# jopohl/urh

Measured on NVIDIA H100. Metric: MSamples/s IQ demod+digitize (complex64), higher is better.
Workload: dtype f32

## Files before the change

urh_b200/csrc/center.cu:

```cuda
#include "dense.cuh"
#include "tilescan.cuh"

#include <math.h>
#include <stdlib.h>

int urh_window_var_bitwise(urh_ctx* ctx, const float* d_x, int64_t n, const int64_t* d_prefix, int64_t t0, int64_t t1, int64_t r0,
                           int64_t r1, float* h_out2);

struct CenStats {
    double sum, sumsq;
    float mn, mx;
    long long cnt;
};

__global__ void __launch_bounds__(URH_WARPS_PER_BLOCK * 32)
k_tile_stats_f32(const float* __restrict__ x, int64_t n, int64_t ntiles, UrhTileStats* __restrict__ ts) {
    const int lane = threadIdx.x & 31;
    const int64_t tile = (int64_t)blockIdx.x * URH_WARPS_PER_BLOCK + (threadIdx.x >> 5);
    if (tile >= ntiles) return;
    const int64_t base = tile * URH_TILE;
    UrhStatAcc acc;
    acc.init();
    acc.all_noise = false;
    if (base + URH_TILE <= n && (((uintptr_t)x) & 15) == 0) {
        const float4* p = (const float4*)(x + base) + lane;
        constexpr int ITERS = URH_TILE / 128;
        float4 cur[4], nxt[4];
#pragma unroll
        for (int j = 0; j < 4; j++) cur[j] = __ldg(p + j * 32);
        for (int it = 0; it < ITERS; it += 4) {
            if (it + 4 < ITERS) {
#pragma unroll
                for (int j = 0; j < 4; j++) nxt[j] = __ldg(p + (it + 4 + j) * 32);
            }
#pragma unroll
            for (int j = 0; j < 4; j++) {
                acc.add(cur[j].x); acc.add(cur[j].y); acc.add(cur[j].z); acc.add(cur[j].w);
            }
#pragma unroll
            for (int j = 0; j < 4; j++) cur[j] = nxt[j];
        }
    } else {
        for (int j = lane; j < URH_TILE; j += 32)
            if (base + j < n) acc.add(x[base + j]);
    }
    acc.store(ts + tile, lane);
}

struct ScanKept {
    const UrhTileStats* ts;
    int64_t* prefix;
    __device__ __forceinline__ int64_t load(int64_t t) const { return ts[t].cnt; }
    __device__ __forceinline__ void post(int64_t t, const int64_t& excl, const int64_t&) const { prefix[t] = excl; }
};
struct CenAddI64 {
    __device__ __forceinline__ int64_t operator()(int64_t a, int64_t b) const { return a + b; }
};

static int kept_prefix(urh_ctx* ctx, const UrhTileStats* ts, int64_t ntiles, int64_t* prefix) {
    ScanKept fk;
    fk.ts = ts; fk.prefix = prefix;
    return urhts::scan<int64_t, CenAddI64, ScanKept>(ctx, ntiles, (int64_t)0, CenAddI64(), fk, prefix + ntiles);
}

#define CEN_PER (URH_TILE / 256)
__device__ __forceinline__ int64_t cen_tile_ranks(const float* __restrict__ x, int64_t n, int64_t t, int64_t tile_rank0, float (&v)[CEN_PER],
                                                  int* s_pre) {
    const int64_t base = t * URH_TILE + (int64_t)threadIdx.x * CEN_PER;
    int mine = 0;
#pragma unroll
    for (int j = 0; j < CEN_PER; j++) {
        v[j] = (base + j < n) ? x[base + j] : -5.0f;
        mine += (v[j] > -4.0f) ? 1 : 0;
    }
    s_pre[threadIdx.x] = mine;
    __syncthreads();
    for (int off = 1; off < 256; off <<= 1) {
        int add = 0;
        if (threadIdx.x >= off) add = s_pre[threadIdx.x - off];
        __syncthreads();
        s_pre[threadIdx.x] += add;
        __syncthreads();
    }
    return tile_rank0 + s_pre[threadIdx.x] - mine;
}

__device__ __forceinline__ void cen_block_fold(double sum, double sq, float mn, float mx, long long cnt, CenStats* out) {
    __shared__ double s_sum[256], s_sq[256];
    __shared__ float s_mn[256], s_mx[256];
    __shared__ long long s_cnt[256];
    __syncthreads();
    s_sum[threadIdx.x] = sum; s_sq[threadIdx.x] = sq; s_mn[threadIdx.x] = mn; s_mx[threadIdx.x] = mx; s_cnt[threadIdx.x] = cnt;
    __syncthreads();
    for (int off = 128; off > 0; off >>= 1) {
        if (threadIdx.x < off) {
            s_sum[threadIdx.x] += s_sum[threadIdx.x + off];
            s_sq[threadIdx.x] += s_sq[threadIdx.x + off];
            s_mn[threadIdx.x] = fminf(s_mn[threadIdx.x], s_mn[threadIdx.x + off]);
            s_mx[threadIdx.x] = fmaxf(s_mx[threadIdx.x], s_mx[threadIdx.x + off]);
            s_cnt[threadIdx.x] += s_cnt[threadIdx.x + off];
        }
        __syncthreads();
    }
    if (threadIdx.x == 0) {
        CenStats r;
        r.sum = s_sum[0]; r.sumsq = s_sq[0]; r.mn = s_mn[0]; r.mx = s_mx[0]; r.cnt = s_cnt[0];
        *out = r;
    }
}

int urh_center_tiles_begin(urh_ctx* ctx, const float* d_x, const UrhTileStats* ts, int64_t n, int64_t* h_total) {
    const int64_t ntiles = urh_div_up(n, URH_TILE);
    int64_t* prefix;
    URH_CHECK(urh_arena(ctx, (size_t)ntiles + 1, &prefix));
    URH_CHECK(kept_prefix(ctx, ts, ntiles, prefix));
    URH_CHECK(urh_read_i64(ctx, prefix + ntiles, 1, h_total));
    ctx->center_prefix = prefix;
    ctx->center_ts = ts;
    ctx->center_n = n;
    ctx->center_x = d_x;
    return URH_OK;
}

static int tiles_from_array(urh_ctx* ctx, const float* d_x, int64_t n, int64_t* h_total) {
    urh_arena_reset(ctx);
    ctx->center_prefix = nullptr;
    const int64_t ntiles = urh_div_up(n, URH_TILE);
    UrhTileStats* ts;
    URH_CHECK(urh_arena(ctx, (size_t)ntiles, &ts));
    URH_LAUNCH(ctx, k_tile_stats_f32, (unsigned)urh_div_up(ntiles, URH_WARPS_PER_BLOCK), URH_WARPS_PER_BLOCK * 32, 0, d_x, n, ntiles, ts);
    return urh_center_tiles_begin(ctx, d_x, ts, n, h_total);
}

static bool tiles_match(const urh_ctx* ctx, const float* d_x, int64_t n) {
    return ctx->center_prefix && ctx->center_n == n && ctx->center_x == (const void*)d_x;
}

extern "C" int urh_center_window_var(urh_ctx* ctx, const float* d_qad, int64_t n, int64_t r0, int64_t r1, double* h_out2) {
    h_out2[0] = h_out2[1] = 0.0;
    if (!tiles_match(ctx, d_qad, n)) URH_FAIL(ctx, URH_ERR_INVALID, "the tile table of this array must precede urh_center_window_var");
    if (r1 <= r0) return URH_OK;
    float mv[2];
    URH_CHECK(urh_window_var_bitwise(ctx, d_qad, n, (const int64_t*)ctx->center_prefix, 0, urh_div_up(n, URH_TILE) - 1, r0, r1, mv));
    h_out2[0] = (double)mv[0];
    h_out2[1] = (double)mv[1];
    return URH_OK;
}

extern "C" int urh_center_stats(urh_ctx* ctx, const float* d_x, int64_t n, int64_t max_size, double* h_out) {
    for (int i = 0; i < 7; i++) h_out[i] = 0.0;
    if (n <= 0) return URH_OK;
    int64_t total = 0;
    URH_CHECK(tiles_from_array(ctx, d_x, n, &total));
    int64_t r0 = (int64_t)(0.05 * (double)total), r1 = (int64_t)(0.95 * (double)total);
    if (max_size >= 0 && r1 - r0 > max_size) r1 = r0 + max_size;
    h_out[0] = (double)total; h_out[1] = (double)r0; h_out[2] = (double)r1;
    if (r1 <= r0) return URH_OK;
    double w[5];
    URH_CHECK(urh_center_window_stats(ctx, d_x, n, r0, r1, w));
    if (w[0] <= 0.0) return URH_OK;
    h_out[3] = w[1]; h_out[4] = w[2];
    float mv[2];
    URH_CHECK(urh_window_var_bitwise(ctx, d_x, n, (const int64_t*)ctx->center_prefix, 0, urh_div_up(n, URH_TILE) - 1, r0, r1, mv));
    h_out[5] = (double)mv[0];
    h_out[6] = (double)mv[1];
    return URH_OK;
}


template <typename K>
__device__ __forceinline__ double cen_edge(K k, const double& hmin, const double& edge1, const double& delta) {
    return (k == 0) ? hmin : (k == 1 ? edge1 : __dadd_rn(hmin, __dmul_rn((double)k, delta)));
}

__device__ __forceinline__ void cen_edge_table(long long k0, long long stride, long long nbins, const double& hmin, const double& edge1,
                                               const double& delta, float* __restrict__ fe, unsigned long long* __restrict__ hist,
                                               unsigned long long* __restrict__ xhist) {
    for (long long k = k0; k <= nbins; k += stride) {
        const double e = cen_edge(k, hmin, edge1, delta);
        fe[k] = __double2float_ru(e);
        if (k == nbins) {
            fe[nbins + 1] = __double2float_rd(e);
            fe[nbins + 2] = fmaxf(__double2float_ru(hmin), nextafterf(-4.0f, 0.0f));
        }
        if (k < nbins) {
            hist[k] = 0ull;
            if (xhist) xhist[k] = 0ull;
        }
    }
}

struct HistBins {
    const float* fe;
    float f_min, f_hi, scale, off;
    int nbins;
    __device__ __forceinline__ void load(const float* fe_, float scale_, int nbins_) {
        fe = fe_; nbins = nbins_; scale = scale_;
        f_hi = fe[nbins + 1];
        f_min = fe[nbins + 2];
        off = -fe[0] * scale;
    }
    template <bool FAST>
    __device__ __forceinline__ int bin_of(float f) const {
        const bool valid = f >= f_min && f <= f_hi;
        if (FAST) {
            const float t = fmaf(f, scale, off);
            int r = __float_as_int(t + 12582912.0f) - 0x4B400000;
            r = max(0, min(r, nbins));
            int k = r - ((f < fe[r]) ? 1 : 0);
            k = min(k, nbins - 1);
            return valid ? k : -1;
        }
        if (!valid) return -1;
        int k = (int)((f - fe[0]) * scale);
        k = max(0, min(k, nbins - 1));
        while (k > 0 && f < fe[k]) k--;
        while (k < nbins - 1 && f >= fe[k + 1]) k++;
        return k;
    }
};

struct HistCache {
    float lo0, hi0, lo1, hi1, lo2, hi2, lo3, hi3;
    int h0, h1, h2, h3;
    unsigned c0, c1, c2, c3;
    __device__ __forceinline__ void init() {
        lo0 = lo1 = lo2 = lo3 = INFINITY;
        hi0 = hi1 = hi2 = hi3 = -INFINITY;
        h0 = h1 = h2 = h3 = 0;
        c0 = c1 = c2 = c3 = 0u;
    }
};

template <bool SMEM>
__device__ __forceinline__ void hist_bump(unsigned int* s_hist, unsigned long long* hist, int k, unsigned c) {
    if (SMEM) atomicAdd(&s_hist[k], c);
    else atomicAdd(&hist[k], (unsigned long long)c);
}

template <bool SMEM, bool FAST>
__device__ __forceinline__ void hist_miss(HistCache& hc, const HistBins& hb, unsigned int* s_hist, unsigned long long* hist, float f) {
    const int k = hb.bin_of<FAST>(f);
    if (k < 0) return;
    const float lo = fmaxf(hb.fe[k], hb.f_min);
    const float hi = (k == hb.nbins - 1) ? nextafterf(hb.f_hi, INFINITY) : hb.fe[k + 1];
    unsigned cm = hc.c0; int which = 0;
    if (hc.c1 < cm) { cm = hc.c1; which = 1; }
    if (hc.c2 < cm) { cm = hc.c2; which = 2; }
    if (hc.c3 < cm) { cm = hc.c3; which = 3; }
    const int old = which == 0 ? hc.h0 : which == 1 ? hc.h1 : which == 2 ? hc.h2 : hc.h3;
    if (cm) hist_bump<SMEM>(s_hist, hist, old, cm);
    if (which == 0) { hc.h0 = k; hc.c0 = 1u; hc.lo0 = lo; hc.hi0 = hi; }
    else if (which == 1) { hc.h1 = k; hc.c1 = 1u; hc.lo1 = lo; hc.hi1 = hi; }
    else if (which == 2) { hc.h2 = k; hc.c2 = 1u; hc.lo2 = lo; hc.hi2 = hi; }
    else { hc.h3 = k; hc.c3 = 1u; hc.lo3 = lo; hc.hi3 = hi; }
}

template <bool SMEM, bool FAST>
__device__ __forceinline__ void hist_put(HistCache& hc, const HistBins& hb, unsigned int* s_hist, unsigned long long* hist, float f,
                                         unsigned one) {
    unsigned miss;
    asm("{\n\t.reg .pred p0, p1, p2, p3, pv;\n\t"
        "setp.ge.f32 p0, %5, %6;\n\tsetp.lt.and.f32 p0, %5, %7, p0;\n\t@p0 mad.lo.u32 %0, %0, %15, %15;\n\t"
        "setp.ge.f32 p1, %5, %8;\n\tsetp.lt.and.f32 p1, %5, %9, p1;\n\t@p1 mad.lo.u32 %1, %1, %15, %15;\n\t"
        "setp.ge.f32 p2, %5, %10;\n\tsetp.lt.and.f32 p2, %5, %11, p2;\n\t@p2 mad.lo.u32 %2, %2, %15, %15;\n\t"
        "setp.ge.f32 p3, %5, %12;\n\tsetp.lt.and.f32 p3, %5, %13, p3;\n\t@p3 mad.lo.u32 %3, %3, %15, %15;\n\t"
        "or.pred p0, p0, p1;\n\tor.pred p2, p2, p3;\n\tor.pred p0, p0, p2;\n\t"
        "setp.ge.f32 pv, %5, %14;\n\t"
        "and.pred pv, pv, !p0;\n\t"
        "selp.u32 %4, 1, 0, pv;\n\t}"
        : "+r"(hc.c0), "+r"(hc.c1), "+r"(hc.c2), "+r"(hc.c3), "=r"(miss)
        : "f"(f), "f"(hc.lo0), "f"(hc.hi0), "f"(hc.lo1), "f"(hc.hi1), "f"(hc.lo2), "f"(hc.hi2), "f"(hc.lo3), "f"(hc.hi3),
          "f"(hb.f_min), "r"(one));
    if (miss) hist_miss<SMEM, FAST>(hc, hb, s_hist, hist, f);
}

template <bool SMEM>
__device__ __forceinline__ void hist_flush(HistCache& hc, unsigned int* s_hist, unsigned long long* hist) {
    if (hc.c0) hist_bump<SMEM>(s_hist, hist, hc.h0, hc.c0);
    if (hc.c1) hist_bump<SMEM>(s_hist, hist, hc.h1, hc.c1);
    if (hc.c2) hist_bump<SMEM>(s_hist, hist, hc.h2, hc.c2);
    if (hc.c3) hist_bump<SMEM>(s_hist, hist, hc.h3, hc.c3);
}

template <bool SMEM, bool FAST>
__device__ __forceinline__ void hist_interior_body(const float* __restrict__ x, int64_t n, int64_t t_first, int64_t t_end, int blk, int nblk,
                                                   const float* __restrict__ g_fe, float scale, int nbins,
                                                   unsigned long long* __restrict__ hist, int edges_in_smem,
                                                   const int64_t* __restrict__ prefix) {
    extern __shared__ unsigned int s_dyn[];
    unsigned int* s_hist = s_dyn;
    float* s_fe = (float*)(s_dyn + (SMEM ? nbins : 0));
    const int lane = threadIdx.x & 31;
    if (SMEM)
        for (int b = threadIdx.x; b < nbins; b += 256) s_hist[b] = 0u;
    if (edges_in_smem)
        for (int b = threadIdx.x; b < nbins + 3; b += 256) s_fe[b] = g_fe[b];
    __syncthreads();
    HistBins hb;
    if (FAST) hb.load(s_fe, scale, nbins);
    else hb.load(edges_in_smem ? s_fe : g_fe, scale, nbins);
    HistCache hc;
    hc.init();
    const int64_t gw = (int64_t)blk * 8 + (threadIdx.x >> 5), nw = (int64_t)nblk * 8;
    const bool vec = (((uintptr_t)x) & 15) == 0;
    const unsigned one = blockDim.x >> 8;
    {
        for (int64_t t = t_first + gw; t < t_end; t += nw) {
            if (prefix[t + 1] == prefix[t]) continue;
            const int64_t base = t * URH_TILE;
            if (vec) {
                const float4* p = (const float4*)(x + base) + lane;
                constexpr int ITERS = URH_TILE / 128, DEPTH = 4;
                float4 buf[DEPTH];
#pragma unroll
                for (int j = 0; j < DEPTH; j++) buf[j] = __ldg(p + j * 32);
#pragma unroll 1
                for (int it = 0; it < ITERS; it += DEPTH) {
                    const bool more = it + DEPTH < ITERS;
#pragma unroll
                    for (int j = 0; j < DEPTH; j++) {
                        const float4 v = buf[j];
                        if (more) buf[j] = __ldg(p + (it + DEPTH + j) * 32);
                        hist_put<SMEM, FAST>(hc, hb, s_hist, hist, v.x, one);
                        hist_put<SMEM, FAST>(hc, hb, s_hist, hist, v.y, one);
                        hist_put<SMEM, FAST>(hc, hb, s_hist, hist, v.z, one);
                        hist_put<SMEM, FAST>(hc, hb, s_hist, hist, v.w, one);
                    }
                }
            } else {
                for (int j = lane; j < URH_TILE; j += 32) hist_put<SMEM, FAST>(hc, hb, s_hist, hist, x[base + j], one);
            }
        }
    }
    hist_flush<SMEM>(hc, s_hist, hist);
    if (SMEM) {
        __syncthreads();
        for (int b = threadIdx.x; b < nbins; b += 256)
            if (s_hist[b]) atomicAdd(&hist[b], (unsigned long long)s_hist[b]);
    }
}

__device__ __forceinline__ void hist_window_ends_body(const float* __restrict__ x, int64_t n, const int64_t* __restrict__ prefix,
                                                      const int64_t* __restrict__ win, int64_t r0, int64_t r1,
                                                      const float* __restrict__ g_fe, float scale, int nbins,
                                                      unsigned long long* __restrict__ hist, unsigned long long* __restrict__ hist2 = nullptr) {
    __shared__ int s_pre[256];
    const int64_t t = win[blockIdx.x];
    if (t < 0 || (blockIdx.x == 1 && t == win[0])) return;
    HistBins hb;
    hb.load(g_fe, scale, nbins);
    float v[CEN_PER];
    int64_t rank = cen_tile_ranks(x, n, t, prefix[t], v, s_pre);
#pragma unroll
    for (int j = 0; j < CEN_PER; j++) {
        const bool kept = v[j] > -4.0f;
        const int k = hb.bin_of<false>(v[j]);
        if (k >= 0 && rank >= r0 && rank < r1) {
            atomicAdd(&hist[k], 1ull);
            if (hist2) atomicAdd(&hist2[k], 1ull);
        }
        rank += kept ? 1 : 0;
    }
}

extern "C" int urh_center_histogram(urh_ctx* ctx, const float* d_x, int64_t n, int64_t r0, int64_t r1, double hmin,
                                    double hstep, int64_t nbins, int64_t* h_hist) {
    if (nbins <= 0 || n <= 0) return URH_OK;
    if (!tiles_match(ctx, d_x, n)) {
        int64_t total = 0;
        URH_CHECK(tiles_from_array(ctx, d_x, n, &total));
    }
    return urh_center_histogram_tiles(ctx, d_x, n, r0, r1, hmin, hstep, nbins, h_hist);
}

#define CEN_MAX_BINS 6000
#define CEN_VAR_MIN_RATIO 0x1p-14

struct __align__(16) CenterPlan {
    long long total, offset;
    long long r0, r1;
    long long lr0, lr1;
    long long win[4];
    CenStats local;
    double hmin, edge1, delta;
    long long nbins;
    double center;
    float centerf;
    float scale;
    int fast;
    int state;
    unsigned int ticket;
    int certified;
    long long straddle;
    long long pad;
};

__global__ void k_center_ranks(const int64_t* __restrict__ counts, int rank, int world, int64_t max_size, CenterPlan* __restrict__ plan) {
    long long total = 0, offset = 0;
    for (int q = 0; q < world; q++) {
        if (q < rank) offset += counts[q];
        total += counts[q];
    }
    const long long kept = counts[rank];
    long long r0 = (long long)(0.05 * (double)total), r1 = (long long)(0.95 * (double)total);
    if (max_size >= 0 && r1 - r0 > max_size) r1 = r0 + max_size;
    plan->total = total; plan->offset = offset; plan->r0 = r0; plan->r1 = r1;
    long long a = r0 - offset, b = r1 - offset;
    a = a < 0 ? 0 : (a > kept ? kept : a);
    b = b < 0 ? 0 : (b > kept ? kept : b);
    plan->lr0 = a; plan->lr1 = b;
    plan->ticket = 0u;
    plan->state = 1;
    plan->certified = 0;
    plan->straddle = 0;
}

__device__ __forceinline__ int64_t cen_tile_of_rank(const int64_t* __restrict__ prefix, int64_t ntiles, int64_t r) {
    int64_t lo = 0, hi = ntiles;
    while (hi - lo > 1) {
        const int64_t mid = (lo + hi) >> 1;
        if (prefix[mid] <= r) lo = mid; else hi = mid;
    }
    return lo;
}

__device__ __forceinline__ void cen_window_tiles(const int64_t* __restrict__ prefix, int64_t ntiles, long long r0, long long r1,
                                                 long long (&w)[4]) {
    long long w0 = -1, w1 = -1, w2 = -1, w3 = -1;
    if (r1 > r0) {
        w0 = cen_tile_of_rank(prefix, ntiles, r0);
        w1 = cen_tile_of_rank(prefix, ntiles, r1 - 1);
        const bool cov0 = prefix[w0] >= r0 && prefix[w0 + 1] <= r1;
        const bool cov1 = prefix[w1] >= r0 && prefix[w1 + 1] <= r1;
        w2 = cov0 ? -1 : w0;
        w3 = (cov1 || w1 == w0) ? -1 : w1;
    }
    w[0] = w0; w[1] = w1; w[2] = w2; w[3] = w3;
}

__global__ void __launch_bounds__(256) k_center_window(const float* __restrict__ x, int64_t n, const UrhTileStats* __restrict__ ts,
                                                      const int64_t* __restrict__ prefix, int64_t ntiles, CenterPlan* __restrict__ plan,
                                                      CenStats* __restrict__ partial) {
    __shared__ long long s_win[4];
    __shared__ int s_pre[256];
    __shared__ bool s_last;
    const long long r0 = plan->lr0, r1 = plan->lr1;
    if (threadIdx.x == 0) {
        long long w[4];
        cen_window_tiles(prefix, ntiles, r0, r1, w);
        s_win[0] = w[0]; s_win[1] = w[1]; s_win[2] = w[2]; s_win[3] = w[3];
        if (blockIdx.x == 0) { plan->win[0] = w[0]; plan->win[1] = w[1]; plan->win[2] = w[2]; plan->win[3] = w[3]; }
    }
    __syncthreads();
    double sum = 0.0, sq = 0.0;
    float mn = INFINITY, mx = -INFINITY;
    long long cnt = 0;
    if (s_win[0] >= 0) {
        for (int64_t t = s_win[0] + (int64_t)blockIdx.x * 256 + threadIdx.x; t <= s_win[1]; t += (int64_t)gridDim.x * 256) {
            const int64_t a = prefix[t], b = prefix[t + 1];
            if (b > a && a >= r0 && b <= r1) {
                const UrhTileStats v = ts[t];
                sum += v.sum; sq += v.sumsq; mn = fminf(mn, v.mn); mx = fmaxf(mx, v.mx); cnt += v.cnt;
            }
        }
    }
    cen_block_fold(sum, sq, mn, mx, cnt, partial + blockIdx.x);
    if (blockIdx.x < 2) {
        const int64_t t = s_win[2 + blockIdx.x];
        sum = 0.0; sq = 0.0; mn = INFINITY; mx = -INFINITY; cnt = 0;
        if (t >= 0) {
            float v[CEN_PER];
            int64_t rank = cen_tile_ranks(x, n, t, prefix[t], v, s_pre);
#pragma unroll
            for (int j = 0; j < CEN_PER; j++) {
                if (v[j] > -4.0f) {
                    if (rank >= r0 && rank < r1) {
                        sum += (double)v[j];
                        sq += (double)v[j] * (double)v[j];
                        mn = fminf(mn, v[j]);
                        mx = fmaxf(mx, v[j]);
                        cnt++;
                    }
                    rank++;
                }
            }
        }
        cen_block_fold(sum, sq, mn, mx, cnt, partial + gridDim.x + blockIdx.x);
    }
    __threadfence();
    __syncthreads();
    if (threadIdx.x == 0) s_last = atomicAdd(&plan->ticket, 1u) == gridDim.x - 1;
    __syncthreads();
    if (!s_last) return;
    __threadfence();
    sum = 0.0; sq = 0.0; mn = INFINITY; mx = -INFINITY; cnt = 0;
    for (int64_t t = threadIdx.x; t < (int64_t)gridDim.x + 2; t += 256) {
        CenStats p;
        {
            const int4* src = (const int4*)(partial + t);
            int4 w0 = __ldcg(src), w1 = __ldcg(src + 1);
            memcpy(&p, &w0, 16);
            memcpy((char*)&p + 16, &w1, 16);
        }
        sum += p.sum; sq += p.sumsq; mn = fminf(mn, p.mn); mx = fmaxf(mx, p.mx); cnt += p.cnt;
    }
    cen_block_fold(sum, sq, mn, mx, cnt, &plan->local);
}

__global__ void __launch_bounds__(256) k_center_plan(const CenStats* __restrict__ parts, int world, CenterPlan* __restrict__ plan,
                                                    float* __restrict__ fe, unsigned long long* __restrict__ hist,
                                                    unsigned long long* __restrict__ xhist) {
    __shared__ int s_state;
    __shared__ long long s_nbins;
    __shared__ double s_hmin, s_edge1, s_delta;
    if (threadIdx.x == 0) {
        double cnt = 0.0, sum = 0.0, sq = 0.0;
        float mn = INFINITY, mx = -INFINITY;
        for (int q = 0; q < world; q++) {
            cnt += (double)parts[q].cnt;
            mn = fminf(mn, parts[q].mn);
            mx = fmaxf(mx, parts[q].mx);
            sum = __dadd_rn(sum, parts[q].sum);
            sq = __dadd_rn(sq, parts[q].sumsq);
        }
        int state = 0;
        long long nbins = 0;
        double hmin = 0.0, edge1 = 0.0, delta = 0.0;
        if (plan->r1 > plan->r0 && cnt > 0.0) {
            const double mean = __ddiv_rn(sum, cnt);
            double ss = __dsub_rn(sq, __dmul_rn(__dmul_rn(cnt, mean), mean));
            if (ss < 0.0) ss = 0.0;
            const double var = __ddiv_rn(ss, cnt);
            const double hstep = (double)__double2float_rn(var);
            hmin = (double)mn;
            const double stop = __dadd_rn((double)mx, hstep);
            if (!(var >= __dmul_rn(__dmul_rn(mean, mean), CEN_VAR_MIN_RATIO))) state = 2;
            else if (hstep != 0.0) {
                const double val = __ddiv_rn(__dsub_rn(stop, hmin), hstep);
                if (val == val && fabs(val) < 9.0e18) {
                    const long long len = (long long)ceil(val);
                    if (len >= 2) {
                        nbins = len - 1;
                        edge1 = __dadd_rn(hmin, hstep);
                        delta = __dsub_rn(edge1, hmin);
                        state = (nbins <= CEN_MAX_BINS && delta > 0.0) ? 1 : 2;
                    }
                }
            }
        }
        plan->hmin = hmin; plan->edge1 = edge1; plan->delta = delta; plan->nbins = nbins;
        plan->state = state;
        plan->center = 0.0; plan->centerf = 0.0f;
        if (state == 1) {
            plan->scale = (float)(1.0 / delta);
            const double edge_abs = fmax(fabs(hmin), fabs(hmin + (double)nbins * delta));
            plan->fast = (edge_abs / delta < 1048576.0) ? 1 : 0;
        }
        s_state = state; s_nbins = nbins; s_hmin = hmin; s_edge1 = edge1; s_delta = delta;
    }
    __syncthreads();
    if (s_state != 1) return;
    cen_edge_table(threadIdx.x, 256, s_nbins, s_hmin, s_edge1, s_delta, fe, hist, xhist);
}

template <bool SMEM, bool FAST, int MIN_BLOCKS>
__global__ void __launch_bounds__(256, MIN_BLOCKS) k_hist_interior(const float* __restrict__ x, int64_t n, const CenterPlan* __restrict__ plan,
                                                                  const float* __restrict__ g_fe, unsigned long long* __restrict__ hist,
                                                                  const int64_t* __restrict__ prefix, int edges_in_smem) {
    if (plan->state != 1 || plan->certified || (plan->fast != 0) != FAST) return;
    hist_interior_body<SMEM, FAST>(x, n, plan->win[0] + 1, plan->win[1], blockIdx.x, gridDim.x, g_fe, plan->scale, (int)plan->nbins, hist,
                                   edges_in_smem, prefix);
}

__device__ __forceinline__ void cen_full_slabs(int64_t win0, int64_t win1, int64_t slab_tiles, int64_t* sf, int64_t* se) {
    *sf = (win0 + slab_tiles) / slab_tiles;
    *se = win1 / slab_tiles;
}

__global__ void __launch_bounds__(256) k_hist_window_ends(const float* __restrict__ x, int64_t n, const int64_t* __restrict__ prefix,
                                                         const CenterPlan* __restrict__ plan, const float* __restrict__ g_fe,
                                                         unsigned long long* __restrict__ hist, unsigned long long* __restrict__ xhist,
                                                         int64_t slab_tiles) {
    if (plan->state != 1) return;
    if (blockIdx.x < 2) {
        hist_window_ends_body(x, n, prefix, (const int64_t*)plan->win, plan->lr0, plan->lr1, g_fe, plan->scale, (int)plan->nbins, hist, xhist);
        return;
    }
    const int64_t w0 = plan->win[0], w1 = plan->win[1];
    int64_t sf, se;
    cen_full_slabs(w0, w1, slab_tiles, &sf, &se);
    int64_t a_end = w1, b_begin = w1;
    if (sf < se) { a_end = sf * slab_tiles; b_begin = se * slab_tiles; }
    const int blk = blockIdx.x - 2, nblk = gridDim.x - 2, nbins = (int)plan->nbins;
    const float scale = plan->scale;
    if (plan->fast) {
        hist_interior_body<true, true>(x, n, w0 + 1, a_end, blk, nblk, g_fe, scale, nbins, xhist, 1, prefix);
        hist_interior_body<true, true>(x, n, b_begin, w1, blk, nblk, g_fe, scale, nbins, xhist, 1, prefix);
    } else {
        hist_interior_body<true, false>(x, n, w0 + 1, a_end, blk, nblk, g_fe, scale, nbins, xhist, 1, prefix);
        hist_interior_body<true, false>(x, n, b_begin, w1, blk, nblk, g_fe, scale, nbins, xhist, 1, prefix);
    }
}

__device__ __forceinline__ double cen_left_edge(const CenterPlan* plan, int k) {
    return cen_edge(k, plan->hmin, plan->edge1, plan->delta);
}

#define CERT_THREADS 512
__global__ void __launch_bounds__(CERT_THREADS) k_center_certify(const UrhFine fine, CenterPlan* __restrict__ plan, const float* __restrict__ fe,
                                                                 const unsigned long long* __restrict__ xhist, unsigned long long* __restrict__ lo,
                                                                 unsigned long long* __restrict__ hi) {
    __shared__ unsigned long long s_ge[URH_FINE_NB + 1];
    __shared__ unsigned long long s_part[CERT_THREADS];
    __shared__ unsigned char s_flag[CEN_MAX_BINS];
    __shared__ unsigned long long s_key[3];
    __shared__ unsigned int s_certain;
    if (plan->state != 1) return;
    const int tid = threadIdx.x;
    constexpr int PER = URH_FINE_NB / CERT_THREADS;
    int64_t sf, se;
    cen_full_slabs(plan->win[0], plan->win[1], fine.slab_tiles, &sf, &se);
    unsigned long long b[PER], tot = 0;
#pragma unroll
    for (int j = 0; j < PER; j++) {
        unsigned long long v = 0;
        for (int64_t sl = sf; sl < se; sl++) v += fine.gh[sl * URH_FINE_NB + tid * PER + j];
        b[j] = v;
        tot += v;
    }
    s_part[tid] = tot;
    if (tid < 3) s_key[tid] = 0ull;
    if (tid == 0) s_certain = 0u;
    __syncthreads();
    for (int off = 1; off < CERT_THREADS; off <<= 1) {
        const unsigned long long add = (tid + off < CERT_THREADS) ? s_part[tid + off] : 0ull;
        __syncthreads();
        s_part[tid] += add;
        __syncthreads();
    }
    unsigned long long run = (tid + 1 < CERT_THREADS) ? s_part[tid + 1] : 0ull;
#pragma unroll
    for (int j = PER - 1; j >= 0; j--) {
        run += b[j];
        s_ge[tid * PER + j] = run;
    }
    if (tid == 0) s_ge[URH_FINE_NB] = 0ull;
    __syncthreads();
    const int nbins = (int)plan->nbins;
    const float f_hi = fe[nbins + 1], f_min = fe[nbins + 2], top = nextafterf(f_hi, INFINITY);
    auto ge = [&](float t, unsigned long long& glo, unsigned long long& ghi) {
        const int bt = urh_fine_bucket(t, fine.scale, fine.off);
        const bool straddles = urh_fine_bucket(nextafterf(t, -INFINITY), fine.scale, fine.off) == bt;
        ghi = s_ge[bt];
        glo = straddles ? s_ge[bt + 1] : s_ge[bt];
    };
    for (int k = tid; k < nbins; k += CERT_THREADS) {
        const float a = fmaxf(fe[k], f_min), e = (k == nbins - 1) ? top : fminf(fe[k + 1], top);
        unsigned long long l = 0, u = 0;
        if (a < e) {
            unsigned long long alo, ahi, elo, ehi;
            ge(a, alo, ahi);
            ge(e, elo, ehi);
            l = alo > ehi ? alo - ehi : 0ull;
            u = ahi - elo;
        }
        lo[k] = xhist[k] + l;
        hi[k] = xhist[k] + u;
    }
    __syncthreads();
    int window = (int)(0.05 * (double)nbins) + 1;
    if (window < 2) window = 2;
    for (int k = tid; k < nbins; k += CERT_THREADS) {
        const unsigned long long l = lo[k], u = hi[k];
        bool certain = l > 0ull, possible = u > 0ull;
        for (int d = -(window - 1); d < window && (certain || possible); d++) {
            const int j = k + d;
            if (d == 0 || j < 0 || j >= nbins) continue;
            certain = certain && l > hi[j];
            possible = possible && u > lo[j];
        }
        s_flag[k] = certain ? 1 : (possible ? 2 : 0);
        if (certain) atomicAdd(&s_certain, 1u);
    }
    __syncthreads();
    for (int pass = 0; pass < 3; pass++) {
        const long long p0 = pass > 0 ? (long long)(8191 - (s_key[0] & 8191)) : -1, p1 = pass > 1 ? (long long)(8191 - (s_key[1] & 8191)) : -1;
        for (int k = tid; k < nbins; k += CERT_THREADS) {
            if (k == p0 || k == p1) continue;
            if (pass < 2 && s_flag[k] == 1) atomicMax(&s_key[pass], (lo[k] << 13) | (unsigned long long)(8191 - k));
            if (pass == 2 && s_flag[k] != 0) atomicMax(&s_key[2], hi[k]);
        }
        __syncthreads();
    }
    if (tid != 0 || s_certain < 2u) return;
    const int k1 = 8191 - (int)(s_key[0] & 8191), k2 = 8191 - (int)(s_key[1] & 8191);
    plan->straddle = (long long)((hi[k1] - lo[k1]) + (hi[k2] - lo[k2]));
    if (!(lo[k2] > s_key[2])) return;
    const double c = __ddiv_rn(__dadd_rn(cen_left_edge(plan, k1), cen_left_edge(plan, k2)), 2.0);
    plan->center = c;
    plan->centerf = __double2float_rn(c);
    plan->certified = 1;
}

__global__ void __launch_bounds__(256) k_center_pick(const unsigned long long* __restrict__ y, CenterPlan* __restrict__ plan) {
    __shared__ unsigned long long s_best[256];
    __shared__ int s_idx[256];
    __shared__ int s_cnt[256];
    if (plan->state != 1 || plan->certified) return;
    const int nbins = (int)plan->nbins;
    int window = (int)(0.05 * (double)nbins) + 1;
    if (window < 2) window = 2;
    unsigned long long top_val[2] = {0ull, 0ull};
    int top_idx[2] = {-1, -1};
    int found = 0;
    bool undecided = false;
    for (int pass = 0; pass < 2 && !undecided; pass++) {
        unsigned long long best = 0ull;
        int bi = -1, ties = 0;
        for (int i = threadIdx.x; i < nbins; i += 256) {
            if (pass == 1 && i == top_idx[0]) continue;
            const unsigned long long v = y[i];
            if (v == 0ull || v < best) continue;
            bool peak = true;
            for (int d = 1; d < window && peak; d++) {
                const unsigned long long a = (i + d < nbins) ? y[i + d] : 0ull;
                const unsigned long long b = (i - d >= 0) ? y[i - d] : 0ull;
                peak = v > a && v > b;
            }
            if (!peak) continue;
            if (v > best) { best = v; bi = i; ties = 1; }
            else ties++;
        }
        s_best[threadIdx.x] = best; s_idx[threadIdx.x] = bi; s_cnt[threadIdx.x] = ties;
        __syncthreads();
        if (threadIdx.x == 0) {
            unsigned long long b = 0ull;
            int idx = -1, t = 0;
            for (int j = 0; j < 256; j++) {
                if (s_idx[j] < 0) continue;
                if (s_best[j] > b) { b = s_best[j]; idx = s_idx[j]; t = s_cnt[j]; }
                else if (s_best[j] == b) t += s_cnt[j];
            }
            s_best[0] = b; s_idx[0] = idx; s_cnt[0] = t;
        }
        __syncthreads();
        const unsigned long long b = s_best[0];
        const int idx = s_idx[0], t = s_cnt[0];
        __syncthreads();
        if (idx < 0) break;
        if (pass == 0) {
            top_val[0] = b; top_idx[0] = idx; found = 1;
            if (t == 2) {
                int other = -1;
                for (int i = threadIdx.x; i < nbins; i += 256) {
                    if (i == idx || y[i] != b) continue;
                    bool peak = true;
                    for (int d = 1; d < window && peak; d++) {
                        const unsigned long long a = (i + d < nbins) ? y[i + d] : 0ull;
                        const unsigned long long c = (i - d >= 0) ? y[i - d] : 0ull;
                        peak = b > a && b > c;
                    }
                    if (peak) other = i;
                }
                s_idx[threadIdx.x] = other;
                __syncthreads();
                if (threadIdx.x == 0) {
                    int o = -1;
                    for (int j = 0; j < 256; j++) if (s_idx[j] >= 0) o = s_idx[j];
                    s_idx[0] = o;
                }
                __syncthreads();
                top_idx[1] = s_idx[0]; top_val[1] = b; found = 2;
                __syncthreads();
                break;
            }
            if (t > 2) undecided = true;
        } else {
            if (t > 1) undecided = true;
            else { top_val[1] = b; top_idx[1] = idx; found = 2; }
        }
    }
    if (threadIdx.x != 0) return;
    if (undecided) { plan->state = 2; return; }
    if (found == 0) { plan->state = 0; return; }
    double c;
    if (found == 1) c = cen_left_edge(plan, top_idx[0]);
    else c = __ddiv_rn(__dadd_rn(cen_left_edge(plan, top_idx[0]), cen_left_edge(plan, top_idx[1])), 2.0);
    plan->center = c;
    plan->centerf = __double2float_rn(c);
    plan->state = 1;
    (void)top_val;
}

__global__ void __launch_bounds__(256) k_center_set(const int64_t* __restrict__ prefix, int64_t ntiles, long long r0, long long r1, double hmin,
                                                   double hstep, long long nbins, float scale, int fast, CenterPlan* __restrict__ plan,
                                                   float* __restrict__ fe, unsigned long long* __restrict__ hist) {
    const double edge1 = __dadd_rn(hmin, hstep);
    if (blockIdx.x == 0 && threadIdx.x == 0) {
        plan->lr0 = r0; plan->lr1 = r1;
        plan->ticket = 0u;
        plan->state = 1;
        plan->certified = 0;
        if (nbins > 0) {
            long long w[4];
            cen_window_tiles(prefix, ntiles, r0, r1, w);
            for (int i = 0; i < 4; i++) plan->win[i] = w[i];
            plan->hmin = hmin; plan->edge1 = edge1; plan->delta = hstep; plan->nbins = nbins;
            plan->scale = scale;
            plan->fast = fast;
        }
    }
    if (nbins > 0)
        cen_edge_table((long long)blockIdx.x * blockDim.x + threadIdx.x, (long long)gridDim.x * blockDim.x, nbins, hmin, edge1, hstep, fe, hist,
                       nullptr);
}

extern "C" int urh_center_window_stats(urh_ctx* ctx, const float* d_qad, int64_t n, int64_t r0, int64_t r1, double* h_out5) {
    h_out5[0] = 0.0; h_out5[1] = INFINITY; h_out5[2] = -INFINITY; h_out5[3] = 0.0; h_out5[4] = 0.0;
    if (!tiles_match(ctx, d_qad, n)) URH_FAIL(ctx, URH_ERR_INVALID, "urh_afp_demod_tiles (same qad, same n) must precede urh_center_window_stats");
    if (r1 <= r0) return URH_OK;
    const int64_t ntiles = urh_div_up(n, URH_TILE);
    const int64_t* prefix = (const int64_t*)ctx->center_prefix;
    CenterPlan* plan;
    CenStats* partial;
    const int nb = ctx->sm_count * 2;
    URH_CHECK(urh_arena(ctx, 1, &plan));
    URH_CHECK(urh_arena(ctx, (size_t)nb + 2, &partial));
    URH_LAUNCH(ctx, k_center_set, 1, 1, 0, prefix, ntiles, (long long)r0, (long long)r1, 0.0, 0.0, 0LL, 0.0f, 0, plan, nullptr, nullptr);
    URH_LAUNCH(ctx, k_center_window, nb, 256, 0, d_qad, n, (const UrhTileStats*)ctx->center_ts, prefix, ntiles, plan, partial);
    CenStats st;
    URH_CUDA(ctx, cudaMemcpyAsync(ctx->h_mail, &plan->local, sizeof(CenStats), cudaMemcpyDeviceToHost, ctx->stream));
    URH_CUDA(ctx, cudaStreamSynchronize(ctx->stream));
    memcpy(&st, ctx->h_mail, sizeof(st));
    h_out5[0] = (double)st.cnt; h_out5[1] = (double)st.mn; h_out5[2] = (double)st.mx; h_out5[3] = st.sum; h_out5[4] = st.sumsq;
    return URH_OK;
}

extern "C" int urh_center_histogram_tiles(urh_ctx* ctx, const float* d_qad, int64_t n, int64_t r0, int64_t r1, double hmin,
                                          double hstep, int64_t nbins, int64_t* h_hist) {
    if (nbins <= 0) return URH_OK;
    if (!tiles_match(ctx, d_qad, n)) URH_FAIL(ctx, URH_ERR_INVALID, "urh_afp_demod_tiles (same qad, same n) must precede urh_center_histogram_tiles");
    if (nbins > (int64_t)1 << 30) URH_FAIL(ctx, URH_ERR_INVALID, "too many histogram bins");
    if (r1 <= r0) {
        memset(h_hist, 0, (size_t)nbins * sizeof(int64_t));
        return URH_OK;
    }
    const int64_t ntiles = urh_div_up(n, URH_TILE);
    const int64_t* prefix = (const int64_t*)ctx->center_prefix;
    CenterPlan* plan;
    float* fe;
    unsigned long long* hist;
    URH_CHECK(urh_arena(ctx, 1, &plan));
    URH_CHECK(urh_arena(ctx, (size_t)nbins + 3, &fe));
    URH_CHECK(urh_arena(ctx, (size_t)nbins, &hist));
    const bool in_smem = nbins <= 12000;
    const int edges_smem = (in_smem && nbins <= 6000) ? 1 : 0;
    const size_t dyn = (in_smem ? (size_t)nbins * 4 : 0) + (edges_smem ? (size_t)(nbins + 3) * 4 : 0);
    const float scale = (float)(1.0 / hstep);
    const double edge_abs = fmax(fabs(hmin), fabs(hmin + (double)nbins * hstep));
    const int fast = (edges_smem && hstep > 0.0 && edge_abs / hstep < 1048576.0) ? 1 : 0;
    const unsigned gs = (unsigned)min(urh_div_up(ntiles, 8), (int64_t)ctx->sm_count * 8);
    URH_LAUNCH(ctx, k_center_set, (unsigned)urh_div_up(nbins + 1, 256), 256, 0, prefix, ntiles, (long long)r0, (long long)r1, hmin, hstep,
               (long long)nbins, scale, fast, plan, fe, hist);
    const CenterPlan* cplan = plan;
    const float* cfe = fe;
    if (fast) URH_LAUNCH(ctx, (k_hist_interior<true, true, 3>), gs, 256, dyn, d_qad, n, cplan, cfe, hist, prefix, edges_smem);
    else if (edges_smem) URH_LAUNCH(ctx, (k_hist_interior<true, false, 3>), gs, 256, dyn, d_qad, n, cplan, cfe, hist, prefix, edges_smem);
    else if (in_smem) URH_LAUNCH(ctx, (k_hist_interior<true, false, 4>), gs, 256, dyn, d_qad, n, cplan, cfe, hist, prefix, edges_smem);
    else URH_LAUNCH(ctx, (k_hist_interior<false, false, 4>), gs, 256, dyn, d_qad, n, cplan, cfe, hist, prefix, edges_smem);
    URH_LAUNCH(ctx, k_hist_window_ends, 2, 256, 0, d_qad, n, prefix, cplan, cfe, hist, (unsigned long long*)nullptr, (int64_t)1);
    URH_CUDA(ctx, cudaMemcpyAsync(h_hist, hist, (size_t)nbins * sizeof(int64_t), cudaMemcpyDeviceToHost, ctx->stream));
    URH_CUDA(ctx, cudaStreamSynchronize(ctx->stream));
    return URH_OK;
}

int urh_center_chain(urh_ctx* ctx, const float* d_qad, int64_t n, const UrhTileStats* ts, int64_t max_size, int rank, int world,
                     const UrhFine* fine, CenterPlan** d_plan_out) {
    const int64_t ntiles = urh_div_up(n, URH_TILE);
    int64_t* prefix;
    CenterPlan* plan;
    CenStats* partial;
    float* fe;
    unsigned long long* hist;
    int64_t* d_counts;
    CenStats* d_parts;
    unsigned long long *xhist = nullptr, *cert_lo = nullptr, *cert_hi = nullptr;
    const int nb = ctx->sm_count * 2;
    URH_CHECK(urh_arena(ctx, (size_t)ntiles + 1, &prefix));
    URH_CHECK(urh_arena(ctx, 1, &plan));
    URH_CHECK(urh_arena(ctx, (size_t)nb + 2, &partial));
    URH_CHECK(urh_arena(ctx, (size_t)CEN_MAX_BINS + 3, &fe));
    URH_CHECK(urh_arena(ctx, (size_t)CEN_MAX_BINS, &hist));
    URH_CHECK(urh_arena(ctx, (size_t)world, &d_counts));
    URH_CHECK(urh_arena(ctx, (size_t)world, &d_parts));
    if (fine) {
        URH_CHECK(urh_arena(ctx, (size_t)CEN_MAX_BINS, &xhist));
        URH_CHECK(urh_arena(ctx, (size_t)CEN_MAX_BINS, &cert_lo));
        URH_CHECK(urh_arena(ctx, (size_t)CEN_MAX_BINS, &cert_hi));
    }
    URH_CHECK(kept_prefix(ctx, ts, ntiles, prefix));
    const int64_t* counts = prefix + ntiles;
    if (world > 1) {
        URH_TL_MARK(ctx, "x1 kept counts: enter");
        URH_CHECK(urh_nccl_allgather(ctx, prefix + ntiles, d_counts, sizeof(int64_t)));
        URH_TL_MARK(ctx, "x1 kept counts: done");
        counts = d_counts;
    }
    URH_LAUNCH(ctx, k_center_ranks, 1, 1, 0, counts, rank, world, max_size, plan);
    URH_LAUNCH(ctx, k_center_window, nb, 256, 0, d_qad, n, ts, (const int64_t*)prefix, ntiles, plan, partial);
    const CenStats* parts = &plan->local;
    if (world > 1) {
        URH_TL_MARK(ctx, "x2 window partials: enter");
        URH_CHECK(urh_nccl_allgather(ctx, &plan->local, d_parts, sizeof(CenStats)));
        URH_TL_MARK(ctx, "x2 window partials: done");
        parts = d_parts;
    }
    URH_LAUNCH(ctx, k_center_plan, 1, 256, 0, parts, world, plan, fe, hist, xhist);
    const size_t dyn = (size_t)CEN_MAX_BINS * 4 + (size_t)(CEN_MAX_BINS + 3) * 4;
    const unsigned gs = (unsigned)min(urh_div_up(ntiles, 8), (int64_t)ctx->sm_count * 8);
    URH_LAUNCH(ctx, k_hist_window_ends, fine ? 2 + ctx->sm_count * 4 : 2, 256, fine ? dyn : 0, d_qad, n, (const int64_t*)prefix,
               (const CenterPlan*)plan, (const float*)fe, hist, xhist, fine ? fine->slab_tiles : (int64_t)1);
    if (fine) URH_LAUNCH(ctx, k_center_certify, 1, CERT_THREADS, 0, *fine, plan, (const float*)fe, (const unsigned long long*)xhist, cert_lo, cert_hi);
    URH_LAUNCH(ctx, (k_hist_interior<true, true, 3>), gs, 256, dyn, d_qad, n, (const CenterPlan*)plan, (const float*)fe, hist, (const int64_t*)prefix, 1);
    URH_LAUNCH(ctx, (k_hist_interior<true, false, 3>), gs, 256, dyn, d_qad, n, (const CenterPlan*)plan, (const float*)fe, hist, (const int64_t*)prefix, 1);
    if (world > 1) {
        URH_TL_MARK(ctx, "x3 histogram sum: enter");
        URH_CHECK(urh_nccl_allreduce_i64(ctx, (int64_t*)hist, CEN_MAX_BINS, 0));
        URH_TL_MARK(ctx, "x3 histogram sum: done");
    }
    URH_LAUNCH(ctx, k_center_pick, 1, 256, 0, (const unsigned long long*)hist, plan);
    ctx->center_prefix = prefix;
    ctx->center_ts = ts;
    ctx->center_n = n;
    ctx->center_x = d_qad;
    *d_plan_out = plan;
    return URH_OK;
}

int urh_center_plan_certify_stats(urh_ctx* ctx, const CenterPlan* plan, int64_t* h_dst3) {
    h_dst3[0] = h_dst3[1] = h_dst3[2] = 0;
    URH_CUDA(ctx, cudaMemcpyAsync(h_dst3, &plan->certified, sizeof(int), cudaMemcpyDeviceToHost, ctx->stream));
    URH_CUDA(ctx, cudaMemcpyAsync(h_dst3 + 2, &plan->straddle, sizeof(long long), cudaMemcpyDeviceToHost, ctx->stream));
    return URH_OK;
}

extern "C" int urh_center_certify_stats(urh_ctx* ctx, int64_t* h_out3) {
    for (int i = 0; i < 3; i++) h_out3[i] = ctx->center_cert[i];
    return URH_OK;
}

int urh_center_plan_result(urh_ctx* ctx, const CenterPlan* plan, const float** d_centerf, const double** d_center, const int** d_state) {
    if (d_centerf) *d_centerf = &plan->centerf;
    if (d_center) *d_center = &plan->center;
    if (d_state) *d_state = &plan->state;
    return URH_OK;
}
```

urh_b200/csrc/dense.cuh:

```cuda
#pragma once
#include "common.cuh"
#include "fdlibm_atan2f.h"

#define URH_TILE 2048
#define URH_WARPS_PER_BLOCK 8
#define URH_MAX_THR 255

struct UrhClassify {
    float noise_value;
    int order;
    float thr[URH_MAX_THR];
};

struct __align__(16) UrhTileSummary {
    int16_t first_cls;
    int16_t last_cls;
    int32_t head_len;
    int32_t tail_len;
    int32_t ncand;
};

struct __align__(16) UrhTileStats {
    double sum, sumsq;
    float mn, mx;
    int32_t cnt;
    int32_t all_noise;
};

struct UrhStatAcc {
    double sum, sumsq;
    float mn, mx;
    int cnt;
    bool all_noise;
    __device__ __forceinline__ void init() { sum = 0.0; sumsq = 0.0; mn = INFINITY; mx = -INFINITY; cnt = 0; all_noise = true; }
    __device__ __forceinline__ void add(float v) {
        if (v > -4.0f) {
            const double d = (double)v;
            sum += d;
            sumsq += d * d;
            mn = fminf(mn, v);
            mx = fmaxf(mx, v);
            cnt++;
        }
    }
    __device__ __forceinline__ void store(UrhTileStats* out, int lane) {
        for (int off = 16; off > 0; off >>= 1) {
            sum += __shfl_down_sync(URH_FULL_MASK, sum, off);
            sumsq += __shfl_down_sync(URH_FULL_MASK, sumsq, off);
            mn = fminf(mn, __shfl_down_sync(URH_FULL_MASK, mn, off));
            mx = fmaxf(mx, __shfl_down_sync(URH_FULL_MASK, mx, off));
            cnt += __shfl_down_sync(URH_FULL_MASK, cnt, off);
        }
        const int alln = __all_sync(URH_FULL_MASK, all_noise) ? 1 : 0;
        if (lane == 0) {
            UrhTileStats t;
            t.sum = sum; t.sumsq = sumsq; t.mn = mn; t.mx = mx; t.cnt = cnt; t.all_noise = alln;
            *out = t;
        }
    }
};

#define URH_FINE_NB 4096
#define URH_FINE_SLABS 64
struct UrhFine {
    unsigned int* gh;
    int64_t slab_tiles;
    float scale, off;
};
__device__ __forceinline__ int urh_fine_bucket(float f, float scale, float off) {
    float t = __fmaf_rd(f, scale, off + 8388608.0f);
    t = fminf(fmaxf(t, 8388608.0f), 8388608.0f + (float)(URH_FINE_NB - 1));
    return __float_as_int(t) - 0x4B000000;
}
__device__ __forceinline__ void urh_fine_add(float f, const UrhFine& fn, unsigned int* s, unsigned int* g) {
    if (f > -4.0f) {
        const int b = urh_fine_bucket(f, fn.scale, fn.off);
        if (g) atomicAdd(g + b, 1u);
        else atomicAdd(s + b, 1u);
    }
}
__device__ __forceinline__ unsigned int* urh_fine_row(const UrhFine& fn, int64_t tile, int64_t block_tile0) {
    const int64_t slab = tile / fn.slab_tiles;
    return (slab == block_tile0 / fn.slab_tiles) ? nullptr : fn.gh + slab * URH_FINE_NB;
}
__device__ __forceinline__ void urh_fine_zero(unsigned int* s) {
    for (int w = threadIdx.x * 4; w < URH_FINE_NB; w += blockDim.x * 4) *(uint4*)(s + w) = make_uint4(0u, 0u, 0u, 0u);
    __syncthreads();
}
__device__ __forceinline__ void urh_fine_flush(const UrhFine& fn, unsigned int* s, int64_t block_tile0) {
    __syncthreads();
    unsigned int* g = fn.gh + (block_tile0 / fn.slab_tiles) * URH_FINE_NB;
    for (int w = threadIdx.x * 4; w < URH_FINE_NB; w += blockDim.x * 4) {
        const uint4 v = *(const uint4*)(s + w);
        if (v.x) atomicAdd(g + w, v.x);
        if (v.y) atomicAdd(g + w + 1, v.y);
        if (v.z) atomicAdd(g + w + 2, v.z);
        if (v.w) atomicAdd(g + w + 3, v.w);
    }
}

__device__ __forceinline__ void urh_cmulf(float a, float b, float c, float d, float& re, float& im) {
    const float ac = __fmul_rn(a, c), bd = __fmul_rn(b, d), ad = __fmul_rn(a, d), bc = __fmul_rn(b, c);
    re = __fsub_rn(ac, bd);
    im = __fadd_rn(ad, bc);
    if (isnan(re) && isnan(im)) {
        bool recalc = false;
        if (isinf(a) || isinf(b)) {
            a = copysignf(isinf(a) ? 1.0f : 0.0f, a);
            b = copysignf(isinf(b) ? 1.0f : 0.0f, b);
            if (isnan(c)) c = copysignf(0.0f, c);
            if (isnan(d)) d = copysignf(0.0f, d);
            recalc = true;
        }
        if (isinf(c) || isinf(d)) {
            c = copysignf(isinf(c) ? 1.0f : 0.0f, c);
            d = copysignf(isinf(d) ? 1.0f : 0.0f, d);
            if (isnan(a)) a = copysignf(0.0f, a);
            if (isnan(b)) b = copysignf(0.0f, b);
            recalc = true;
        }
        if (!recalc && (isinf(ac) || isinf(bd) || isinf(ad) || isinf(bc))) {
            if (isnan(a)) a = copysignf(0.0f, a);
            if (isnan(b)) b = copysignf(0.0f, b);
            if (isnan(c)) c = copysignf(0.0f, c);
            if (isnan(d)) d = copysignf(0.0f, d);
            recalc = true;
        }
        if (recalc) {
            re = __fmul_rn(INFINITY, __fsub_rn(__fmul_rn(a, c), __fmul_rn(b, d)));
            im = __fmul_rn(INFINITY, __fadd_rn(__fmul_rn(a, d), __fmul_rn(b, c)));
        }
    }
}

template <int DT> struct UrhElem;
template <> struct UrhElem<URH_DT_I8> { typedef int8_t type; };
template <> struct UrhElem<URH_DT_U8> { typedef uint8_t type; };
template <> struct UrhElem<URH_DT_I16> { typedef int16_t type; };
template <> struct UrhElem<URH_DT_U16> { typedef uint16_t type; };
template <> struct UrhElem<URH_DT_F32> { typedef float type; };

struct UrhPair {
    float r0, i0, r1, i1;
};

__device__ __forceinline__ float4 urh_ldg_f4(const void* p) {
    float4 v;
    asm volatile("ld.global.nc.L1::no_allocate.v4.f32 {%0,%1,%2,%3}, [%4];"
                 : "=f"(v.x), "=f"(v.y), "=f"(v.z), "=f"(v.w)
                 : "l"(p));
    return v;
}
__device__ __forceinline__ uint2 urh_ldg_u2(const void* p) {
    uint2 v;
    asm volatile("ld.global.nc.L1::no_allocate.v2.u32 {%0,%1}, [%2];" : "=r"(v.x), "=r"(v.y) : "l"(p));
    return v;
}
__device__ __forceinline__ uint32_t urh_ldg_u1(const void* p) {
    uint32_t v;
    asm volatile("ld.global.nc.L1::no_allocate.u32 %0, [%1];" : "=r"(v) : "l"(p));
    return v;
}
__device__ __forceinline__ void urh_stg_f2(float* p, float a, float b) {
    asm volatile("st.global.L1::no_allocate.v2.f32 [%0], {%1,%2};" ::"l"(p), "f"(a), "f"(b) : "memory");
}

template <int DT>
__device__ __forceinline__ UrhPair urh_load_pair(const void* base, int64_t i, int64_t n, bool vec) {
    typedef typename UrhElem<DT>::type E;
    const E* p = (const E*)base + 2 * i;
    UrhPair o;
    o.r0 = o.i0 = o.r1 = o.i1 = 0.0f;
    if (i + 1 < n && vec) {
        if (DT == URH_DT_F32) {
            const float4 v = urh_ldg_f4(p);
            o.r0 = v.x; o.i0 = v.y; o.r1 = v.z; o.i1 = v.w;
        } else if (DT == URH_DT_I16) {
            const uint2 v = urh_ldg_u2(p);
            o.r0 = (float)(int16_t)(v.x & 0xffff); o.i0 = (float)(int16_t)(v.x >> 16);
            o.r1 = (float)(int16_t)(v.y & 0xffff); o.i1 = (float)(int16_t)(v.y >> 16);
        } else if (DT == URH_DT_U16) {
            const uint2 v = urh_ldg_u2(p);
            o.r0 = (float)(v.x & 0xffff); o.i0 = (float)(v.x >> 16);
            o.r1 = (float)(v.y & 0xffff); o.i1 = (float)(v.y >> 16);
        } else if (DT == URH_DT_I8) {
            const uint32_t v = urh_ldg_u1(p);
            o.r0 = (float)(int8_t)(v & 0xff); o.i0 = (float)(int8_t)((v >> 8) & 0xff);
            o.r1 = (float)(int8_t)((v >> 16) & 0xff); o.i1 = (float)(int8_t)(v >> 24);
        } else {
            const uint32_t v = urh_ldg_u1(p);
            o.r0 = (float)(v & 0xff); o.i0 = (float)((v >> 8) & 0xff);
            o.r1 = (float)((v >> 16) & 0xff); o.i1 = (float)(v >> 24);
        }
    } else {
        if (i < n) { o.r0 = (float)__ldg(p); o.i0 = (float)__ldg(p + 1); }
        if (i + 1 < n) { o.r1 = (float)__ldg(p + 2); o.i1 = (float)__ldg(p + 3); }
    }
    return o;
}

struct UrhDemodParams {
    float noise_sqrd;
    float noise_value;
    float max_mag;
    float one, mone;
};

struct UrhFskTerms {
    float A, B, C, D;
};
__device__ __forceinline__ UrhFskTerms urh_fsk_terms(float re, float im) {
    UrhFskTerms t;
    const float zt = __fsub_rn(__fmul_rn(0.0f, im), 0.0f);
    t.C = __fadd_rn(re, zt);
    t.A = __fsub_rn(re, zt);
    t.D = __fadd_rn(0.0f, im);
    t.B = __fsub_rn(0.0f, t.D);
    return t;
}
__device__ __forceinline__ float urh_fsk_angle(float A, float B, float C, float D) {
    float xr, xi;
    urh_cmulf(A, B, C, D, xr, xi);
    return urh_atan2f_v2(xi, xr);
}

__device__ __forceinline__ int urh_classify(float s, const UrhClassify& C) {
    if (s == C.noise_value) return -1;
    if (C.order == 2) return (s <= C.thr[0]) ? 0 : 1;
    int c = C.order - 1;
    for (int k = 0; k < C.order - 1; k++) {
        if (s <= C.thr[k]) { c = k; break; }
    }
    return c;
}

__device__ __forceinline__ uint64_t urh_spread_bits(uint32_t x) {
    uint64_t v = x;
    v = (v | (v << 16)) & 0x0000FFFF0000FFFFull;
    v = (v | (v << 8)) & 0x00FF00FF00FF00FFull;
    v = (v | (v << 4)) & 0x0F0F0F0F0F0F0F0Full;
    v = (v | (v << 2)) & 0x3333333333333333ull;
    v = (v | (v << 1)) & 0x5555555555555555ull;
    return v;
}

struct UrhRunTracker {
    int tol;
    int run_start, run_cls, first_cls, head_len, ncand, carry_cls;
    bool is_head;
    uint32_t cm_n, cm_a;
    uint32_t* stage;

    __device__ __forceinline__ void init(int tol_, uint32_t* stage_) {
        tol = tol_; stage = stage_;
        run_start = 0; run_cls = -2; first_cls = -2; head_len = 0; ncand = 0; carry_cls = -2; is_head = true;
        cm_n = 0xffffffffu; cm_a = 0xffffffffu;
    }
    __device__ __forceinline__ void emit(int pos, int cls, int lane) {
        if (lane == 0) stage[ncand] = ((uint32_t)pos << 16) | (uint32_t)(cls + 1);
        ncand++;
    }
    __device__ __forceinline__ void feed(int it, int c0, int c1, bool v0, bool v1, int lane) {
        int pc = __shfl_up_sync(URH_FULL_MASK, c1, 1);
        if (lane == 0) pc = carry_cls;
        const bool b0 = v0 && (c0 != pc);
        const bool b1 = v1 && (c1 != c0);
        carry_cls = __shfl_sync(URH_FULL_MASK, c1, 31);
        const uint32_t m0 = __ballot_sync(URH_FULL_MASK, b0);
        const uint32_t m1 = __ballot_sync(URH_FULL_MASK, b1);
        if ((m0 | m1) == 0u) return;
        walk(it, m0, m1, c0, c1, lane);
    }
    __device__ __forceinline__ void feed_masks(int it, uint32_t n0, uint32_t a0, uint32_t n1, uint32_t a1, int lane) {
        if ((((n0 ^ cm_n) | (n1 ^ cm_n)) | ((a0 ^ cm_a) | (a1 ^ cm_a))) == 0u) return;
        uint32_t m0 = (((n1 << 1) | (cm_n & 1u)) ^ n0) | (((a1 << 1) | (cm_a & 1u)) ^ a0);
        if (run_cls == -2) m0 |= 1u;
        uint32_t m1 = (n0 ^ n1) | (a0 ^ a1);
        feed_masks_slow(it, n0, a0, n1, a1, m0, m1, lane);
        cm_n = (run_cls < 0) ? 0xffffffffu : 0u;
        cm_a = (run_cls == 1) ? 0xffffffffu : 0u;
    }
    __device__ __forceinline__ void feed_masks_slow(int it, uint32_t n0, uint32_t a0, uint32_t n1, uint32_t a1, uint32_t m0, uint32_t m1,
                                                    int lane) {
        const int nb = __popc(m0) + __popc(m1);
        if (nb == 1 && run_cls != -2 && !is_head) {
            const bool take0 = m0 != 0u;
            const int l = __ffs(m0 | m1) - 1;
            const int p = it * 64 + 2 * l + (take0 ? 0 : 1);
            const uint32_t nbit = ((take0 ? n0 : n1) >> l) & 1u, abit = ((take0 ? a0 : a1) >> l) & 1u;
            if (p - run_start > tol) emit(run_start + tol, run_cls, lane);
            run_start = p;
            run_cls = nbit ? -1 : (int)abit;
            return;
        }
        if (nb > 4) {
            const int c0 = ((n0 >> lane) & 1u) ? -1 : (int)((a0 >> lane) & 1u);
            const int c1 = ((n1 >> lane) & 1u) ? -1 : (int)((a1 >> lane) & 1u);
            walk_parallel(it, m0, m1, c0, c1, lane);
            return;
        }
        while (m0 | m1) {
            const int l0 = m0 ? (__ffs(m0) - 1) : 64;
            const int l1 = m1 ? (__ffs(m1) - 1) : 64;
            const bool take0 = l0 <= l1;
            const int l = take0 ? l0 : l1;
            if (take0) m0 &= m0 - 1; else m1 &= m1 - 1;
            const int p = it * 64 + 2 * l + (take0 ? 0 : 1);
            const uint32_t nbit = ((take0 ? n0 : n1) >> l) & 1u, abit = ((take0 ? a0 : a1) >> l) & 1u;
            const int cls_p = nbit ? -1 : (int)abit;
            if (run_cls == -2) {
                first_cls = cls_p;
            } else if (is_head) {
                head_len = p;
                is_head = false;
            } else if (p - run_start > tol) {
                emit(run_start + tol, run_cls, lane);
            }
            run_start = p;
            run_cls = cls_p;
        }
    }
    __device__ __forceinline__ void walk(int it, uint32_t m0, uint32_t m1, int c0, int c1, int lane) {
        if (__popc(m0) + __popc(m1) > 4) {
            walk_parallel(it, m0, m1, c0, c1, lane);
            return;
        }
        while (m0 | m1) {
            const int l0 = m0 ? (__ffs(m0) - 1) : 64;
            const int l1 = m1 ? (__ffs(m1) - 1) : 64;
            const bool take0 = l0 <= l1;
            const int l = take0 ? l0 : l1;
            if (take0) m0 &= m0 - 1; else m1 &= m1 - 1;
            const int p = it * 64 + 2 * l + (take0 ? 0 : 1);
            const int cls_p = __shfl_sync(URH_FULL_MASK, take0 ? c0 : c1, l);
            if (run_cls == -2) {
                first_cls = cls_p;
            } else if (is_head) {
                head_len = p;
                is_head = false;
            } else if (p - run_start > tol) {
                emit(run_start + tol, run_cls, lane);
            }
            run_start = p;
            run_cls = cls_p;
        }
    }
    __device__ __forceinline__ void walk_parallel(int it, uint32_t m0, uint32_t m1, int c0, int c1, int lane) {
        const uint32_t lt = (1u << lane) - 1u;
        const int base = it * 64;
        int cprev0 = __shfl_up_sync(URH_FULL_MASK, c1, 1);
        if (lane == 0) cprev0 = run_cls;
        const int cprev1 = c0;
        const uint32_t b1 = m1 & lt, b0 = m0 & lt;
        int q0 = -1;
        if (b1) q0 = 2 * (31 - __clz(b1)) + 1;
        if (b0) q0 = max(q0, 2 * (31 - __clz(b0)));
        const bool has0 = (m0 >> lane) & 1u, has1 = (m1 >> lane) & 1u;
        const int q1 = has0 ? 2 * lane : q0;
        const bool carried_head = is_head;
        const int start0 = (q0 >= 0) ? base + q0 : run_start;
        const int start1 = (q1 >= 0) ? base + q1 : run_start;
        const int p0 = base + 2 * lane, p1 = p0 + 1;
        const bool head0 = (q0 >= 0) ? (start0 == 0) : (carried_head || run_cls == -2);
        const bool head1 = (q1 >= 0) ? (start1 == 0) : (carried_head || run_cls == -2);
        const bool emit0 = has0 && !head0 && (p0 - start0 > tol);
        const bool emit1 = has1 && !head1 && (p1 - start1 > tol);
        const uint32_t e0 = __ballot_sync(URH_FULL_MASK, emit0), e1 = __ballot_sync(URH_FULL_MASK, emit1);
        const int before = __popc(e0 & lt) + __popc(e1 & lt);
        if (emit0) stage[ncand + before] = ((uint32_t)(start0 + tol) << 16) | (uint32_t)(cprev0 + 1);
        if (emit1) stage[ncand + before + (emit0 ? 1 : 0)] = ((uint32_t)(start1 + tol) << 16) | (uint32_t)(cprev1 + 1);
        ncand += __popc(e0) + __popc(e1);
        uint32_t f0 = m0, f1 = m1;
        if (run_cls == -2) {
            first_cls = __shfl_sync(URH_FULL_MASK, c0, 0);
            f0 &= ~1u;
        }
        if (is_head && (f0 | f1)) {
            const int l0 = f0 ? (__ffs(f0) - 1) : 64, l1 = f1 ? (__ffs(f1) - 1) : 64;
            head_len = base + ((l0 <= l1) ? 2 * l0 : 2 * l1 + 1);
            is_head = false;
        }
        const int h0 = m0 ? (31 - __clz(m0)) : -1, h1 = m1 ? (31 - __clz(m1)) : -1;
        const bool last_is_1 = h1 >= h0;
        const int hl = last_is_1 ? h1 : h0;
        run_start = base + 2 * hl + (last_is_1 ? 1 : 0);
        run_cls = __shfl_sync(URH_FULL_MASK, last_is_1 ? c1 : c0, hl);
    }
    __device__ __forceinline__ void finish(int tile_len, UrhTileSummary* out, int lane) {
        if (is_head) head_len = tile_len;
        else if (tile_len - run_start > tol) emit(run_start + tol, run_cls, lane);
        if (lane == 0) {
            UrhTileSummary s;
            s.first_cls = (int16_t)first_cls;
            s.last_cls = (int16_t)run_cls;
            s.head_len = head_len;
            s.tail_len = tile_len - run_start;
            s.ncand = ncand;
            *out = s;
        }
    }
};

struct UrhTileResolve {
    uint32_t n0, a0, n1, a1;
    __device__ __forceinline__ void init() { n0 = a0 = n1 = a1 = 0u; }
    __device__ __forceinline__ void keep(int g, uint32_t gn0, uint32_t ga0, uint32_t gn1, uint32_t ga1, int lane) {
        if (lane == g) { n0 = gn0; a0 = ga0; n1 = gn1; a1 = ga1; }
    }
    __device__ __forceinline__ static int cls_of(uint32_t nbit, uint32_t abit) { return (nbit & 1u) ? -1 : (int)(abit & 1u); }

    template <bool WRITE>
    __device__ __forceinline__ int walk(uint32_t m0, uint32_t m1, uint32_t pn, uint32_t pa, int q, int tol, int lane, uint32_t* dst) const {
        int k = 0;
        const int base = lane * 64;
        while (m0 | m1) {
            const int l0 = m0 ? (__ffs(m0) - 1) : 64;
            const int l1 = m1 ? (__ffs(m1) - 1) : 64;
            const bool take0 = l0 <= l1;
            const int l = take0 ? l0 : l1;
            if (take0) m0 &= m0 - 1; else m1 &= m1 - 1;
            const int p = base + 2 * l + (take0 ? 0 : 1);
            if (q > 0 && p - q > tol) {
                if (WRITE) {
                    uint32_t nb, ab;
                    if (!take0) { nb = n0 >> l; ab = a0 >> l; }
                    else if (l > 0) { nb = n1 >> (l - 1); ab = a1 >> (l - 1); }
                    else { nb = pn; ab = pa; }
                    dst[k] = ((uint32_t)(q + tol) << 16) | (uint32_t)(cls_of(nb, ab) + 1);
                }
                k++;
            }
            q = p;
        }
        return k;
    }

    __device__ __forceinline__ void finish(int tol, uint32_t* stage, UrhTileSummary* out, int lane) const {
        const uint32_t pn = __shfl_up_sync(URH_FULL_MASK, n1 >> 31, 1), pa = __shfl_up_sync(URH_FULL_MASK, a1 >> 31, 1);
        uint32_t m0 = (((n1 << 1) | (pn & 1u)) ^ n0) | (((a1 << 1) | (pa & 1u)) ^ a0);
        if (lane == 0) m0 |= 1u;
        const uint32_t m1 = (n0 ^ n1) | (a0 ^ a1);
        int last = -1;
        if (m1) last = lane * 64 + 2 * (31 - __clz(m1)) + 1;
        if (m0) last = max(last, lane * 64 + 2 * (31 - __clz(m0)));
        int incl = last;
#pragma unroll
        for (int off = 1; off < 32; off <<= 1) {
            const int t = __shfl_up_sync(URH_FULL_MASK, incl, off);
            if (lane >= off) incl = max(incl, t);
        }
        int q = __shfl_up_sync(URH_FULL_MASK, incl, 1);
        if (lane == 0) q = -1;
        const int L = __shfl_sync(URH_FULL_MASK, incl, 31);
        uint32_t f0 = m0, f1 = m1;
        if (lane == 0) f0 &= ~1u;
        int first = URH_TILE;
        if (f0 | f1) {
            const int l0 = f0 ? (__ffs(f0) - 1) : 64, l1 = f1 ? (__ffs(f1) - 1) : 64;
            first = lane * 64 + ((l0 <= l1) ? 2 * l0 : 2 * l1 + 1);
        }
        const int head_len = __reduce_min_sync(URH_FULL_MASK, first);
        const int mine = walk<false>(m0, m1, pn, pa, q, tol, lane, nullptr);
        int pre = mine;
#pragma unroll
        for (int off = 1; off < 32; off <<= 1) {
            const int t = __shfl_up_sync(URH_FULL_MASK, pre, off);
            if (lane >= off) pre += t;
        }
        int total = __shfl_sync(URH_FULL_MASK, pre, 31);
        if (mine) walk<true>(m0, m1, pn, pa, q, tol, lane, stage + (pre - mine));
        const int last_cls = __shfl_sync(URH_FULL_MASK, cls_of(n1 >> 31, a1 >> 31), 31);
        if (L > 0 && URH_TILE - L > tol) {
            if (lane == 0) stage[total] = ((uint32_t)(L + tol) << 16) | (uint32_t)(last_cls + 1);
            total++;
        }
        if (lane == 0) {
            UrhTileSummary s;
            s.first_cls = (int16_t)cls_of(n0, a0);
            s.last_cls = (int16_t)last_cls;
            s.head_len = head_len;
            s.tail_len = URH_TILE - L;
            s.ncand = total;
            *out = s;
        }
    }
};
```

urh_b200/csrc/digitize.cu:

```cuda
#include "dense.cuh"
#include "tilescan.cuh"
#include "sparse.cuh"
#include "fsk_fast.cuh"
#include "dense_f32.cuh"
#include "stream_ring.cuh"

#include <math.h>
#include <stdlib.h>


template <int DT, int MOD, bool DIGITIZE>
__device__ __forceinline__ void dense_iq_tile(const void* __restrict__ iq, int64_t n, const UrhDemodParams& dp, float* __restrict__ qad_out,
                                              int vec_in, int vec_out, const UrhClassify& cls, int tol, UrhTileSummary* __restrict__ tiles,
                                              uint32_t* __restrict__ staging, int stage_cap, int16_t* __restrict__ init_cls, int cls_of_zero,
                                              int64_t tile, int has_halo, UrhTileStats* __restrict__ tile_stats, const UrhFine& fine,
                                              unsigned int* s_fine, unsigned int* g_fine) {
    const int lane = threadIdx.x & 31;
    const int64_t tile_start = tile * URH_TILE;
    const int tile_len = (int)((n - tile_start) < URH_TILE ? (n - tile_start) : URH_TILE);
    const int iters = (tile_len + 63) >> 6;

    UrhRunTracker rt;
    if (DIGITIZE) rt.init(tol, staging + tile * (int64_t)stage_cap);
    UrhStatAcc acc;
    acc.init();

    float cA = 0.0f, cB = 0.0f;
    if (MOD == URH_MOD_FSK && (tile_start > 0 || has_halo) && lane == 0) {
        typedef typename UrhElem<DT>::type E;
        const E* pp = (const E*)iq + 2 * (tile_start - 1);
        const UrhFskTerms t = urh_fsk_terms((float)pp[0], (float)pp[1]);
        cA = t.A; cB = t.B;
    }

    UrhPair cur = urh_load_pair<DT>(iq, tile_start + 2 * lane, n, vec_in != 0);
    for (int it = 0; it < iters; it++) {
        const int64_t pos0 = tile_start + (int64_t)it * 64 + 2 * lane;
        UrhPair nxt;
        if (it + 1 < iters) nxt = urh_load_pair<DT>(iq, pos0 + 64, n, vec_in != 0);

        const float m0 = __fadd_rn(__fmul_rn(cur.r0, cur.r0), __fmul_rn(cur.i0, cur.i0));
        const float m1 = __fadd_rn(__fmul_rn(cur.r1, cur.r1), __fmul_rn(cur.i1, cur.i1));
        float s0 = dp.noise_value, s1 = dp.noise_value;
        if (MOD == URH_MOD_FSK) {
            const UrhFskTerms t0 = urh_fsk_terms(cur.r0, cur.i0);
            const UrhFskTerms t1 = urh_fsk_terms(cur.r1, cur.i1);
            float pA = __shfl_up_sync(URH_FULL_MASK, t1.A, 1);
            float pB = __shfl_up_sync(URH_FULL_MASK, t1.B, 1);
            if (lane == 0) { pA = cA; pB = cB; }
            cA = __shfl_sync(URH_FULL_MASK, t1.A, 31);
            cB = __shfl_sync(URH_FULL_MASK, t1.B, 31);
            if (!(m0 <= dp.noise_sqrd)) s0 = urh_fsk_angle(pA, pB, t0.C, t0.D);
            if (!(m1 <= dp.noise_sqrd)) s1 = urh_fsk_angle(t0.A, t0.B, t1.C, t1.D);
        } else if (MOD == URH_MOD_ASK) {
            if (!(m0 <= dp.noise_sqrd)) s0 = __fdiv_rn(__fsqrt_rn(m0), dp.max_mag);
            if (!(m1 <= dp.noise_sqrd)) s1 = __fdiv_rn(__fsqrt_rn(m1), dp.max_mag);
        }
        if (pos0 == 0 && !has_halo) s0 = dp.noise_value;

        const bool v0 = pos0 < n, v1 = pos0 + 1 < n;
        if (tile_stats) {
            if (v0) { acc.add(s0); acc.all_noise = acc.all_noise && (s0 == dp.noise_value); }
            if (v1) { acc.add(s1); acc.all_noise = acc.all_noise && (s1 == dp.noise_value); }
            if (s_fine) {
                if (v0) urh_fine_add(s0, fine, s_fine, g_fine);
                if (v1) urh_fine_add(s1, fine, s_fine, g_fine);
            }
        }
        if (qad_out) {
            if (v1 && vec_out) urh_stg_f2(qad_out + pos0, s0, s1);
            else {
                if (v0) qad_out[pos0] = s0;
                if (v1) qad_out[pos0 + 1] = s1;
            }
        }
        if (DIGITIZE) {
            const int c0 = urh_classify(s0, cls), c1 = urh_classify(s1, cls);
            if (pos0 == 0) *init_cls = (int16_t)((s0 == cls.noise_value) ? -1 : cls_of_zero);
            rt.feed(it, c0, c1, v0, v1, lane);
        }
        cur = nxt;
    }
    if (tile_stats) acc.store(tile_stats + tile, lane);
    if (DIGITIZE) rt.finish(tile_len, tiles + tile, lane);
}

template <int DT, int MOD, bool DIGITIZE>
__global__ void __launch_bounds__(URH_WARPS_PER_BLOCK * 32)
k_dense_iq(const void* __restrict__ iq, int64_t n, UrhDemodParams dp, float* __restrict__ qad_out, int vec_in,
           int vec_out, const __grid_constant__ UrhClassify cls, int tol, UrhTileSummary* __restrict__ tiles,
           uint32_t* __restrict__ staging, int stage_cap, int16_t* __restrict__ init_cls, int cls_of_zero,
           int64_t tile_begin, int64_t tile_count, int has_halo, UrhTileStats* __restrict__ tile_stats, const UrhFine fine) {
    extern __shared__ unsigned int s_fine[];
    const int64_t tile_rel = (int64_t)blockIdx.x * URH_WARPS_PER_BLOCK + (threadIdx.x >> 5);
    const int64_t block_tile0 = tile_begin + (int64_t)blockIdx.x * URH_WARPS_PER_BLOCK;
    if (fine.gh) urh_fine_zero(s_fine);
    if (tile_rel < tile_count && (tile_begin + tile_rel) * URH_TILE < n)
        dense_iq_tile<DT, MOD, DIGITIZE>(iq, n, dp, qad_out, vec_in, vec_out, cls, tol, tiles, staging, stage_cap, init_cls, cls_of_zero,
                                    tile_begin + tile_rel, has_halo, tile_stats, fine,
                                    fine.gh ? s_fine : nullptr, fine.gh ? urh_fine_row(fine, tile_begin + tile_rel, block_tile0) : nullptr);
    if (fine.gh) urh_fine_flush(fine, s_fine, block_tile0);
}

template <int DT, bool DIGITIZE, bool WRITE, bool STATS>
__global__ void __launch_bounds__(URH_WARPS_PER_BLOCK * 32, (DT == URH_DT_F32) ? 5 : 4)
k_fsk_fifo(const void* __restrict__ iq, int64_t n, UrhDemodParams dp, float* __restrict__ qad_out, float thr0,
           float cls_noise, int tol, UrhTileSummary* __restrict__ tiles, uint32_t* __restrict__ staging, int stage_cap,
           int64_t tile_begin, int64_t tile_count, UrhTileStats* __restrict__ tile_stats, const UrhFine fine,
           const float* __restrict__ d_thr0 = nullptr, float* __restrict__ margin = nullptr) {
    __shared__ __align__(16) unsigned char s_fifo[URH_WARPS_PER_BLOCK][URH_FSK_FIFO + 1][64 * 2 * sizeof(typename UrhElem<DT>::type)];
    extern __shared__ unsigned int s_fine[];
    const bool fine_on = STATS && fine.gh;
    if (DIGITIZE && STATS) thr0 = *d_thr0;
    const int lane = threadIdx.x & 31;
    const int64_t tile_rel = (int64_t)blockIdx.x * URH_WARPS_PER_BLOCK + (threadIdx.x >> 5);
    const int64_t block_tile0 = tile_begin + (int64_t)blockIdx.x * URH_WARPS_PER_BLOCK;
    if (fine_on) urh_fine_zero(s_fine);
    if (tile_rel < tile_count) {
        const int64_t tile = tile_begin + tile_rel;
        UrhRunTracker rt;
        if (DIGITIZE) rt.init(tol, staging + tile * (int64_t)stage_cap);
        UrhOne one;
        one.p = dp.one;
        one.m = dp.mone;
        const uint32_t fifo = (uint32_t)__cvta_generic_to_shared(&s_fifo[threadIdx.x >> 5][0][0]);
        urh_fsk_full_tile<DT, DIGITIZE, WRITE, STATS>(iq, n, tile * URH_TILE, dp, qad_out, thr0, cls_noise, rt, lane, one,
                                                      STATS ? tile_stats + tile : nullptr, fifo, DIGITIZE ? tiles + tile : nullptr, fine,
                                                      fine_on ? s_fine : nullptr, fine_on ? urh_fine_row(fine, tile, block_tile0) : nullptr,
                                                      (DIGITIZE && STATS) ? margin + tile : nullptr);
    }
    if (fine_on) urh_fine_flush(fine, s_fine, block_tile0);
}

#define URH_GUESS_SAMPLES 16384
#define URH_GUESS_BINS 128
#define URH_GUESS_THREADS 1024
__global__ void __launch_bounds__(URH_GUESS_THREADS) k_speculate_guess(const float2* __restrict__ iq, int64_t n, float noise_sqrd, int forced,
                                                                      float forced_tg, float* __restrict__ d_tg, unsigned int* __restrict__ redone) {
    constexpr int PER = URH_GUESS_SAMPLES / URH_GUESS_THREADS;
    __shared__ unsigned int s_hist[URH_GUESS_BINS];
    __shared__ float s_mn[32], s_mx[32];
    if (forced) {
        if (threadIdx.x == 0) { *d_tg = forced_tg; *redone = 0u; }
        return;
    }
    for (int b = threadIdx.x; b < URH_GUESS_BINS; b += blockDim.x) s_hist[b] = 0u;
    float v[PER];
    float mn = INFINITY, mx = -INFINITY;
#pragma unroll
    for (int k = 0; k < PER; k++) {
        const int64_t i = 1 + (int64_t)(k * URH_GUESS_THREADS + threadIdx.x) * (n - 1) / URH_GUESS_SAMPLES;
        const float2 p = iq[i - 1], c = iq[i];
        v[k] = NAN;
        if (!(c.x * c.x + c.y * c.y <= noise_sqrd)) {
            v[k] = atan2f(p.x * c.y - p.y * c.x, p.x * c.x + p.y * c.y);
            mn = fminf(mn, v[k]);
            mx = fmaxf(mx, v[k]);
        }
    }
    for (int off = 16; off > 0; off >>= 1) {
        mn = fminf(mn, __shfl_xor_sync(URH_FULL_MASK, mn, off));
        mx = fmaxf(mx, __shfl_xor_sync(URH_FULL_MASK, mx, off));
    }
    if ((threadIdx.x & 31) == 0) { s_mn[threadIdx.x >> 5] = mn; s_mx[threadIdx.x >> 5] = mx; }
    __syncthreads();
    mn = INFINITY; mx = -INFINITY;
    for (int w = 0; w < URH_GUESS_THREADS / 32; w++) { mn = fminf(mn, s_mn[w]); mx = fmaxf(mx, s_mx[w]); }
    const float width = (mx - mn) / URH_GUESS_BINS;
    if (width > 0.0f) {
#pragma unroll
        for (int k = 0; k < PER; k++)
            if (!isnan(v[k])) atomicAdd(&s_hist[min((int)((v[k] - mn) / width), URH_GUESS_BINS - 1)], 1u);
    }
    __syncthreads();
    if (threadIdx.x != 0) return;
    *redone = 0u;
    if (!(mn <= mx)) { *d_tg = 0.0f; return; }
    if (!(width > 0.0f)) { *d_tg = mn; return; }
    constexpr int WINDOW = (int)(0.05 * URH_GUESS_BINS) + 1;
    int top[2] = {-1, -1};
    for (int b = 0; b < URH_GUESS_BINS; b++) {
        const unsigned int y = s_hist[b];
        bool peak = y > 0u;
        for (int d = 1; d < WINDOW && peak; d++)
            peak = y > (b + d < URH_GUESS_BINS ? s_hist[b + d] : 0u) && y > (b - d >= 0 ? s_hist[b - d] : 0u);
        if (!peak) continue;
        if (top[0] < 0 || y > s_hist[top[0]]) { top[1] = top[0]; top[0] = b; }
        else if (top[1] < 0 || y > s_hist[top[1]]) top[1] = b;
    }
    if (top[0] < 0) *d_tg = 0.5f * (mn + mx);
    else if (top[1] < 0) *d_tg = mn + ((float)top[0] + 0.5f) * width;
    else *d_tg = mn + (0.5f * (float)(top[0] + top[1]) + 0.5f) * width;
}


extern "C" int urh_get_center_thresholds(float center, float spacing, int modulation_order, float* h_out) {
    const int n = modulation_order / 2;
    for (int i = 0; i < n; i++) {
        volatile float t = (float)(n - (i + 1)) * spacing;
        h_out[i] = center - t;
    }
    for (int i = n; i < modulation_order - 1; i++) {
        volatile float t = (float)(i + 1 - n) * spacing;
        h_out[i] = center + t;
    }
    return URH_OK;
}

static int fill_classify(urh_ctx* ctx, UrhClassify* C, int mod_type, float center, uint8_t bits_per_symbol,
                         float spacing) {
    if (bits_per_symbol > 8) URH_FAIL(ctx, URH_ERR_INVALID, "bits_per_symbol %d > 8 not supported", (int)bits_per_symbol);
    memset(C, 0, sizeof(*C));
    C->noise_value = urh_noise_value(mod_type);
    C->order = 1 << bits_per_symbol;
    if (C->order > 1) urh_get_center_thresholds(center, spacing, C->order, C->thr);
    return URH_OK;
}

static int host_classify(float s, const UrhClassify& C) {
    int c = C.order - 1;
    for (int k = 0; k < C.order - 1; k++)
        if (s <= C.thr[k]) { c = k; break; }
    return c;
}

static float max_magnitude_for(int dtype) {
    switch (dtype) {
        case URH_DT_I8: return (float)sqrt(127.0 * 127.0 + 128.0 * 128.0);
        case URH_DT_U8: return (float)sqrt(255.0 * 255.0);
        case URH_DT_I16: return (float)sqrt(32768.0 * 32768.0 + 32767.0 * 32767.0);
        case URH_DT_U16: return (float)sqrt(65535.0 * 65535.0);
        default: return (float)sqrt(2.0);
    }
}

static bool iq_vec_aligned(const void* p, int dtype) { return ((uintptr_t)p % (2 * (size_t)urh_iq_bytes(dtype))) == 0; }

struct DensePass {
    float* qad = nullptr;
    const UrhDigitizer* dz = nullptr;
    int has_halo = 0;
    UrhTileStats* tile_stats = nullptr;
    int64_t tile_lo = 0, tile_hi = -1;
    UrhFine fine = {};
    UrhSpec* spec = nullptr;
};

template <int DT, int MOD, bool DIG>
static int launch_dense_iq_t(urh_ctx* ctx, const void* d_iq, int64_t n, const UrhDemodParams& dp, const UrhClassify& cls,
                             const DensePass& o) {
    static const UrhDigitizer none = {};
    const UrhDigitizer& dz = o.dz ? *o.dz : none;
    int16_t* init_cls = DIG ? dz.d_init : nullptr;
    const int cls_of_zero = DIG ? host_classify(0.0f, cls) : 0;
    const int64_t ntiles = urh_div_up(n, URH_TILE);
    const size_t fine_smem = o.fine.gh ? (size_t)URH_FINE_NB * sizeof(unsigned int) : 0;
    const int64_t tile_lo = o.tile_lo, tile_hi = (o.tile_hi < 0 || o.tile_hi > ntiles) ? ntiles : o.tile_hi;
    const int vec_in = iq_vec_aligned(d_iq, DT) ? 1 : 0;
    const int vec_out = (o.qad && ((uintptr_t)o.qad % 8) == 0) ? 1 : 0;
    const int threads = URH_WARPS_PER_BLOCK * 32;
    auto generic = [&](int64_t begin, int64_t end) -> int {
        begin = begin < tile_lo ? tile_lo : begin;
        end = end > tile_hi ? tile_hi : end;
        const int64_t count = end - begin;
        if (count <= 0) return URH_OK;
        URH_LAUNCH(ctx, (k_dense_iq<DT, MOD, DIG>), (unsigned)urh_div_up(count, URH_WARPS_PER_BLOCK), threads, fine_smem, d_iq, n, dp,
                   o.qad, vec_in, vec_out, cls, dz.tol, dz.tiles, dz.staging, dz.cap, init_cls, cls_of_zero, begin, count, o.has_halo,
                   o.tile_stats, o.fine);
        return URH_OK;
    };
    const int64_t nfull = n / URH_TILE;
    const bool fast = MOD == URH_MOD_FSK && vec_in && (!o.qad || vec_out) && (!DIG || cls.order == 2) && nfull > 1;
    URH_PROF_BEGIN(ctx);
    if (fast) {
        const int64_t fb = tile_lo > 1 ? tile_lo : 1, fe = tile_hi < nfull ? tile_hi : nfull;
        if (fe > fb) {
            const unsigned grid = (unsigned)urh_div_up(fe - fb, URH_WARPS_PER_BLOCK);
            bool speculated = false;
            if constexpr (DT == URH_DT_F32 && MOD == URH_MOD_FSK && !DIG) {
                if (o.spec && o.tile_stats && o.qad) {
                    URH_LAUNCH(ctx, (k_fsk_fifo<DT, true, true, true>), grid, threads, fine_smem, d_iq, n, dp, o.qad, 0.0f, dp.noise_value,
                               dz.tol, dz.tiles, dz.staging, dz.cap, fb, fe - fb, o.tile_stats, o.fine, (const float*)o.spec->tg, o.spec->margin);
                    o.spec->lo = fb;
                    o.spec->hi = fe;
                    speculated = true;
                }
            }
            if (speculated) {
            } else if (o.tile_stats && o.qad && !DIG) {
                URH_LAUNCH(ctx, (k_fsk_fifo<DT, false, true, true>), grid, threads, fine_smem, d_iq, n, dp, o.qad, cls.thr[0], cls.noise_value,
                           dz.tol, dz.tiles, dz.staging, dz.cap, fb, fe - fb, o.tile_stats, o.fine);
            } else if (o.qad) {
                URH_LAUNCH(ctx, (k_fsk_fifo<DT, DIG, true, false>), grid, threads, 0, d_iq, n, dp, o.qad, cls.thr[0], cls.noise_value, dz.tol,
                           dz.tiles, dz.staging, dz.cap, fb, fe - fb, nullptr, UrhFine{});
            } else {
                URH_LAUNCH(ctx, (k_fsk_fifo<DT, DIG, false, false>), grid, threads, 0, d_iq, n, dp, o.qad, cls.thr[0], cls.noise_value, dz.tol,
                           dz.tiles, dz.staging, dz.cap, fb, fe - fb, nullptr, UrhFine{});
            }
        }
        URH_CHECK(generic(0, 1));
        URH_CHECK(generic(nfull, ntiles));
    } else {
        URH_CHECK(generic(0, ntiles));
    }
    URH_PROF_END(ctx);
    return URH_OK;
}

template <int DT>
static int launch_dense_iq_dt(urh_ctx* ctx, int mod_type, const void* d_iq, int64_t n, const UrhDemodParams& dp, const UrhClassify& cls,
                              const DensePass& o) {
    const bool dig = o.dz && !o.spec;
    if (mod_type == URH_MOD_ASK)
        return dig ? launch_dense_iq_t<DT, URH_MOD_ASK, true>(ctx, d_iq, n, dp, cls, o) : launch_dense_iq_t<DT, URH_MOD_ASK, false>(ctx, d_iq, n, dp, cls, o);
    return dig ? launch_dense_iq_t<DT, URH_MOD_FSK, true>(ctx, d_iq, n, dp, cls, o) : launch_dense_iq_t<DT, URH_MOD_FSK, false>(ctx, d_iq, n, dp, cls, o);
}

static int launch_dense_iq(urh_ctx* ctx, int dtype, int mod_type, const void* d_iq, int64_t n, const UrhDemodParams& dp,
                           const UrhClassify& cls, const DensePass& o) {
    switch (dtype) {
        case URH_DT_I8: return launch_dense_iq_dt<URH_DT_I8>(ctx, mod_type, d_iq, n, dp, cls, o);
        case URH_DT_U8: return launch_dense_iq_dt<URH_DT_U8>(ctx, mod_type, d_iq, n, dp, cls, o);
        case URH_DT_I16: return launch_dense_iq_dt<URH_DT_I16>(ctx, mod_type, d_iq, n, dp, cls, o);
        case URH_DT_U16: return launch_dense_iq_dt<URH_DT_U16>(ctx, mod_type, d_iq, n, dp, cls, o);
        case URH_DT_F32: return launch_dense_iq_dt<URH_DT_F32>(ctx, mod_type, d_iq, n, dp, cls, o);
        default: URH_FAIL(ctx, URH_ERR_DTYPE, "Unsupported dtype");
    }
}

int urh_costas_demod(urh_ctx* ctx, const void* d_iq, int dtype, int64_t n, float noise_sqrd, int loop_order,
                     float bandwidth, float* d_out);

static UrhDemodParams make_demod_params(float noise_mag, int mod_type, int dtype) {
    UrhDemodParams dp;
    volatile float nm = noise_mag;
    volatile float sq = nm * nm;
    dp.noise_sqrd = sq;
    dp.noise_value = urh_noise_value(mod_type);
    dp.max_mag = max_magnitude_for(dtype);
    dp.one = 1.0f;
    dp.mone = -1.0f;
    return dp;
}

extern "C" int urh_afp_demod(urh_ctx* ctx, const void* d_iq, int dtype, int64_t n, float noise_mag, int mod_type,
                             int mod_order, float costas_loop_bandwidth, float* d_out) {
    if (n < 0) URH_FAIL(ctx, URH_ERR_INVALID, "negative length");
    if (urh_iq_bytes(dtype) == 0) URH_FAIL(ctx, URH_ERR_DTYPE, "Unsupported dtype");
    if (n == 0) return URH_OK;
    if (n <= 2 || (mod_type != URH_MOD_ASK && mod_type != URH_MOD_FSK && mod_type != URH_MOD_PSK)) {
        URH_CUDA(ctx, cudaMemsetAsync(d_out, 0, (size_t)n * sizeof(float), ctx->stream));
        if (n > 2) {
            const float nv = urh_noise_value(mod_type);
            URH_CUDA(ctx, cudaMemcpyAsync(d_out, &nv, sizeof(float), cudaMemcpyHostToDevice, ctx->stream));
            URH_CUDA(ctx, cudaStreamSynchronize(ctx->stream));
        }
        return URH_OK;
    }
    const UrhDemodParams dp = make_demod_params(noise_mag, mod_type, dtype);
    if (mod_type == URH_MOD_PSK) return urh_costas_demod(ctx, d_iq, dtype, n, dp.noise_sqrd, mod_order, costas_loop_bandwidth, d_out);
    UrhClassify cls;
    memset(&cls, 0, sizeof(cls));
    return launch_dense_iq(ctx, dtype, mod_type, d_iq, n, dp, cls, DensePass{d_out});
}

int urh_center_tiles_begin(urh_ctx* ctx, const float* d_x, const UrhTileStats* ts, int64_t n, int64_t* h_total);

extern "C" int urh_afp_demod_tiles(urh_ctx* ctx, const void* d_iq, int dtype, int64_t n, float noise_mag, int mod_type,
                                   float* d_qad_out, int halo, int64_t* h_kept) {
    if (n <= 2 || (mod_type != URH_MOD_ASK && mod_type != URH_MOD_FSK) || !d_qad_out)
        URH_FAIL(ctx, URH_ERR_INVALID, "urh_afp_demod_tiles: ASK/FSK, n > 2 and a qad buffer are required");
    if (urh_iq_bytes(dtype) == 0) URH_FAIL(ctx, URH_ERR_DTYPE, "Unsupported dtype");
    urh_arena_reset(ctx);
    const UrhDemodParams dp = make_demod_params(noise_mag, mod_type, dtype);
    UrhClassify cls;
    memset(&cls, 0, sizeof(cls));
    const int64_t ntiles = urh_div_up(n, URH_TILE);
    UrhTileStats* ts;
    URH_CHECK(urh_arena(ctx, (size_t)ntiles, &ts));
    URH_CHECK(launch_dense_iq(ctx, dtype, mod_type, d_iq, n, dp, cls, DensePass{d_qad_out, nullptr, halo, ts}));
    return urh_center_tiles_begin(ctx, d_qad_out, ts, n, h_kept);
}

static int pulses_begin(urh_ctx* ctx, int64_t* k, bool args_ok = true) {
    if (!k || !args_ok) return URH_ERR_INVALID;
    *k = 0;
    ctx->pulses_k = 0;
    return URH_OK;
}

static int launch_dense_qad(urh_ctx* ctx, const UrhDigitizer& dz, const float* x, int64_t s0, int64_t s1, const UrhClassify& cls,
                            const float* d_thr0 = nullptr, const UrhTileStats* ts = nullptr) {
    const int64_t n = s1 - s0;
    const unsigned grid = (unsigned)urh_div_up(urh_div_up(n, URH_TILE), URH_WARPS_PER_BLOCK);
    const int vec_in = (((uintptr_t)x % 8) == 0) ? 1 : 0;
    int16_t* init = s0 == 0 ? dz.d_init : nullptr;
    const int c0 = d_thr0 ? 0 : host_classify(0.0f, cls);
    if (ts) ts += s0 / URH_TILE;
    if (cls.order == 2)
        URH_LAUNCH(ctx, (k_dense_f32<SrcQad2, float>), grid, URH_WARPS_PER_BLOCK * 32, 0, x, n, vec_in, cls, dz.tol, dz.tiles, dz.staging,
                   dz.cap, init, c0, d_thr0, ts);
    else
        URH_LAUNCH(ctx, (k_dense_f32<SrcQad, float>), grid, URH_WARPS_PER_BLOCK * 32, 0, x, n, vec_in, cls, dz.tol, dz.tiles, dz.staging,
                   dz.cap, init, c0, d_thr0, ts);
    return URH_OK;
}

extern "C" int urh_grab_pulse_lens(urh_ctx* ctx, const float* d_qad, int64_t n, float center, uint16_t tolerance,
                                   int mod_type, uint32_t samples_per_symbol, uint8_t bits_per_symbol,
                                   float center_spacing, int64_t* k) {
    URH_CHECK(pulses_begin(ctx, k));
    if (n < 0) URH_FAIL(ctx, URH_ERR_INVALID, "negative length");
    if (n == 0) return URH_OK;
    urh_arena_reset(ctx);
    UrhClassify cls;
    URH_CHECK(fill_classify(ctx, &cls, mod_type, center, bits_per_symbol, center_spacing));
    UrhDigitizer dz;
    URH_CHECK(dz.init(ctx, n, tolerance, mod_type == URH_MOD_ASK, samples_per_symbol, urh_div_up(n, URH_TILE), false));
    URH_PROF_BEGIN(ctx);
    URH_CHECK(launch_dense_qad(ctx, dz, d_qad, 0, n, cls));
    URH_PROF_END(ctx);
    return finish_tiles(ctx, dz, FinishShard::local(dz), k);
}

extern "C" int urh_demod_digitize(urh_ctx* ctx, const void* d_iq, int dtype, int64_t n, float noise_mag,
                                  int mod_type, float center, uint16_t tolerance, uint32_t samples_per_symbol,
                                  uint8_t bits_per_symbol, float center_spacing, float* d_qad_out, int64_t* k) {
    URH_CHECK(pulses_begin(ctx, k));
    if (n < 0) URH_FAIL(ctx, URH_ERR_INVALID, "negative length");
    if (urh_iq_bytes(dtype) == 0) URH_FAIL(ctx, URH_ERR_DTYPE, "Unsupported dtype");
    if (n == 0) return URH_OK;
    if (n <= 2 || (mod_type != URH_MOD_ASK && mod_type != URH_MOD_FSK)) {
        float* q = d_qad_out;
        if (!q) URH_CUDA(ctx, cudaMalloc((void**)&q, (size_t)n * sizeof(float)));
        int rc = urh_afp_demod(ctx, d_iq, dtype, n, noise_mag, mod_type, 1 << bits_per_symbol, 0.1f, q);
        if (rc == URH_OK)
            rc = urh_grab_pulse_lens(ctx, q, n, center, tolerance, mod_type, samples_per_symbol, bits_per_symbol,
                                     center_spacing, k);
        if (!d_qad_out) {
            cudaStreamSynchronize(ctx->stream);
            cudaFree(q);
        }
        return rc;
    }
    urh_arena_reset(ctx);
    UrhClassify cls;
    URH_CHECK(fill_classify(ctx, &cls, mod_type, center, bits_per_symbol, center_spacing));
    const UrhDemodParams dp = make_demod_params(noise_mag, mod_type, dtype);
    UrhDigitizer dz;
    URH_CHECK(dz.init(ctx, n, tolerance, mod_type == URH_MOD_ASK, samples_per_symbol, urh_div_up(n, URH_TILE), false));
    URH_CHECK(launch_dense_iq(ctx, dtype, mod_type, d_iq, n, dp, cls, DensePass{d_qad_out, &dz}));
    return finish_tiles(ctx, dz, FinishShard::local(dz), k);
}

static int64_t rows_bound(int64_t n, int tol) { return n / (tol + 1) + 3; }

struct StreamSizes {
    int64_t cs;
    int64_t src_slot;
    int64_t qad_slot;
    int64_t ring_bytes;
    int64_t arena;
    int64_t scan_items;
    int64_t rows_chunk;
};
static int64_t scan_workspace_bytes(int64_t items) {
    const int64_t nb = 2 * (items / 256 + 1);
    return 256 + (nb > 8192 ? nb : 8192) * (4 + 2 * (int64_t)urhts::SLOT);
}
static int64_t finish_arena_bytes(int64_t tiles, int64_t rows_cap, bool ask) {
    return r256(tiles * (int64_t)sizeof(RunCarry)) + 2 * r256(tiles * 4) + 2 * r256(tiles * 8) + r256((32 + 8) * 8) +
           (ask ? r256(rows_cap * 16) : 0);
}
static int psk_order_of(int entry) { return (entry & URH_STREAM_PSK) ? ((entry & URH_STREAM_PSK4) ? 4 : 2) : 0; }
static int psk_entry_flags(int mod_order) { return URH_STREAM_PSK | (mod_order >= 4 ? URH_STREAM_PSK4 : 0); }

static StreamSizes stream_sizes(int64_t n, int dtype, int tol, int64_t chunk_samples, int ring, int entry) {
    StreamSizes z;
    const int kind = entry & 0xf;
    const int psk = psk_order_of(entry);
    const bool resident = entry & URH_STREAM_RESIDENT;
    const int64_t ntiles = urh_div_up(n, URH_TILE);
    z.cs = resident ? ntiles * URH_TILE : stream_chunk_samples(n, chunk_samples);
    const int64_t ct = z.cs / URH_TILE;
    const int64_t cap = stage_cap_for(tol);
    const bool iq = kind != URH_STREAM_ENTRY_GRAB_PULSE_LENS;
    const bool digitize = kind != URH_STREAM_ENTRY_AFP_DEMOD;
    z.rows_chunk = rows_bound(z.cs, tol);
    if (resident) {
        z.src_slot = iq ? n * urh_iq_bytes(dtype) : n * 4;
        z.qad_slot = (kind == URH_STREAM_ENTRY_GRAB_PULSE_LENS) ? 0 : n * 4;
        z.ring_bytes = r256(z.src_slot) + r256(z.qad_slot);
    } else {
        z.src_slot = (kind == URH_STREAM_ENTRY_GRAB_PULSE_LENS && (entry & URH_STREAM_QAD_ON_DEVICE)) ? 0
                     : URH_STREAM_PAD + z.cs * (iq ? urh_iq_bytes(dtype) : 4);
        const bool qad_ring = kind == URH_STREAM_ENTRY_AFP_DEMOD ||
                              (kind == URH_STREAM_ENTRY_DEMOD_DIGITIZE && ((entry & URH_STREAM_QAD_OUT) || psk));
        z.qad_slot = qad_ring ? z.cs * 4 : 0;
        z.ring_bytes = ring * (r256(z.src_slot) + r256(z.qad_slot));
        if (kind == URH_STREAM_ENTRY_DEMOD_CENTER_DIGITIZE) z.ring_bytes += r256(n * 4);
    }
    z.arena = 0;
    z.scan_items = ct > z.rows_chunk ? ct : z.rows_chunk;
    if (digitize) z.arena += r256(ct * (int64_t)sizeof(UrhTileSummary)) + r256(ct * cap * 4) + r256(16) + r256(sizeof(UrhChain)) +
                             finish_arena_bytes(ct, z.rows_chunk, true);
    if (psk && !resident) z.arena += urh_costas_arena_bytes(z.cs, psk) + r256(16) + r256(6 * 8);
    if (kind == URH_STREAM_ENTRY_DEMOD_CENTER_DIGITIZE) {
        z.arena += r256(ntiles * (int64_t)sizeof(UrhTileStats)) + r256((int64_t)URH_FINE_SLABS * URH_FINE_NB * 4) + r256((ntiles + 1) * 8) +
                   ((int64_t)2 << 20);
        if (ntiles > z.scan_items) z.scan_items = ntiles;
    }
    return z;
}

static int64_t segment_arena_bytes(int64_t tiles) {
    const int64_t cap = URH_TILE / 10 + 2, cand = tiles * URH_TILE / 10 + 3;
    return r256(tiles * (int64_t)sizeof(UrhTileSummary)) + r256(tiles * cap * 4) + 2 * r256(2 * (int64_t)sizeof(RunCarry)) +
           r256(tiles * 4) + r256(tiles * 8) + r256(32) + r256(cand * 8) + r256(cand * 2);
}
SegmentStreamSizes urh_segment_stream_sizes(int64_t n, int dtype, int64_t chunk_samples) {
    SegmentStreamSizes z;
    z.cs = stream_chunk_samples(n, chunk_samples);
    z.src_slot = r256(URH_STREAM_PAD + z.cs * urh_iq_bytes(dtype));
    z.mag_bytes = r256(z.cs * 8);
    z.arena = segment_arena_bytes(z.cs / URH_TILE);
    return z;
}

extern "C" int urh_stream_footprint(int64_t n, int dtype, int tolerance, int64_t chunk_samples, int ring, int entry, int64_t rows,
                                    int64_t* bytes) {
    if (!bytes || n < 0 || tolerance < 0 || tolerance > 0xffff || (entry & 0xf) > URH_STREAM_ENTRY_ESTIMATE) return URH_ERR_INVALID;
    if ((entry & 0xf) == URH_STREAM_ENTRY_SEGMENT_MESSAGES) {
        if (urh_iq_bytes(dtype) == 0) return URH_ERR_DTYPE;
        if (entry & URH_STREAM_RESIDENT) {
            const int64_t ntiles = urh_div_up(n, URH_TILE);
            *bytes = r256(n * urh_iq_bytes(dtype)) + r256(n * 8) + segment_arena_bytes(ntiles) + URH_ARENA_BLOCK + scan_workspace_bytes(ntiles);
            return URH_OK;
        }
        if (ring < 2 || ring > URH_STREAM_MAX_RING) return URH_ERR_INVALID;
        const SegmentStreamSizes z = urh_segment_stream_sizes(n, dtype, chunk_samples);
        *bytes = ring * z.src_slot + z.mag_bytes + stream_arena_bytes(z.arena) + scan_workspace_bytes(z.cs / URH_TILE);
        return URH_OK;
    }
    if ((entry & 0xf) == URH_STREAM_ENTRY_ESTIMATE) {
        if (!(entry & URH_STREAM_RESIDENT)) return URH_ERR_INVALID;
        if (urh_iq_bytes(dtype) == 0) return URH_ERR_DTYPE;
        int64_t demod = 0;
        URH_CHECK(urh_stream_footprint(n, dtype, 0, chunk_samples, ring, URH_STREAM_ENTRY_AFP_DEMOD | URH_STREAM_PSK | URH_STREAM_RESIDENT,
                                       -1, &demod));
        *bytes = r256(n * 8) + demod;
        return URH_OK;
    }
    if (!(entry & URH_STREAM_RESIDENT) && (ring < 2 || ring > URH_STREAM_MAX_RING)) return URH_ERR_INVALID;
    if ((entry & 0xf) != URH_STREAM_ENTRY_GRAB_PULSE_LENS && urh_iq_bytes(dtype) == 0) return URH_ERR_DTYPE;
    if ((entry & URH_STREAM_PSK) && (entry & 0xf) != URH_STREAM_ENTRY_AFP_DEMOD && (entry & 0xf) != URH_STREAM_ENTRY_DEMOD_DIGITIZE)
        return URH_ERR_INVALID;
    const StreamSizes z = stream_sizes(n, dtype, tolerance, chunk_samples, ring, entry);
    const bool digitize = (entry & 0xf) != URH_STREAM_ENTRY_AFP_DEMOD;
    const int64_t r = rows == -2 ? n / 64 + 1024 : (rows < 0 ? rows_bound(n, tolerance) : rows);
    if (entry & URH_STREAM_RESIDENT) {
        const int64_t ntiles = urh_div_up(n, URH_TILE);
        int64_t b = z.ring_bytes + URH_ARENA_BLOCK;
        if (digitize)
            b += r256(ntiles * (int64_t)sizeof(UrhTileSummary)) + r256(ntiles * (int64_t)stage_cap_for(tolerance) * 4) +
                 finish_arena_bytes(ntiles, r + r / 4, true) + 16 * (r + r / 4);
        if ((entry & 0xf) == URH_STREAM_ENTRY_DEMOD_CENTER_DIGITIZE)
            b += r256(ntiles * (int64_t)sizeof(UrhTileStats)) + r256((int64_t)URH_FINE_SLABS * URH_FINE_NB * 4) + r256((ntiles + 1) * 8);
        if (psk_order_of(entry)) b += urh_costas_arena_bytes(n, psk_order_of(entry));
        *bytes = b;
        return URH_OK;
    }
    int64_t b = z.ring_bytes + stream_arena_bytes(z.arena);
    b += scan_workspace_bytes(z.scan_items);
    if (digitize) b += 3 * 16 * (r + z.rows_chunk);
    *bytes = b;
    return URH_OK;
}

extern "C" int urh_stream_stats(urh_ctx* ctx, int64_t* h_out3) {
    h_out3[0] = ctx->stream_free_low;
    h_out3[1] = ctx->stream_chunks;
    h_out3[2] = (int64_t)ctx->arena_peak;
    return URH_OK;
}

struct StreamDigitizer {
    UrhDigitizer dz;
    UrhChain* chain;
    int64_t rows, rows_all;
    UrhArenaMark mark;
    int init(urh_ctx* ctx, int64_t n, int64_t cs, int tol, bool ask, uint32_t sps) {
        rows = 0;
        rows_all = rows_bound(n, tol);
        URH_CHECK(dz.init(ctx, n, tol, ask, sps, cs / URH_TILE, true));
        URH_CHECK(urh_arena(ctx, 1, &chain));
        mark = urh_arena_mark(ctx);
        return URH_OK;
    }
    int finish(urh_ctx* ctx, int64_t s0, int64_t s1) {
        const int64_t rc = rows_bound(s1 - s0, dz.tol);
        const int64_t need = rows + rc;
        if (need > (int64_t)ctx->pulses_cap_rows) {
            int64_t grow = 2 * (int64_t)ctx->pulses_cap_rows;
            if (grow > rows_all + rc) grow = rows_all + rc;
            URH_CHECK(urh_ensure_pulses_keep(ctx, (size_t)(grow > need ? grow : need), (size_t)rows));
        }
        urh_arena_release(ctx, mark);
        int64_t kc = 0;
        URH_CHECK(finish_tiles(ctx, dz, FinishShard::chunk(chain, s0, s1, dz.n, rows, rc), &kc));
        urh_stream_sample_free(ctx);
        rows += kc;
        return URH_OK;
    }
};

static int stream_check(urh_ctx* ctx, int64_t n, int ring, int mod_type, int dtype, bool iq);
static int psk_stream_check(urh_ctx* ctx, int64_t n, int ring, int dtype) {
    URH_CHECK(stream_check(ctx, n, ring, URH_MOD_PSK, dtype, false));
    if (n <= 2) URH_FAIL(ctx, URH_ERR_INVALID, "streamed PSK demodulation: n > 2");
    if (urh_iq_bytes(dtype) == 0) URH_FAIL(ctx, URH_ERR_DTYPE, "Unsupported dtype");
    return URH_OK;
}

static int stream_check(urh_ctx* ctx, int64_t n, int ring, int mod_type, int dtype, bool iq) {
    if (n <= 0) URH_FAIL(ctx, URH_ERR_INVALID, "streamed call: empty capture");
    if (ring < 2 || ring > URH_STREAM_MAX_RING) URH_FAIL(ctx, URH_ERR_INVALID, "streamed call: ring of %d slots (2..%d)", ring, URH_STREAM_MAX_RING);
    if (iq && (n <= 2 || (mod_type != URH_MOD_ASK && mod_type != URH_MOD_FSK)))
        URH_FAIL(ctx, URH_ERR_INVALID, "streamed demodulation: ASK/FSK and n > 2 (PSK is a serial recurrence)");
    if (iq && urh_iq_bytes(dtype) == 0) URH_FAIL(ctx, URH_ERR_DTYPE, "Unsupported dtype");
    return URH_OK;
}

static int stream_dense_iq(urh_ctx* ctx, int dtype, int mod_type, const char* slot, int64_t n, const UrhDemodParams& dp,
                           const UrhClassify& cls, const UrhWindow& w, DensePass o) {
    const void* iq = slot + URH_STREAM_PAD - w.k0 * urh_iq_bytes(dtype);
    o.tile_lo = w.k0 / URH_TILE;
    o.tile_hi = urh_div_up(w.k1, URH_TILE);
    UrhDigitizer view;
    if (o.dz) {
        view = *o.dz;
        view.tiles -= o.tile_lo;
        view.staging -= o.tile_lo * view.cap;
        o.dz = &view;
    }
    return launch_dense_iq(ctx, dtype, mod_type, iq, n, dp, cls, o);
}

struct CenterPlan;
int urh_center_chain(urh_ctx* ctx, const float* d_qad, int64_t n, const UrhTileStats* ts, int64_t max_size, int rank, int world,
                     const UrhFine* fine, CenterPlan** d_plan_out);
int urh_center_plan_result(urh_ctx* ctx, const CenterPlan* plan, const float** d_centerf, const double** d_center, const int** d_state);
int urh_center_plan_certify_stats(urh_ctx* ctx, const CenterPlan* plan, int64_t* h_dst3);

extern "C" int urh_shard_digitize(urh_ctx* ctx, const void* d_iq, int dtype, const float* d_qad_in, int64_t n, int has_halo,
                                  float noise_mag, int mod_type, float center, uint16_t tolerance, uint32_t samples_per_symbol,
                                  uint8_t bits_per_symbol, float center_spacing, float* d_qad_out, int64_t global_offset,
                                  int64_t n_total, int64_t* k) {
    URH_CHECK(pulses_begin(ctx, k));
    if (n <= 0) URH_FAIL(ctx, URH_ERR_INVALID, "empty shard");
    if (mod_type != URH_MOD_ASK && mod_type != URH_MOD_FSK) URH_FAIL(ctx, URH_ERR_INVALID, "sharded path: ASK / FSK only");
    if (!d_qad_in && urh_iq_bytes(dtype) == 0) URH_FAIL(ctx, URH_ERR_DTYPE, "Unsupported dtype");
    if (!ctx->nccl_comm) URH_FAIL(ctx, URH_ERR_INVALID, "NCCL communicator not initialised (urh_nccl_init)");
    urh_arena_reset(ctx);
    UrhClassify cls;
    URH_CHECK(fill_classify(ctx, &cls, mod_type, center, bits_per_symbol, center_spacing));
    UrhDigitizer dz;
    URH_CHECK(dz.init(ctx, n, tolerance, mod_type == URH_MOD_ASK, samples_per_symbol, urh_div_up(n, URH_TILE), true));
    if (d_qad_in) {
        URH_PROF_BEGIN(ctx);
        URH_CHECK(launch_dense_qad(ctx, dz, d_qad_in, 0, n, cls));
        URH_PROF_END(ctx);
    } else {
        const UrhDemodParams dp = make_demod_params(noise_mag, mod_type, dtype);
        URH_CHECK(launch_dense_iq(ctx, dtype, mod_type, d_iq, n, dp, cls, DensePass{d_qad_out, &dz, has_halo}));
    }
    return finish_tiles(ctx, dz, FinishShard::shard(ctx, dz, global_offset, n_total), k);
}

struct CenterMail {
    double center;
    int state, pad;
    int64_t cert[3];
    int64_t kept;
    unsigned int redone;
};
static_assert(40 * sizeof(int64_t) + sizeof(CenterMail) <= 64 * sizeof(int64_t), "CenterMail outgrows the mailbox");

struct StreamCenter {
    int ring;
    int64_t chunk_samples;
    const void* h_iq;
    float* h_qad;
    int64_t* kept;
};

struct CenterStep {
    const void* d_iq;
    int dtype, mod_type, has_halo;
    int64_t n, ntiles;
    float* d_qad;
    UrhDemodParams dp;
    UrhClassify cls;
    UrhTileStats* ts;
    UrhFine fine;
    bool speculate;
    UrhSpec spec;
    UrhDigitizer dz;
};

static int center_setup(urh_ctx* ctx, CenterStep& S, bool certify, bool tables, const char* forced_guess, int tol, uint32_t sps) {
    URH_CHECK(urh_arena(ctx, (size_t)S.ntiles, &S.ts));
    if (certify) {
        S.fine.slab_tiles = urh_div_up(S.ntiles, URH_FINE_SLABS);
        if (S.fine.slab_tiles < URH_WARPS_PER_BLOCK) S.fine.slab_tiles = URH_WARPS_PER_BLOCK;
        const int64_t nslabs = urh_div_up(S.ntiles, S.fine.slab_tiles);
        URH_CHECK(urh_arena(ctx, (size_t)(nslabs * URH_FINE_NB), &S.fine.gh));
        URH_CUDA(ctx, cudaMemsetAsync(S.fine.gh, 0, (size_t)(nslabs * URH_FINE_NB) * sizeof(unsigned int), ctx->stream));
        S.fine.scale = (S.mod_type == URH_MOD_FSK) ? 512.0f : 4096.0f;
        S.fine.off = (S.mod_type == URH_MOD_FSK) ? 2048.0f : 0.0f;
    }
    S.cls.noise_value = urh_noise_value(S.mod_type);
    S.cls.order = 2;
    if (tables) URH_CHECK(S.dz.init(ctx, S.n, tol, S.mod_type == URH_MOD_ASK, sps, S.ntiles, false));
    if (S.speculate) {
        float* tg;
        URH_CHECK(urh_arena(ctx, 1, &tg));
        URH_CHECK(urh_arena(ctx, 1, &S.spec.redone));
        URH_CHECK(urh_arena(ctx, (size_t)S.ntiles, &S.spec.margin));
        S.spec.tg = tg;
        URH_LAUNCH(ctx, k_speculate_guess, 1, URH_GUESS_THREADS, 0, (const float2*)S.d_iq, S.n, S.dp.noise_sqrd, forced_guess ? 1 : 0,
                   forced_guess ? strtof(forced_guess, nullptr) : 0.0f, tg, S.spec.redone);
    }
    return URH_OK;
}

static int center_demod(urh_ctx* ctx, CenterStep& S, int64_t t0, int64_t t1) {
    DensePass o{S.d_qad, nullptr, S.has_halo, S.ts, t0, t1, S.fine};
    if (S.speculate) {
        o.dz = &S.dz;
        o.spec = &S.spec;
    }
    return launch_dense_iq(ctx, S.dtype, S.mod_type, S.d_iq, S.n, S.dp, S.cls, o);
}

static int center_demod_host(urh_ctx* ctx, CenterStep& S, const void* h_iq, int64_t chunk_samples) {
    const int64_t chunk_tiles = chunk_samples >= URH_TILE ? chunk_samples / URH_TILE : 1;
    const size_t sample_bytes = (size_t)urh_iq_bytes(S.dtype);
    int chunk_no = 0;
    for (int64_t t0 = 0; t0 < S.ntiles; t0 += chunk_tiles, chunk_no++) {
        const int64_t t1 = (t0 + chunk_tiles < S.ntiles) ? t0 + chunk_tiles : S.ntiles;
        const int64_t s0 = t0 * URH_TILE, s1 = (t1 * URH_TILE < S.n) ? t1 * URH_TILE : S.n;
        cudaEvent_t ev = ctx->ev_copy[chunk_no & 1];
        URH_CUDA(ctx, cudaMemcpyAsync((char*)S.d_iq + (size_t)s0 * sample_bytes, (const char*)h_iq + (size_t)s0 * sample_bytes,
                                      (size_t)(s1 - s0) * sample_bytes, cudaMemcpyHostToDevice, ctx->copy_stream[0]));
        URH_CUDA(ctx, cudaEventRecord(ev, ctx->copy_stream[0]));
        URH_CUDA(ctx, cudaStreamWaitEvent(ctx->stream, ev, 0));
        URH_CHECK(center_demod(ctx, S, t0, t1));
    }
    return URH_OK;
}

static int center_demod_ring(urh_ctx* ctx, CenterStep& S, const StreamCenter& sc, int tol, StreamRing& R, int64_t* cs) {
    const StreamSizes z = stream_sizes(S.n, S.dtype, tol, sc.chunk_samples, sc.ring, URH_STREAM_ENTRY_DEMOD_CENTER_DIGITIZE);
    *cs = z.cs;
    const int64_t slot = r256(z.src_slot);
    URH_CHECK(R.init(ctx, sc.ring, sc.ring * slot));
    std::vector<UrhWindow> win;
    URH_CHECK(urh_filter_windows(URH_FILTER_TILES, S.n, S.n, 1, 0, sc.chunk_samples, nullptr, nullptr, 0, win));
    return stream_run(ctx, win, R, (const char*)sc.h_iq, urh_iq_bytes(S.dtype), R.mem, slot, sc.h_qad != nullptr,
                      [&](int64_t, const UrhWindow& w, int s) {
                          return stream_dense_iq(ctx, S.dtype, S.mod_type, R.mem + s * slot, S.n, S.dp, S.cls, w,
                                                 DensePass{S.d_qad, nullptr, 0, S.ts, 0, -1, S.fine});
                      },
                      [&](int64_t, const UrhWindow& w, int, cudaStream_t cp) {
                          URH_CUDA(ctx, cudaMemcpyAsync(sc.h_qad + w.k0, S.d_qad + w.k0, (size_t)(w.k1 - w.k0) * sizeof(float),
                                                        cudaMemcpyDeviceToHost, cp));
                          return URH_OK;
                      },
                      place_after_pad, true);
}

static int center_copy_results(urh_ctx* ctx, const CenterPlan* plan, CenterMail* mail) {
    const double* d_center;
    const int* d_state;
    urh_center_plan_result(ctx, plan, nullptr, &d_center, &d_state);
    URH_CUDA(ctx, cudaMemcpyAsync(&mail->center, d_center, sizeof(double), cudaMemcpyDeviceToHost, ctx->stream));
    URH_CUDA(ctx, cudaMemcpyAsync(&mail->state, d_state, sizeof(int), cudaMemcpyDeviceToHost, ctx->stream));
    return urh_center_plan_certify_stats(ctx, plan, mail->cert);
}

static int center_digitize_resident(urh_ctx* ctx, CenterStep& S, const CenterPlan* plan, const FinishShard& sh, CenterMail* mail,
                                    int64_t* rows) {
    const float* d_centerf;
    urh_center_plan_result(ctx, plan, &d_centerf, nullptr, nullptr);
    URH_CUDA(ctx, cudaMemsetAsync(S.dz.d_init, 0, 16, ctx->stream));
    const int vec_in = (((uintptr_t)S.d_qad % 8) == 0) ? 1 : 0;
    int64_t grid = urh_div_up(S.ntiles, URH_WARPS_PER_BLOCK);
    if (S.speculate) {
        int per_sm = 0;
        URH_CUDA(ctx, cudaOccupancyMaxActiveBlocksPerMultiprocessor(&per_sm, k_dense_f32<SrcQad2, float>, URH_WARPS_PER_BLOCK * 32, 0));
        const int64_t resident = (int64_t)ctx->sm_count * (per_sm > 0 ? per_sm : 1);
        if (grid > resident) grid = resident;
    }
    URH_LAUNCH(ctx, (k_dense_f32<SrcQad2, float>), (unsigned)grid, URH_WARPS_PER_BLOCK * 32, 0, (const float*)S.d_qad, S.n, vec_in, S.cls,
               S.dz.tol, S.dz.tiles, S.dz.staging, S.dz.cap, S.dz.d_init, 0, d_centerf, (const UrhTileStats*)S.ts, S.spec);
    URH_CHECK(center_copy_results(ctx, plan, mail));
    mail->redone = 0u;
    if (S.speculate) URH_CUDA(ctx, cudaMemcpyAsync(&mail->redone, S.spec.redone, sizeof(unsigned int), cudaMemcpyDeviceToHost, ctx->stream));
    return finish_tiles(ctx, S.dz, sh, rows);
}

static int center_digitize_chunked(urh_ctx* ctx, CenterStep& S, const CenterPlan* plan, int64_t cs, int tol, uint32_t sps,
                                   CenterMail* mail, int64_t* rows) {
    URH_CHECK(center_copy_results(ctx, plan, mail));
    URH_CUDA(ctx, cudaMemcpyAsync(&mail->kept, (const int64_t*)ctx->center_prefix + S.ntiles, sizeof(int64_t), cudaMemcpyDeviceToHost,
                                  ctx->stream));
    URH_CUDA(ctx, cudaStreamSynchronize(ctx->stream));
    if (mail->state != 1) return URH_OK;
    const float* d_centerf;
    urh_center_plan_result(ctx, plan, &d_centerf, nullptr, nullptr);
    StreamDigitizer sd;
    URH_CHECK(sd.init(ctx, S.n, cs, tol, S.mod_type == URH_MOD_ASK, sps));
    for (int64_t s0 = 0; s0 < S.n; s0 += cs) {
        const int64_t s1 = s0 + cs < S.n ? s0 + cs : S.n;
        URH_CHECK(launch_dense_qad(ctx, sd.dz, S.d_qad + s0, s0, s1, S.cls, d_centerf, S.ts));
        URH_CHECK(sd.finish(ctx, s0, s1));
    }
    *rows = sd.rows;
    return URH_OK;
}

static int demod_center_digitize_impl(urh_ctx* ctx, const void* d_iq, int dtype, int64_t n, int has_halo, float noise_mag, int mod_type,
                                      uint16_t tolerance, uint32_t samples_per_symbol, int64_t max_size, float* d_qad_out, bool sharded,
                                      int64_t global_offset, int64_t n_total, double* center, int* center_state, int64_t* k,
                                      const void* h_iq = nullptr, int64_t chunk_samples = 0, const StreamCenter* sc = nullptr) {
    URH_CHECK(pulses_begin(ctx, k, center && center_state));
    *center = 0.0;
    *center_state = 0;
    if (n <= 2 || (mod_type != URH_MOD_ASK && mod_type != URH_MOD_FSK) || !d_qad_out)
        URH_FAIL(ctx, URH_ERR_INVALID, "demod_center_digitize: ASK/FSK, n > 2 and a qad buffer are required");
    if (urh_iq_bytes(dtype) == 0) URH_FAIL(ctx, URH_ERR_DTYPE, "Unsupported dtype");
    if (sharded && !ctx->nccl_comm) URH_FAIL(ctx, URH_ERR_INVALID, "NCCL communicator not initialised (urh_nccl_init)");
    const bool no_certify = getenv("URH_B200_CENTER_NO_CERTIFY") != nullptr, no_speculate = getenv("URH_B200_NO_SPECULATE") != nullptr;
    const char* forced_guess = getenv("URH_B200_SPECULATE_GUESS");
    urh_arena_reset(ctx);
    URH_TL_RESET(ctx);
    URH_TL_MARK(ctx, "step start");
    CenterStep S = {};
    S.d_iq = d_iq; S.dtype = dtype; S.mod_type = mod_type; S.has_halo = has_halo;
    S.n = n; S.ntiles = urh_div_up(n, URH_TILE);
    S.d_qad = d_qad_out;
    S.dp = make_demod_params(noise_mag, mod_type, dtype);
    S.speculate = !sharded && !h_iq && !sc && mod_type == URH_MOD_FSK && dtype == URH_DT_F32 && !no_speculate;
    URH_CHECK(center_setup(ctx, S, !sharded && !no_certify, !sc, forced_guess, tolerance, samples_per_symbol));

    StreamRing ring;
    int64_t cs = 0;
    if (sc) URH_CHECK(center_demod_ring(ctx, S, *sc, tolerance, ring, &cs));
    else if (h_iq) URH_CHECK(center_demod_host(ctx, S, h_iq, chunk_samples));
    else URH_CHECK(center_demod(ctx, S, 0, S.ntiles));

    CenterPlan* plan = nullptr;
    URH_CHECK(urh_center_chain(ctx, d_qad_out, n, S.ts, max_size, sharded ? ctx->nccl_rank : 0, sharded ? ctx->nccl_world : 1,
                               S.fine.gh ? &S.fine : nullptr, &plan));

    CenterMail* mail = (CenterMail*)(ctx->h_mail + 40);
    int64_t rows = 0;
    if (sc)
        URH_CHECK(center_digitize_chunked(ctx, S, plan, cs, tolerance, samples_per_symbol, mail, &rows));
    else
        URH_CHECK(center_digitize_resident(ctx, S, plan, sharded ? FinishShard::shard(ctx, S.dz, global_offset, n_total) : FinishShard::local(S.dz),
                                           mail, &rows));

    *center = mail->center;
    *center_state = mail->state;
    if (sc) *sc->kept = mail->kept;
    ctx->center_cert[0] = mail->cert[0];
    ctx->center_cert[1] = S.fine.gh ? URH_FINE_NB : 0;
    ctx->center_cert[2] = mail->cert[2];
    const int64_t redone = (S.spec.hi > S.spec.lo) ? mail->redone : 0;
    ctx->spec_stats[0] = S.spec.hi - S.spec.lo;
    ctx->spec_stats[1] = S.spec.hi - S.spec.lo - redone;
    ctx->spec_stats[2] = redone;
    if (mail->state != 1) {
        ctx->pulses_k = 0;
        rows = 0;
    }
    *k = rows;
    return URH_OK;
}

extern "C" int urh_speculate_stats(urh_ctx* ctx, int64_t* h_out3) {
    for (int i = 0; i < 3; i++) h_out3[i] = ctx->spec_stats[i];
    return URH_OK;
}

extern "C" int urh_demod_center_digitize(urh_ctx* ctx, const void* d_iq, int dtype, int64_t n, float noise_mag, int mod_type,
                                         uint16_t tolerance, uint32_t samples_per_symbol, int64_t max_size, float* d_qad_out,
                                         double* center, int* center_state, int64_t* k) {
    return demod_center_digitize_impl(ctx, d_iq, dtype, n, 0, noise_mag, mod_type, tolerance, samples_per_symbol, max_size, d_qad_out, false,
                                      0, n, center, center_state, k);
}

extern "C" int urh_demod_center_digitize_host(urh_ctx* ctx, const void* h_iq, int dtype, int64_t n, float noise_mag, int mod_type,
                                              uint16_t tolerance, uint32_t samples_per_symbol, int64_t max_size, int64_t chunk_samples,
                                              void* d_iq_scratch, float* d_qad_out, double* center, int* center_state, int64_t* k) {
    if (!h_iq || !d_iq_scratch) return URH_ERR_INVALID;
    URH_CUDA(ctx, cudaEventRecord(ctx->ev_comp[0], ctx->stream));
    URH_CUDA(ctx, cudaStreamWaitEvent(ctx->copy_stream[0], ctx->ev_comp[0], 0));
    return demod_center_digitize_impl(ctx, d_iq_scratch, dtype, n, 0, noise_mag, mod_type, tolerance, samples_per_symbol, max_size, d_qad_out,
                                      false, 0, n, center, center_state, k, h_iq, chunk_samples > 0 ? chunk_samples : ((int64_t)1 << 24));
}

extern "C" int urh_shard_demod_center_digitize_host(urh_ctx* ctx, const void* h_iq, int dtype, int64_t n, int has_halo, float noise_mag,
                                                    int mod_type, uint16_t tolerance, uint32_t samples_per_symbol, int64_t max_size,
                                                    int64_t chunk_samples, void* d_iq_scratch, float* d_qad_out, int64_t global_offset,
                                                    int64_t n_total, double* center, int* center_state, int64_t* k) {
    if (!h_iq || !d_iq_scratch) return URH_ERR_INVALID;
    URH_CUDA(ctx, cudaEventRecord(ctx->ev_comp[0], ctx->stream));
    URH_CUDA(ctx, cudaStreamWaitEvent(ctx->copy_stream[0], ctx->ev_comp[0], 0));
    return demod_center_digitize_impl(ctx, d_iq_scratch, dtype, n, has_halo, noise_mag, mod_type, tolerance, samples_per_symbol, max_size,
                                      d_qad_out, true, global_offset, n_total, center, center_state, k, h_iq,
                                      chunk_samples > 0 ? chunk_samples : ((int64_t)1 << 24));
}

extern "C" int urh_shard_demod_center_digitize(urh_ctx* ctx, const void* d_iq, int dtype, int64_t n, int has_halo, float noise_mag,
                                               int mod_type, uint16_t tolerance, uint32_t samples_per_symbol, int64_t max_size,
                                               float* d_qad_out, int64_t global_offset, int64_t n_total, double* center,
                                               int* center_state, int64_t* k) {
    return demod_center_digitize_impl(ctx, d_iq, dtype, n, has_halo, noise_mag, mod_type, tolerance, samples_per_symbol, max_size, d_qad_out,
                                      true, global_offset, n_total, center, center_state, k);
}

extern "C" int urh_afp_demod_stream(urh_ctx* ctx, const void* h_iq, int dtype, int64_t n, float noise_mag, int mod_type, int64_t chunk_samples,
                                    int ring, float* h_qad) {
    if (!h_iq || !h_qad) return URH_ERR_INVALID;
    URH_CHECK(stream_check(ctx, n, ring, mod_type, dtype, true));
    urh_arena_reset(ctx);
    const StreamSizes z = stream_sizes(n, dtype, 0, chunk_samples, ring, URH_STREAM_ENTRY_AFP_DEMOD);
    StreamRing R;
    URH_CHECK(R.init(ctx, ring, z.ring_bytes));
    char* d_src = R.mem;
    float* d_qad = (float*)(R.mem + ring * r256(z.src_slot));
    const UrhDemodParams dp = make_demod_params(noise_mag, mod_type, dtype);
    UrhClassify cls;
    memset(&cls, 0, sizeof(cls));
    std::vector<UrhWindow> win;
    URH_CHECK(urh_filter_windows(URH_FILTER_TILES, n, n, 1, 0, chunk_samples, nullptr, nullptr, 0, win));
    return stream_run(ctx, win, R, (const char*)h_iq, urh_iq_bytes(dtype), d_src, r256(z.src_slot), true,
                      [&](int64_t, const UrhWindow& w, int s) {
                          return stream_dense_iq(ctx, dtype, mod_type, d_src + s * r256(z.src_slot), n, dp, cls, w,
                                                 DensePass{d_qad + s * z.cs - w.k0});
                      },
                      contiguous_download(ctx, (const char*)d_qad, z.cs * 4, (char*)h_qad, 4), place_after_pad);
}

extern "C" int urh_grab_pulse_lens_stream(urh_ctx* ctx, const float* qad, int qad_on_device, int64_t n, float center, uint16_t tolerance,
                                          int mod_type, uint32_t samples_per_symbol, uint8_t bits_per_symbol, float center_spacing,
                                          int64_t chunk_samples, int ring, int64_t* k) {
    URH_CHECK(pulses_begin(ctx, k, qad != nullptr));
    URH_CHECK(stream_check(ctx, n, ring, mod_type, 0, false));
    urh_arena_reset(ctx);
    UrhClassify cls;
    URH_CHECK(fill_classify(ctx, &cls, mod_type, center, bits_per_symbol, center_spacing));
    const StreamSizes z = stream_sizes(n, 0, tolerance, chunk_samples, ring,
                                       URH_STREAM_ENTRY_GRAB_PULSE_LENS | (qad_on_device ? URH_STREAM_QAD_ON_DEVICE : 0));
    StreamRing R;
    URH_CHECK(R.init(ctx, ring, z.ring_bytes));
    StreamDigitizer sd;
    URH_CHECK(sd.init(ctx, n, z.cs, tolerance, mod_type == URH_MOD_ASK, samples_per_symbol));
    char* d_src = R.mem;
    std::vector<UrhWindow> win;
    URH_CHECK(urh_filter_windows(URH_FILTER_TILES, n, n, 0, 0, chunk_samples, nullptr, nullptr, 0, win));
    URH_CHECK(stream_run(ctx, win, R, qad_on_device ? nullptr : (const char*)qad, 4, d_src, r256(z.src_slot), false,
                         [&](int64_t, const UrhWindow& w, int s) {
                             const float* x = qad_on_device ? qad + w.k0 : (const float*)(d_src + s * r256(z.src_slot) + URH_STREAM_PAD);
                             URH_CHECK(launch_dense_qad(ctx, sd.dz, x, w.k0, w.k1, cls));
                             return sd.finish(ctx, w.k0, w.k1);
                         },
                         no_download, place_after_pad));
    *k = sd.rows;
    return URH_OK;
}

extern "C" int urh_demod_digitize_stream(urh_ctx* ctx, const void* h_iq, int dtype, int64_t n, float noise_mag, int mod_type, float center,
                                         uint16_t tolerance, uint32_t samples_per_symbol, uint8_t bits_per_symbol, float center_spacing,
                                         int64_t chunk_samples, int ring, float* h_qad_out, int64_t* k) {
    URH_CHECK(pulses_begin(ctx, k, h_iq != nullptr));
    URH_CHECK(stream_check(ctx, n, ring, mod_type, dtype, true));
    urh_arena_reset(ctx);
    UrhClassify cls;
    URH_CHECK(fill_classify(ctx, &cls, mod_type, center, bits_per_symbol, center_spacing));
    const UrhDemodParams dp = make_demod_params(noise_mag, mod_type, dtype);
    const StreamSizes z = stream_sizes(n, dtype, tolerance, chunk_samples, ring,
                                       URH_STREAM_ENTRY_DEMOD_DIGITIZE | (h_qad_out ? URH_STREAM_QAD_OUT : 0));
    StreamRing R;
    URH_CHECK(R.init(ctx, ring, z.ring_bytes));
    StreamDigitizer sd;
    URH_CHECK(sd.init(ctx, n, z.cs, tolerance, mod_type == URH_MOD_ASK, samples_per_symbol));
    char* d_src = R.mem;
    float* d_qad = h_qad_out ? (float*)(R.mem + ring * r256(z.src_slot)) : nullptr;
    std::vector<UrhWindow> win;
    URH_CHECK(urh_filter_windows(URH_FILTER_TILES, n, n, 1, 0, chunk_samples, nullptr, nullptr, 0, win));
    URH_CHECK(stream_run(ctx, win, R, (const char*)h_iq, urh_iq_bytes(dtype), d_src, r256(z.src_slot), h_qad_out != nullptr,
                         [&](int64_t, const UrhWindow& w, int s) {
                             URH_CHECK(stream_dense_iq(ctx, dtype, mod_type, d_src + s * r256(z.src_slot), n, dp, cls, w,
                                                       DensePass{d_qad ? d_qad + s * z.cs - w.k0 : nullptr, &sd.dz}));
                             return sd.finish(ctx, w.k0, w.k1);
                         },
                         contiguous_download(ctx, (const char*)d_qad, z.cs * 4, (char*)h_qad_out, 4), place_after_pad));
    *k = sd.rows;
    return URH_OK;
}

extern "C" int urh_demod_center_digitize_stream(urh_ctx* ctx, const void* h_iq, int dtype, int64_t n, float noise_mag, int mod_type,
                                                uint16_t tolerance, uint32_t samples_per_symbol, int64_t max_size, int64_t chunk_samples,
                                                int ring, float* d_qad_out, float* h_qad_out, double* center, int* center_state,
                                                int64_t* kept, int64_t* k) {
    if (!h_iq || !d_qad_out || !kept) return URH_ERR_INVALID;
    URH_CHECK(stream_check(ctx, n, ring, mod_type, dtype, true));
    StreamCenter sc;
    sc.ring = ring; sc.chunk_samples = chunk_samples; sc.h_iq = h_iq; sc.h_qad = h_qad_out; sc.kept = kept;
    return demod_center_digitize_impl(ctx, nullptr, dtype, n, 0, noise_mag, mod_type, tolerance, samples_per_symbol, max_size, d_qad_out,
                                      false, 0, n, center, center_state, k, nullptr, 0, &sc);
}

extern "C" int urh_afp_demod_psk_stream(urh_ctx* ctx, const void* h_iq, int dtype, int64_t n, float noise_mag, int mod_order,
                                        float costas_loop_bandwidth, int64_t chunk_samples, int ring, float* h_qad) {
    if (!h_iq || !h_qad) return URH_ERR_INVALID;
    URH_CHECK(psk_stream_check(ctx, n, ring, dtype));
    urh_arena_reset(ctx);
    const StreamSizes z = stream_sizes(n, dtype, 0, chunk_samples, ring, URH_STREAM_ENTRY_AFP_DEMOD | psk_entry_flags(mod_order));
    StreamRing R;
    URH_CHECK(R.init(ctx, ring, z.ring_bytes));
    const int64_t slot = r256(z.src_slot);
    char* d_src = R.mem;
    float* d_qad = (float*)(R.mem + ring * slot);
    const UrhDemodParams dp = make_demod_params(noise_mag, URH_MOD_PSK, dtype);
    UrhCostasStream cs;
    URH_CHECK(urh_costas_stream_begin(ctx, &cs));
    const UrhArenaMark mark = urh_arena_mark(ctx);
    std::vector<UrhWindow> win;
    URH_CHECK(urh_filter_windows(URH_FILTER_TILES, n, n, 0, 0, chunk_samples, nullptr, nullptr, 0, win));
    URH_CHECK(stream_run(ctx, win, R, (const char*)h_iq, urh_iq_bytes(dtype), d_src, slot, true,
                         [&](int64_t c, const UrhWindow& w, int s) {
                             urh_arena_release(ctx, mark);
                             return urh_costas_stream_chunk(ctx, &cs, c, d_src + s * slot + URH_STREAM_PAD, dtype, w.k1 - w.k0, dp.noise_sqrd,
                                                            mod_order, costas_loop_bandwidth, d_qad + s * z.cs);
                         },
                         contiguous_download(ctx, (const char*)d_qad, z.cs * 4, (char*)h_qad, 4), place_after_pad));
    return urh_costas_stream_end(ctx, &cs);
}

extern "C" int urh_demod_digitize_psk_stream(urh_ctx* ctx, const void* h_iq, int dtype, int64_t n, float noise_mag, float center,
                                             uint16_t tolerance, uint32_t samples_per_symbol, uint8_t bits_per_symbol, float center_spacing,
                                             int64_t chunk_samples, int ring, float* h_qad_out, int64_t* k) {
    URH_CHECK(pulses_begin(ctx, k, h_iq != nullptr));
    URH_CHECK(psk_stream_check(ctx, n, ring, dtype));
    urh_arena_reset(ctx);
    UrhClassify cls;
    URH_CHECK(fill_classify(ctx, &cls, URH_MOD_PSK, center, bits_per_symbol, center_spacing));
    const int mod_order = 1 << bits_per_symbol;
    const UrhDemodParams dp = make_demod_params(noise_mag, URH_MOD_PSK, dtype);
    const StreamSizes z = stream_sizes(n, dtype, tolerance, chunk_samples, ring,
                                       URH_STREAM_ENTRY_DEMOD_DIGITIZE | (h_qad_out ? URH_STREAM_QAD_OUT : 0) | psk_entry_flags(mod_order));
    StreamRing R;
    URH_CHECK(R.init(ctx, ring, z.ring_bytes));
    const int64_t slot = r256(z.src_slot);
    char* d_src = R.mem;
    float* d_qad = (float*)(R.mem + ring * slot);
    UrhCostasStream cs;
    URH_CHECK(urh_costas_stream_begin(ctx, &cs));
    StreamDigitizer sd;
    URH_CHECK(sd.init(ctx, n, z.cs, tolerance, false, samples_per_symbol));
    std::vector<UrhWindow> win;
    URH_CHECK(urh_filter_windows(URH_FILTER_TILES, n, n, 0, 0, chunk_samples, nullptr, nullptr, 0, win));
    URH_CHECK(stream_run(ctx, win, R, (const char*)h_iq, urh_iq_bytes(dtype), d_src, slot, h_qad_out != nullptr,
                         [&](int64_t c, const UrhWindow& w, int s) {
                             urh_arena_release(ctx, sd.mark);
                             float* q = d_qad + s * z.cs;
                             URH_CHECK(urh_costas_stream_chunk(ctx, &cs, c, d_src + s * slot + URH_STREAM_PAD, dtype, w.k1 - w.k0, dp.noise_sqrd,
                                                               mod_order, 0.1f, q));
                             URH_CHECK(launch_dense_qad(ctx, sd.dz, q, w.k0, w.k1, cls));
                             return sd.finish(ctx, w.k0, w.k1);
                         },
                         contiguous_download(ctx, (const char*)d_qad, z.cs * 4, (char*)h_qad_out, 4), place_after_pad));
    *k = sd.rows;
    return urh_costas_stream_end(ctx, &cs);
}

struct UrhShardState {
    UrhCandidates cand;
};
static UrhShardState* shard_state(urh_ctx* ctx) {
    if (!ctx->shard_state) ctx->shard_state = calloc(1, sizeof(UrhShardState));
    return (UrhShardState*)ctx->shard_state;
}

extern "C" int urh_shard_candidates(urh_ctx* ctx, int carry_valid, int carry_cls, int64_t carry_len, int64_t global_offset,
                                    int64_t* count, const int64_t** d_pos, const int16_t** d_cls, int* last_cand_cls) {
    if (!ctx->shard_tiles) URH_FAIL(ctx, URH_ERR_INVALID, "urh_segment_shard_pass must precede urh_shard_candidates");
    UrhShardCarry in;
    in.valid = carry_valid; in.cls = carry_cls; in.len = carry_len;
    UrhShardState* S = shard_state(ctx);
    URH_CHECK(urh_collect_candidates_shard(ctx, ctx->shard_n, ctx->shard_tol, (const UrhTileSummary*)ctx->shard_tiles,
                                           (const uint32_t*)ctx->shard_staging, ctx->shard_cap, in, global_offset, &S->cand));
    *count = S->cand.count;
    if (d_pos) *d_pos = S->cand.pos;
    if (d_cls) *d_cls = S->cand.cls;
    if (last_cand_cls) {
        *last_cand_cls = 0;
        if (S->cand.count > 0) {
            int16_t v = 0;
            URH_CUDA(ctx, cudaMemcpyAsync(&v, S->cand.cls + S->cand.count - 1, sizeof(v), cudaMemcpyDeviceToHost, ctx->stream));
            URH_CUDA(ctx, cudaStreamSynchronize(ctx->stream));
            *last_cand_cls = v;
        }
    }
    ctx->shard_tiles = nullptr;
    return URH_OK;
}

extern "C" int urh_fetch_candidates(urh_ctx* ctx, int64_t* h_pos, int16_t* h_cls, int64_t count) {
    UrhShardState* S = shard_state(ctx);
    if (count < 0 || count > S->cand.count) URH_FAIL(ctx, URH_ERR_INVALID, "fetch_candidates: count exceeds the table");
    if (count == 0) return URH_OK;
    URH_CUDA(ctx, cudaMemcpyAsync(h_pos, S->cand.pos, (size_t)count * sizeof(int64_t), cudaMemcpyDeviceToHost, ctx->stream));
    URH_CUDA(ctx, cudaMemcpyAsync(h_cls, S->cand.cls, (size_t)count * sizeof(int16_t), cudaMemcpyDeviceToHost, ctx->stream));
    URH_CUDA(ctx, cudaStreamSynchronize(ctx->stream));
    return URH_OK;
}

extern "C" int urh_fetch_pulses(urh_ctx* ctx, int64_t* h_rows, int64_t k) {
    if (k < 0 || k > ctx->pulses_k) URH_FAIL(ctx, URH_ERR_INVALID, "fetch_pulses: k=%lld exceeds last result %lld", (long long)k, (long long)ctx->pulses_k);
    if (k == 0) return URH_OK;
    URH_CUDA(ctx, cudaMemcpyAsync(h_rows, ctx->pulses, (size_t)k * 2 * sizeof(int64_t), cudaMemcpyDeviceToHost, ctx->stream));
    URH_CUDA(ctx, cudaStreamSynchronize(ctx->stream));
    return URH_OK;
}

extern "C" int urh_pulses_device_ptr(urh_ctx* ctx, const int64_t** d_rows, int64_t* k) {
    if (d_rows) *d_rows = ctx->pulses;
    if (k) *k = ctx->pulses_k;
    return URH_OK;
}


__global__ void k_selftest_div(uint64_t seed, int64_t count, unsigned long long* mismatches, unsigned long long* tested) {
    const int64_t stride = (int64_t)gridDim.x * blockDim.x;
    unsigned long long bad = 0, ok = 0;
    for (int64_t i = (int64_t)blockIdx.x * blockDim.x + threadIdx.x; i < count; i += stride) {
        uint64_t h = seed + (uint64_t)i * 0x9E3779B97F4A7C15ull;
        h = (h ^ (h >> 30)) * 0xBF58476D1CE4E5B9ull;
        h = (h ^ (h >> 27)) * 0x94D049BB133111EBull;
        h ^= h >> 31;
        uint64_t g = h * 0xD6E8FEB86659FD93ull + 0x632BE59BD9B4E019ull;
        g ^= g >> 29;
        const uint32_t span = URH_DIVWIN_HI - URH_DIVWIN_LO;
        uint32_t ea = URH_DIVWIN_LO + (uint32_t)((h >> 40) % span), eb = URH_DIVWIN_LO + (uint32_t)((g >> 40) % span);
        uint32_t ma = (uint32_t)h & 0x7fffff, mb = (uint32_t)g & 0x7fffff;
        if ((i & 15) == 1) ma = 0;
        if ((i & 15) == 2) mb = 0;
        if ((i & 15) == 3) { ma = 0x7fffff; }
        if ((i & 15) == 4) { mb = 0x7fffff; }
        if ((i & 15) == 5) { eb = ea; }
        float a0 = __uint_as_float((ea << 23) | ma), b0 = __uint_as_float((eb << 23) | mb);
        float a1 = __uint_as_float(((URH_DIVWIN_LO + (uint32_t)((g >> 12) % span)) << 23) | ((uint32_t)(h >> 9) & 0x7fffff));
        float b1 = __uint_as_float(((URH_DIVWIN_LO + (uint32_t)((h >> 12) % span)) << 23) | ((uint32_t)(g >> 9) & 0x7fffff));
        if ((i & 15) == 6) { a1 = __uint_as_float((URH_DIVWIN_LO << 23)); b1 = __uint_as_float(((URH_DIVWIN_HI - 1) << 23) | 0x7fffff); }
        if ((i & 15) == 8) { b1 = __uint_as_float((URH_DIVWIN_LO << 23)); a1 = __uint_as_float(((URH_DIVWIN_HI - 1) << 23) | 0x7fffff); }
        if ((i & 63) == 7) a1 = 0.0f;
        const float2 q = urh_div2_window(make_float2(a0, a1), make_float2(b0, b1));
        const float r0 = __fdiv_rn(a0, b0), r1 = __fdiv_rn(a1, b1);
        bad += (__float_as_uint(q.x) != __float_as_uint(r0)) + (__float_as_uint(q.y) != __float_as_uint(r1));
        ok += 2;
    }
    atomicAdd(mismatches, bad);
    atomicAdd(tested, ok);
}

extern "C" int urh_selftest_packed_div(urh_ctx* ctx, uint64_t seed, int64_t count, int64_t* mismatches, int64_t* tested) {
    urh_arena_reset(ctx);
    unsigned long long* d;
    URH_CHECK(urh_arena(ctx, 2, &d));
    URH_CUDA(ctx, cudaMemsetAsync(d, 0, 16, ctx->stream));
    URH_LAUNCH(ctx, k_selftest_div, (unsigned)(ctx->sm_count * 8), 256, 0, seed, count, d, d + 1);
    int64_t h[2];
    URH_CHECK(urh_read_i64(ctx, (const int64_t*)d, 2, h));
    *mismatches = h[0];
    *tested = h[1];
    return URH_OK;
}
```

urh_b200/csrc/finish.cu:

```cuda
#include "sparse.cuh"
#include "tilescan.cuh"

#include <limits.h>

#define CLS_NONE INT_MIN

struct __align__(16) CandAgg {
    int64_t cnt;
    int32_t last_cls;
    int32_t pad;
};
struct CandOp {
    __device__ __forceinline__ CandAgg operator()(const CandAgg& a, const CandAgg& b) const {
        CandAgg r;
        r.cnt = a.cnt + b.cnt;
        r.last_cls = (b.last_cls != CLS_NONE) ? b.last_cls : a.last_cls;
        r.pad = 0;
        return r;
    }
};
struct __align__(16) FireAgg {
    int64_t fired;
    int64_t last_pos;
};
struct FireOp {
    __device__ __forceinline__ FireAgg operator()(const FireAgg& a, const FireAgg& b) const {
        FireAgg r;
        r.fired = a.fired + b.fired;
        r.last_pos = (b.last_pos >= 0) ? b.last_pos : a.last_pos;
        return r;
    }
};

struct ScanRunCarry : TileRuns {
    RunCarry* carry;
    __device__ __forceinline__ void post(int64_t t, const RunCarry& excl, const RunCarry&) const { carry[t] = excl; }
};

struct __align__(16) TileFire {
    int32_t first_cls;
    int32_t first_rel;
    int32_t fired;
    int32_t last_rel;
};
struct ScanCandidates {
    const UrhTileSummary* tiles;
    const uint32_t* staging;
    int stage_cap;
    const RunCarry* carry;
    const RunCarry* xcarry;
    int tol;
    int32_t* head_rel;
    int32_t* prev_cls;
    TileFire* fire;
    __device__ __forceinline__ CandAgg load(int64_t t) const {
        const UrhTileSummary s = tiles[t];
        RunCarry c = carry[t];
        if (xcarry) c = RunCarryOp()(*xcarry, c);
        int64_t start_len = 0;
        if (!(c.flags & 2) && c.cls == s.first_cls) start_len = c.len;
        int32_t rel = -1;
        if (start_len <= tol && (int64_t)tol < start_len + s.head_len) rel = (int32_t)(tol - start_len);
        head_rel[t] = rel;
        TileFire f;
        f.first_cls = CLS_NONE; f.first_rel = -1; f.fired = 0; f.last_rel = -1;
        int prev = CLS_NONE;
        if (rel >= 0) {
            prev = s.first_cls;
            f.first_cls = prev;
            f.first_rel = rel;
        }
        const uint32_t* st = staging + t * (int64_t)stage_cap;
        for (int j = 0; j < s.ncand; j += 4) {
            uint32_t w[4];
#pragma unroll
            for (int u = 0; u < 4; u++) w[u] = (j + u < s.ncand) ? st[j + u] : 0u;
#pragma unroll
            for (int u = 0; u < 4; u++) {
                if (j + u < s.ncand) {
                    const int cl = (int)(w[u] & 0xffffu) - 1;
                    const int p = (int)(w[u] >> 16);
                    if (prev == CLS_NONE) {
                        f.first_cls = cl;
                        f.first_rel = p;
                    } else if (cl != prev) {
                        f.fired++;
                        f.last_rel = p;
                    }
                    prev = cl;
                }
            }
        }
        fire[t] = f;
        CandAgg r;
        r.cnt = (int64_t)s.ncand + (rel >= 0 ? 1 : 0);
        r.last_cls = prev;
        r.pad = 0;
        return r;
    }
    __device__ __forceinline__ void post(int64_t t, const CandAgg& excl, const CandAgg&) const { prev_cls[t] = excl.last_cls; }
};

struct ScanFirings {
    const TileFire* fire;
    const int32_t* prev_cls;
    const int16_t* d_prev0;
    int64_t global_offset;
    int64_t* row_off;
    int64_t* prev_fired;
    __device__ __forceinline__ FireAgg load(int64_t t) const {
        const TileFire f = fire[t];
        int prev = prev_cls[t];
        if (prev == CLS_NONE) prev = *d_prev0;
        FireAgg r;
        r.fired = f.fired;
        int32_t last = f.last_rel;
        if (f.first_cls != CLS_NONE && f.first_cls != prev) {
            r.fired++;
            if (last < 0) last = f.first_rel;
        }
        r.last_pos = (last >= 0) ? t * URH_TILE + global_offset + last : -1;
        return r;
    }
    __device__ __forceinline__ void post(int64_t t, const FireAgg& excl, const FireAgg&) const {
        row_off[t] = excl.fired;
        prev_fired[t] = excl.last_pos;
    }
};

constexpr int FIN_TILES = 32;
constexpr int FIN_BATCH = 8;

struct FinRows {
    int64_t* out;
    int64_t cap_rows;
    int tol;
    int is_ask;
    int64_t sps;
};

struct FinWalk {
    int prev;
    int64_t pp;
    int64_t idx;
};

__device__ __forceinline__ void fin_row(const FinRows& R, int64_t idx, int64_t p, int64_t pp, int prev) {
    const int64_t rec = (pp >= 0) ? (p - pp) : (p + 1 - R.tol);
    int64_t st = prev;
    if (R.is_ask && st == -1 && rec < R.sps) st = 0;
    if (idx < R.cap_rows) *((longlong2*)R.out + idx) = make_longlong2(st, rec);
}

__device__ __forceinline__ void fin_chunk(FinWalk& W, uint32_t w, int cnt, int lane, int64_t base, const FinRows& R) {
    const int c = (int)(w & 0xffffu) - 1;
    const int rel = (int)(w >> 16);
    int pc = __shfl_up_sync(URH_FULL_MASK, c, 1);
    if (lane == 0) pc = W.prev;
    const bool fire = lane < cnt && c != pc;
    const unsigned fm = __ballot_sync(URH_FULL_MASK, fire);
    const unsigned lower = fm & ((1u << lane) - 1u);
    const int before = __shfl_sync(URH_FULL_MASK, rel, lower ? 31 - __clz(lower) : 0);
    if (fire) fin_row(R, W.idx + __popc(lower), base + rel, lower ? base + before : W.pp, pc);
    if (fm) W.pp = base + __shfl_sync(URH_FULL_MASK, rel, 31 - __clz(fm));
    W.idx += __popc(fm);
    if (cnt > 0) W.prev = __shfl_sync(URH_FULL_MASK, c, cnt - 1);
}

__global__ void __launch_bounds__(256) k_finish_rows(const UrhTileSummary* __restrict__ tiles, const uint32_t* __restrict__ staging,
                                                    int stage_cap, const int32_t* __restrict__ head_rel, const int32_t* __restrict__ prev_cls,
                                                    const int16_t* __restrict__ d_prev0, const int64_t* __restrict__ row_off,
                                                    const int64_t* __restrict__ prev_fired, const int64_t* __restrict__ d_xprev_fired,
                                                    int64_t ntiles, int64_t global_offset, int64_t n_total, int tol, int is_ask, int64_t sps,
                                                    int emit_tail, int64_t row_base, int64_t* __restrict__ out, int64_t cap_rows,
                                                    int64_t* __restrict__ d_out) {
    const int64_t t0 = ((int64_t)blockIdx.x * blockDim.x + threadIdx.x) / 32 * FIN_TILES;
    if (t0 >= ntiles) return;
    const int lane = threadIdx.x & 31;
    FinRows R;
    R.out = out; R.cap_rows = cap_rows; R.tol = tol; R.is_ask = is_ask; R.sps = sps;
    const int64_t tl = t0 + lane;
    int l_first = 0, l_ncand = 0, l_rel = -1, l_prev = 0;
    int64_t l_idx = 0, l_pp = -1;
    if (tl < ntiles) {
        const UrhTileSummary s = tiles[tl];
        l_first = s.first_cls;
        l_ncand = s.ncand;
        l_rel = head_rel[tl];
        l_prev = prev_cls[tl];
        if (l_prev == CLS_NONE) l_prev = *d_prev0;
        l_idx = row_off[tl];
        l_pp = prev_fired[tl];
        if (l_pp < 0) l_pp = *d_xprev_fired;
    }
    for (int j0 = 0; j0 < FIN_TILES && t0 + j0 < ntiles; j0 += FIN_BATCH) {
        uint32_t w0[FIN_BATCH];
#pragma unroll
        for (int u = 0; u < FIN_BATCH; u++) {
            const int nc = __shfl_sync(URH_FULL_MASK, l_ncand, j0 + u);
            w0[u] = (lane < nc) ? __ldg(staging + (t0 + j0 + u) * (int64_t)stage_cap + lane) : 0u;
        }
#pragma unroll
        for (int u = 0; u < FIN_BATCH; u++) {
            const int j = j0 + u;
            const int64_t t = t0 + j;
            if (t >= ntiles) break;
            const int64_t base = t * URH_TILE + global_offset;
            const int ncand = __shfl_sync(URH_FULL_MASK, l_ncand, j);
            const int rel = __shfl_sync(URH_FULL_MASK, l_rel, j);
            FinWalk W;
            W.prev = __shfl_sync(URH_FULL_MASK, l_prev, j);
            W.pp = __shfl_sync(URH_FULL_MASK, l_pp, j);
            W.idx = __shfl_sync(URH_FULL_MASK, l_idx, j);
            if (rel >= 0) {
                const int c = __shfl_sync(URH_FULL_MASK, l_first, j);
                if (c != W.prev) {
                    if (lane == 0) fin_row(R, W.idx, base + rel, W.pp, W.prev);
                    W.idx++;
                    W.pp = base + rel;
                }
                W.prev = c;
            }
            const uint32_t* st = staging + t * (int64_t)stage_cap;
            for (int k = 0; k < ncand; k += 32) {
                const uint32_t w = (k == 0) ? w0[u] : ((k + lane < ncand) ? __ldg(st + k + lane) : 0u);
                fin_chunk(W, w, min(32, ncand - k), lane, base, R);
            }
            if (t == ntiles - 1 && lane == 0) {
                int64_t idx = W.idx;
                const int64_t fired = idx;
                if (emit_tail && (is_ask || row_base + fired < n_total)) {
                    if (idx < cap_rows) *((longlong2*)out + idx) = make_longlong2(W.prev, (W.pp >= 0) ? (n_total - 1 - W.pp) : (n_total - tol));
                    idx++;
                }
                d_out[0] = idx;
                d_out[1] = fired;
            }
        }
    }
}

struct ScanMergeRows {
    const int64_t* raw;
    int64_t rows;
    int64_t n_total;
    int has_tail;
    int64_t* out;
    int64_t* d_k;
    const int64_t* prev_last;
    int64_t row_base;
    __device__ __forceinline__ int64_t load(int64_t r) const {
        if (r == 0) return (prev_last && raw[0] == *prev_last) ? 0 : 1;
        return raw[2 * r] != raw[2 * r - 2] ? 1 : 0;
    }
    __device__ __forceinline__ void post(int64_t r, const int64_t& excl, const int64_t& head) const {
        const bool is_tail = has_tail && r == rows - 1;
        if (is_tail && row_base + excl >= n_total) {
            *d_k = excl;
            return;
        }
        const int64_t o = excl + head - 1;
        if (head) out[2 * o] = raw[2 * r];
        atomicAdd((unsigned long long*)&out[2 * o + 1], (unsigned long long)raw[2 * r + 1]);
        if (r == rows - 1) *d_k = o + 1;
    }
};
struct AddI64 {
    __device__ __forceinline__ int64_t operator()(int64_t a, int64_t b) const { return a + b; }
};

__global__ void k_pack_stage1(const int16_t* __restrict__ d_init, const RunCarry* __restrict__ total, int64_t* __restrict__ msg) {
    memcpy(msg, total, sizeof(RunCarry));
    msg[2] = *d_init;
    msg[3] = 0;
}
__global__ void k_fold_carry(const int64_t* __restrict__ all, int rank, RunCarry* __restrict__ xcarry) {
    RunCarry acc;
    acc.len = 0; acc.cls = 0; acc.flags = 2 | 1;
    for (int q = 0; q < rank; q++) {
        RunCarry c;
        memcpy(&c, all + 4 * q, sizeof(c));
        acc = RunCarryOp()(acc, c);
    }
    if (rank == 0) acc.flags = 2;
    else acc.flags &= ~1;
    *xcarry = acc;
}
__global__ void k_fold_prev_cls(const int64_t* __restrict__ all, int rank, const int64_t* __restrict__ stage1, int16_t* __restrict__ prev0) {
    int v = (int)stage1[2];
    for (int q = 0; q < rank; q++) {
        CandAgg c;
        memcpy(&c, all + 2 * q, sizeof(c));
        if (c.last_cls != CLS_NONE) v = c.last_cls;
    }
    *prev0 = (int16_t)v;
}
__global__ void k_fold_prev_fired(const int64_t* __restrict__ all, int rank, int64_t* __restrict__ xprev) {
    int64_t v = -1;
    for (int q = 0; q < rank; q++) {
        FireAgg c;
        memcpy(&c, all + 2 * q, sizeof(c));
        if (c.last_pos >= 0) v = c.last_pos;
    }
    *xprev = v;
}

__global__ void k_chain_start(const int16_t* __restrict__ d_init, UrhChain* __restrict__ chain) {
    chain->run.len = 0; chain->run.cls = 0; chain->run.flags = 2 | 1;
    chain->prev_fired = -1;
    chain->last_state = INT64_MIN;
    chain->prev_cls = *d_init;
}
__global__ void k_chain_advance(UrhChain* __restrict__ chain, const RunCarry* __restrict__ tot_run, const CandAgg* __restrict__ tot_cand,
                                const FireAgg* __restrict__ tot_fire) {
    chain->run = RunCarryOp()(chain->run, *tot_run);
    if (tot_cand->last_cls != CLS_NONE) chain->prev_cls = (int16_t)tot_cand->last_cls;
    if (tot_fire->last_pos >= 0) chain->prev_fired = tot_fire->last_pos;
}
__global__ void k_chain_last_row(UrhChain* __restrict__ chain, const int64_t* __restrict__ table, int64_t rows) {
    if (rows > 0) chain->last_state = table[2 * (rows - 1)];
}

int finish_tiles(urh_ctx* ctx, const UrhDigitizer& dz, const FinishShard& sh, int64_t* k) {
    const int64_t n = sh.n;
    const int64_t ntiles = urh_div_up(n, URH_TILE);
    const bool sharded = sh.world > 1;
    UrhChain* chain = sh.chain;
    RunCarry* carry;
    int32_t *head_rel, *prev_cls;
    int64_t *row_off, *prev_fired, *d_small;
    URH_CHECK(urh_arena(ctx, (size_t)ntiles, &carry));
    URH_CHECK(urh_arena(ctx, (size_t)ntiles, &head_rel));
    URH_CHECK(urh_arena(ctx, (size_t)ntiles, &prev_cls));
    URH_CHECK(urh_arena(ctx, (size_t)ntiles, &row_off));
    URH_CHECK(urh_arena(ctx, (size_t)ntiles, &prev_fired));
    TileFire* fire;
    URH_CHECK(urh_arena(ctx, (size_t)ntiles, &fire));
    URH_CHECK(urh_arena(ctx, (size_t)(32 + 8 * (sharded ? sh.world : 0)), &d_small));
    URH_CUDA(ctx, cudaMemsetAsync(d_small, 0xff, 4 * sizeof(int64_t), ctx->stream));
    RunCarry* d_tot_run = (RunCarry*)(d_small + 4);
    CandAgg* d_tot_cand = (CandAgg*)(d_small + 6);
    FireAgg* d_tot_fire = (FireAgg*)(d_small + 8);
    RunCarry* d_xcarry = (RunCarry*)(d_small + 10);
    int16_t* d_prev0 = (int16_t*)(d_small + 12);
    int64_t* d_xprev = d_small + 13;
    int64_t* d_msg1 = d_small + 16;
    int64_t* d_all1 = d_small + 32;
    int64_t* d_all2 = d_all1 + 4 * (sharded ? sh.world : 0);
    int64_t* d_all3 = d_all2 + 2 * (sharded ? sh.world : 0);

    if (chain && sh.global_offset == 0) URH_LAUNCH(ctx, k_chain_start, 1, 1, 0, dz.d_init, chain);
    RunCarry rc_ident;
    rc_ident.len = 0; rc_ident.cls = 0; rc_ident.flags = 2 | 1;
    ScanRunCarry fa;
    fa.tiles = dz.tiles; fa.n = n; fa.carry = carry;
    URH_CHECK((urhts::scan<RunCarry, RunCarryOp, ScanRunCarry>(ctx, ntiles, rc_ident, RunCarryOp(), fa, d_tot_run)));
    if (sharded) {
        URH_LAUNCH(ctx, k_pack_stage1, 1, 1, 0, dz.d_init, (const RunCarry*)d_tot_run, d_msg1);
        URH_TL_MARK(ctx, "x4 run carry: enter");
        URH_CHECK(urh_nccl_allgather(ctx, d_msg1, d_all1, 4 * sizeof(int64_t)));
        URH_TL_MARK(ctx, "x4 run carry: done");
        URH_LAUNCH(ctx, k_fold_carry, 1, 1, 0, (const int64_t*)d_all1, sh.rank, d_xcarry);
    }
    ScanCandidates fb;
    fb.tiles = dz.tiles; fb.staging = dz.staging; fb.stage_cap = dz.cap; fb.carry = carry;
    fb.xcarry = sharded ? d_xcarry : (chain ? &chain->run : nullptr);
    fb.tol = dz.tol; fb.head_rel = head_rel; fb.prev_cls = prev_cls; fb.fire = fire;
    CandAgg ca_ident;
    ca_ident.cnt = 0; ca_ident.last_cls = CLS_NONE; ca_ident.pad = 0;
    URH_CHECK((urhts::scan<CandAgg, CandOp, ScanCandidates, 4>(ctx, ntiles, ca_ident, CandOp(), fb, d_tot_cand)));
    const int16_t* prev0 = chain ? &chain->prev_cls : dz.d_init;
    if (sharded) {
        URH_TL_MARK(ctx, "x5 candidates: enter");
        URH_CHECK(urh_nccl_allgather(ctx, d_tot_cand, d_all2, sizeof(CandAgg)));
        URH_TL_MARK(ctx, "x5 candidates: done");
        URH_LAUNCH(ctx, k_fold_prev_cls, 1, 1, 0, (const int64_t*)d_all2, sh.rank, (const int64_t*)d_all1, d_prev0);
        prev0 = d_prev0;
    }
    ScanFirings fc;
    fc.fire = fire; fc.prev_cls = prev_cls; fc.d_prev0 = prev0; fc.global_offset = sh.global_offset; fc.row_off = row_off;
    fc.prev_fired = prev_fired;
    FireAgg fi_ident;
    fi_ident.fired = 0; fi_ident.last_pos = -1;
    URH_CHECK((urhts::scan<FireAgg, FireOp, ScanFirings>(ctx, ntiles, fi_ident, FireOp(), fc, d_tot_fire)));
    const int64_t* xprev = chain ? &chain->prev_fired : d_small + 2;
    if (sharded) {
        URH_TL_MARK(ctx, "x6 firings: enter");
        URH_CHECK(urh_nccl_allgather(ctx, d_tot_fire, d_all3, sizeof(FireAgg)));
        URH_TL_MARK(ctx, "x6 firings: done");
        URH_LAUNCH(ctx, k_fold_prev_fired, 1, 1, 0, (const int64_t*)d_all3, sh.rank, d_xprev);
        xprev = d_xprev;
    }

    int64_t cap_rows = (int64_t)ctx->pulses_cap_rows;
    const int64_t guess = n / 64 + 1024;
    if (!chain && cap_rows < guess) {
        URH_CHECK(urh_ensure_pulses(ctx, (size_t)guess));
        cap_rows = (int64_t)ctx->pulses_cap_rows;
    }
    const int64_t row_base = chain ? sh.row_base : 0;
    int64_t* raw = ctx->pulses + 2 * row_base;
    int64_t raw_cap = chain ? sh.rows_cap : cap_rows;
    if (dz.is_ask) URH_CHECK(urh_arena(ctx, (size_t)raw_cap * 2, &raw));
    int64_t got[2] = {0, 0};
    for (int attempt = 0; attempt < 2; attempt++) {
        URH_LAUNCH(ctx, k_finish_rows, (unsigned)urh_div_up(ntiles, 8 * FIN_TILES), 256, 0, dz.tiles, dz.staging, dz.cap, (const int32_t*)head_rel,
                   (const int32_t*)prev_cls, prev0, (const int64_t*)row_off, (const int64_t*)prev_fired, xprev, ntiles, sh.global_offset,
                   sh.n_total, dz.tol, dz.is_ask ? 1 : 0, (int64_t)dz.sps, sh.emit_tail, row_base, raw, raw_cap, d_small);
        if (sharded && attempt == 0) URH_TL_MARK(ctx, "rows written");
        URH_CHECK(urh_read_i64(ctx, d_small, 2, got));
        if (got[0] <= raw_cap) break;
        if (attempt == 1 || chain) URH_FAIL(ctx, URH_ERR_CUDA, "finish_tiles: row buffer overflow after regrowth");
        if (dz.is_ask) {
            URH_CHECK(urh_arena(ctx, (size_t)got[0] * 2, &raw));
            raw_cap = got[0];
        } else {
            URH_CHECK(urh_ensure_pulses(ctx, (size_t)got[0]));
            raw = ctx->pulses;
            raw_cap = (int64_t)ctx->pulses_cap_rows;
        }
    }
    if (chain) URH_LAUNCH(ctx, k_chain_advance, 1, 1, 0, chain, (const RunCarry*)d_tot_run, (const CandAgg*)d_tot_cand, (const FireAgg*)d_tot_fire);
    int64_t K = got[0];
    if (dz.is_ask && K > 0) {
        if (!chain) URH_CHECK(urh_ensure_pulses(ctx, (size_t)K));
        int64_t* out = ctx->pulses + 2 * row_base;
        URH_CUDA(ctx, cudaMemsetAsync(out, 0, (size_t)K * 2 * sizeof(int64_t), ctx->stream));
        ScanMergeRows fm;
        fm.raw = raw; fm.rows = K; fm.n_total = sh.n_total; fm.has_tail = (sh.emit_tail && K > got[1]) ? 1 : 0; fm.out = out;
        fm.d_k = d_small;
        fm.prev_last = (chain && row_base > 0) ? &chain->last_state : nullptr;
        fm.row_base = row_base;
        URH_CHECK((urhts::scan<int64_t, AddI64, ScanMergeRows>(ctx, K, (int64_t)0, AddI64(), fm, (int64_t*)nullptr)));
        URH_CHECK(urh_read_i64(ctx, d_small, 1, &K));
        if (chain) URH_LAUNCH(ctx, k_chain_last_row, 1, 1, 0, chain, (const int64_t*)ctx->pulses, row_base + K);
    }
    ctx->pulses_k = row_base + K;
    *k = K;
    return URH_OK;
}
```

urh_b200/csrc/sparse.cuh:

```cuda
#pragma once
#include "dense.cuh"

struct __align__(16) RunCarry {
    int64_t len;
    int32_t cls;
    int32_t flags;
};
struct RunCarryOp {
    __device__ __forceinline__ RunCarry operator()(const RunCarry& a, const RunCarry& b) const {
        if (b.flags & 2) return a;
        if (a.flags & 2) return b;
        RunCarry r;
        if ((b.flags & 1) && b.cls == a.cls) {
            r.len = a.len + b.len;
            r.cls = a.cls;
            r.flags = a.flags & 1;
        } else {
            r.len = b.len;
            r.cls = b.cls;
            r.flags = 0;
        }
        return r;
    }
};

struct TileRuns {
    const UrhTileSummary* tiles;
    int64_t n;
    __device__ __forceinline__ RunCarry load(int64_t t) const {
        const int64_t rem = n - t * URH_TILE;
        const int tile_len = rem < URH_TILE ? (int)rem : URH_TILE;
        const UrhTileSummary s = tiles[t];
        RunCarry r;
        r.len = s.tail_len;
        r.cls = s.last_cls;
        r.flags = (s.head_len == tile_len) ? 1 : 0;
        return r;
    }
};

struct __align__(16) UrhChain {
    RunCarry run;
    int64_t prev_fired;
    int64_t last_state;
    int16_t prev_cls;
    int16_t pad[7];
};

static inline int stage_cap_for(int tol) { return URH_TILE / (tol + 1) + 2; }

struct UrhDigitizer {
    int64_t n;
    int tol, cap;
    bool is_ask;
    uint32_t sps;
    UrhTileSummary* tiles;
    uint32_t* staging;
    int16_t* d_init;
    int init(urh_ctx* ctx, int64_t n_, int tol_, bool ask, uint32_t sps_, int64_t ntiles, bool zero_init) {
        n = n_; tol = tol_; cap = stage_cap_for(tol); is_ask = ask; sps = sps_;
        URH_CHECK(urh_arena(ctx, (size_t)ntiles, &tiles));
        URH_CHECK(urh_arena(ctx, (size_t)ntiles * cap, &staging));
        URH_CHECK(urh_arena(ctx, 8, &d_init));
        if (zero_init) URH_CUDA(ctx, cudaMemsetAsync(d_init, 0, 16, ctx->stream));
        return URH_OK;
    }
};

struct FinishShard {
    int64_t n;
    int rank, world;
    int64_t global_offset;
    int64_t n_total;
    int emit_tail;
    UrhChain* chain;
    int64_t row_base, rows_cap;

    static FinishShard local(const UrhDigitizer& dz) { return FinishShard{dz.n, 0, 1, 0, dz.n, 1, nullptr, 0, 0}; }
    static FinishShard shard(const urh_ctx* ctx, const UrhDigitizer& dz, int64_t global_offset, int64_t n_total) {
        return FinishShard{dz.n, ctx->nccl_rank, ctx->nccl_world, global_offset, n_total, ctx->nccl_rank == ctx->nccl_world - 1 ? 1 : 0,
                           nullptr, 0, 0};
    }
    static FinishShard chunk(UrhChain* chain, int64_t s0, int64_t s1, int64_t n_total, int64_t row_base, int64_t rows_cap) {
        return FinishShard{s1 - s0, 0, 1, s0, n_total, s1 == n_total ? 1 : 0, chain, row_base, rows_cap};
    }
};
int finish_tiles(urh_ctx* ctx, const UrhDigitizer& dz, const FinishShard& sh, int64_t* k);

struct UrhCandidates {
    int64_t count;
    int64_t* pos;
    int16_t* cls;
    int32_t last_cls;
    int64_t last_len;
};

int urh_collect_candidates(urh_ctx* ctx, int64_t n, int tol, const UrhTileSummary* tiles, const uint32_t* staging,
                           int stage_cap, UrhCandidates* out);

struct UrhShardCarry {
    int valid;
    int cls;
    int64_t len;
};
int urh_collect_candidates_shard(urh_ctx* ctx, int64_t n, int tol, const UrhTileSummary* tiles, const uint32_t* staging,
                                 int stage_cap, UrhShardCarry carry_in, int64_t global_offset, UrhCandidates* out);
int urh_shard_run_total(urh_ctx* ctx, int64_t n, const UrhTileSummary* tiles, int64_t* h_out);
```

Measured before the change: 216,900.

## Consolidate center results into one record and cut host round-trips in FSK path

Groups the center, state, certification, straddle, redone flag and row counts into one device record so the host fetches them with a single copy and sync instead of several small copies. The speculative guess kernel is spread over many blocks with a last-block reduction and warp-matched histogram updates. It also takes over zeroing the fine histogram and init buffers, replacing separate memsets. The finish step can write its row count on the device and skip the retry loop, falling back to a second pass only when the row capacity is exceeded. CERT_THREADS is doubled. The trade-off is more coupling between kernels and an extra fallback path that must stay correct.

After: 218,400 (median of 6 runs). Within noise of the previous version (+0.7%).

```diff
diff --git a/urh_b200/csrc/center.cu b/urh_b200/csrc/center.cu
--- a/urh_b200/csrc/center.cu
+++ b/urh_b200/csrc/center.cu
@@ -385,15 +385,11 @@
     CenStats local;
     double hmin, edge1, delta;
     long long nbins;
-    double center;
+    CenterResult res;
     float centerf;
     float scale;
     int fast;
-    int state;
     unsigned int ticket;
-    int certified;
-    long long straddle;
-    long long pad;
 };
 
 __global__ void k_center_ranks(const int64_t* __restrict__ counts, int rank, int world, int64_t max_size, CenterPlan* __restrict__ plan) {
@@ -411,9 +407,9 @@
     b = b < 0 ? 0 : (b > kept ? kept : b);
     plan->lr0 = a; plan->lr1 = b;
     plan->ticket = 0u;
-    plan->state = 1;
-    plan->certified = 0;
-    plan->straddle = 0;
+    plan->res.state = 1;
+    plan->res.certified = 0;
+    plan->res.straddle = 0;
 }
 
 __device__ __forceinline__ int64_t cen_tile_of_rank(const int64_t* __restrict__ prefix, int64_t ntiles, int64_t r) {
@@ -550,8 +546,8 @@
             }
         }
         plan->hmin = hmin; plan->edge1 = edge1; plan->delta = delta; plan->nbins = nbins;
-        plan->state = state;
-        plan->center = 0.0; plan->centerf = 0.0f;
+        plan->res.state = state;
+        plan->res.center = 0.0; plan->centerf = 0.0f;
         if (state == 1) {
             plan->scale = (float)(1.0 / delta);
             const double edge_abs = fmax(fabs(hmin), fabs(hmin + (double)nbins * delta));
@@ -568,7 +564,7 @@
 __global__ void __launch_bounds__(256, MIN_BLOCKS) k_hist_interior(const float* __restrict__ x, int64_t n, const CenterPlan* __restrict__ plan,
                                                                   const float* __restrict__ g_fe, unsigned long long* __restrict__ hist,
                                                                   const int64_t* __restrict__ prefix, int edges_in_smem) {
-    if (plan->state != 1 || plan->certified || (plan->fast != 0) != FAST) return;
+    if (plan->res.state != 1 || plan->res.certified || (plan->fast != 0) != FAST) return;
     hist_interior_body<SMEM, FAST>(x, n, plan->win[0] + 1, plan->win[1], blockIdx.x, gridDim.x, g_fe, plan->scale, (int)plan->nbins, hist,
                                    edges_in_smem, prefix);
 }
@@ -582,7 +578,7 @@
                                                          const CenterPlan* __restrict__ plan, const float* __restrict__ g_fe,
                                                          unsigned long long* __restrict__ hist, unsigned long long* __restrict__ xhist,
                                                          int64_t slab_tiles) {
-    if (plan->state != 1) return;
+    if (plan->res.state != 1) return;
     if (blockIdx.x < 2) {
         hist_window_ends_body(x, n, prefix, (const int64_t*)plan->win, plan->lr0, plan->lr1, g_fe, plan->scale, (int)plan->nbins, hist, xhist);
         return;
@@ -607,7 +603,7 @@
     return cen_edge(k, plan->hmin, plan->edge1, plan->delta);
 }
 
-#define CERT_THREADS 512
+#define CERT_THREADS 1024
 __global__ void __launch_bounds__(CERT_THREADS) k_center_certify(const UrhFine fine, CenterPlan* __restrict__ plan, const float* __restrict__ fe,
                                                                  const unsigned long long* __restrict__ xhist, unsigned long long* __restrict__ lo,
                                                                  unsigned long long* __restrict__ hi) {
@@ -616,7 +612,7 @@
     __shared__ unsigned char s_flag[CEN_MAX_BINS];
     __shared__ unsigned long long s_key[3];
     __shared__ unsigned int s_certain;
-    if (plan->state != 1) return;
+    if (plan->res.state != 1) return;
     const int tid = threadIdx.x;
     constexpr int PER = URH_FINE_NB / CERT_THREADS;
     int64_t sf, se;
@@ -695,19 +691,19 @@
     }
     if (tid != 0 || s_certain < 2u) return;
     const int k1 = 8191 - (int)(s_key[0] & 8191), k2 = 8191 - (int)(s_key[1] & 8191);
-    plan->straddle = (long long)((hi[k1] - lo[k1]) + (hi[k2] - lo[k2]));
+    plan->res.straddle = (long long)((hi[k1] - lo[k1]) + (hi[k2] - lo[k2]));
     if (!(lo[k2] > s_key[2])) return;
     const double c = __ddiv_rn(__dadd_rn(cen_left_edge(plan, k1), cen_left_edge(plan, k2)), 2.0);
-    plan->center = c;
+    plan->res.center = c;
     plan->centerf = __double2float_rn(c);
-    plan->certified = 1;
+    plan->res.certified = 1;
 }
 
 __global__ void __launch_bounds__(256) k_center_pick(const unsigned long long* __restrict__ y, CenterPlan* __restrict__ plan) {
     __shared__ unsigned long long s_best[256];
     __shared__ int s_idx[256];
     __shared__ int s_cnt[256];
-    if (plan->state != 1 || plan->certified) return;
+    if (plan->res.state != 1 || plan->res.certified) return;
     const int nbins = (int)plan->nbins;
     int window = (int)(0.05 * (double)nbins) + 1;
     if (window < 2) window = 2;
@@ -782,14 +778,14 @@
         }
     }
     if (threadIdx.x != 0) return;
-    if (undecided) { plan->state = 2; return; }
-    if (found == 0) { plan->state = 0; return; }
+    if (undecided) { plan->res.state = 2; return; }
+    if (found == 0) { plan->res.state = 0; return; }
     double c;
     if (found == 1) c = cen_left_edge(plan, top_idx[0]);
     else c = __ddiv_rn(__dadd_rn(cen_left_edge(plan, top_idx[0]), cen_left_edge(plan, top_idx[1])), 2.0);
-    plan->center = c;
+    plan->res.center = c;
     plan->centerf = __double2float_rn(c);
-    plan->state = 1;
+    plan->res.state = 1;
     (void)top_val;
 }
 
@@ -800,8 +796,8 @@
     if (blockIdx.x == 0 && threadIdx.x == 0) {
         plan->lr0 = r0; plan->lr1 = r1;
         plan->ticket = 0u;
-        plan->state = 1;
-        plan->certified = 0;
+        plan->res.state = 1;
+        plan->res.certified = 0;
         if (nbins > 0) {
             long long w[4];
             cen_window_tiles(prefix, ntiles, r0, r1, w);
@@ -875,6 +871,12 @@
     return URH_OK;
 }
 
+int urh_center_plan_new(urh_ctx* ctx, CenterPlan** plan, CenterResult** rec) {
+    URH_CHECK(urh_arena(ctx, 1, plan));
+    *rec = &(*plan)->res;
+    return URH_OK;
+}
+
 int urh_center_chain(urh_ctx* ctx, const float* d_qad, int64_t n, const UrhTileStats* ts, int64_t max_size, int rank, int world,
                      const UrhFine* fine, CenterPlan** d_plan_out) {
     const int64_t ntiles = urh_div_up(n, URH_TILE);
@@ -888,7 +890,8 @@
     unsigned long long *xhist = nullptr, *cert_lo = nullptr, *cert_hi = nullptr;
     const int nb = ctx->sm_count * 2;
     URH_CHECK(urh_arena(ctx, (size_t)ntiles + 1, &prefix));
-    URH_CHECK(urh_arena(ctx, 1, &plan));
+    plan = *d_plan_out;
+    if (!plan) URH_CHECK(urh_arena(ctx, 1, &plan));
     URH_CHECK(urh_arena(ctx, (size_t)nb + 2, &partial));
     URH_CHECK(urh_arena(ctx, (size_t)CEN_MAX_BINS + 3, &fe));
     URH_CHECK(urh_arena(ctx, (size_t)CEN_MAX_BINS, &hist));
@@ -940,8 +943,8 @@
 
 int urh_center_plan_certify_stats(urh_ctx* ctx, const CenterPlan* plan, int64_t* h_dst3) {
     h_dst3[0] = h_dst3[1] = h_dst3[2] = 0;
-    URH_CUDA(ctx, cudaMemcpyAsync(h_dst3, &plan->certified, sizeof(int), cudaMemcpyDeviceToHost, ctx->stream));
-    URH_CUDA(ctx, cudaMemcpyAsync(h_dst3 + 2, &plan->straddle, sizeof(long long), cudaMemcpyDeviceToHost, ctx->stream));
+    URH_CUDA(ctx, cudaMemcpyAsync(h_dst3, &plan->res.certified, sizeof(int), cudaMemcpyDeviceToHost, ctx->stream));
+    URH_CUDA(ctx, cudaMemcpyAsync(h_dst3 + 2, &plan->res.straddle, sizeof(long long), cudaMemcpyDeviceToHost, ctx->stream));
     return URH_OK;
 }
 
@@ -952,7 +955,7 @@
 
 int urh_center_plan_result(urh_ctx* ctx, const CenterPlan* plan, const float** d_centerf, const double** d_center, const int** d_state) {
     if (d_centerf) *d_centerf = &plan->centerf;
-    if (d_center) *d_center = &plan->center;
-    if (d_state) *d_state = &plan->state;
+    if (d_center) *d_center = &plan->res.center;
+    if (d_state) *d_state = &plan->res.state;
     return URH_OK;
 }
diff --git a/urh_b200/csrc/dense.cuh b/urh_b200/csrc/dense.cuh
--- a/urh_b200/csrc/dense.cuh
+++ b/urh_b200/csrc/dense.cuh
@@ -58,6 +58,16 @@
             *out = t;
         }
     }
+};
+
+struct CenterResult {
+    double center;
+    int state;
+    int certified;
+    long long straddle;
+    unsigned int redone;
+    int pad;
+    int64_t rows[2];
 };
 
 #define URH_FINE_NB 4096
diff --git a/urh_b200/csrc/digitize.cu b/urh_b200/csrc/digitize.cu
--- a/urh_b200/csrc/digitize.cu
+++ b/urh_b200/csrc/digitize.cu
@@ -135,59 +135,95 @@
 #define URH_GUESS_SAMPLES 16384
 #define URH_GUESS_BINS 128
 #define URH_GUESS_THREADS 1024
+#define URH_GUESS_BLOCKS (URH_GUESS_SAMPLES / URH_GUESS_THREADS)
 __global__ void __launch_bounds__(URH_GUESS_THREADS) k_speculate_guess(const float2* __restrict__ iq, int64_t n, float noise_sqrd, int forced,
-                                                                      float forced_tg, float* __restrict__ d_tg, unsigned int* __restrict__ redone) {
-    constexpr int PER = URH_GUESS_SAMPLES / URH_GUESS_THREADS;
+                                                                      float forced_tg, float* __restrict__ d_tg, unsigned int* __restrict__ redone,
+                                                                      float* __restrict__ vals, float2* __restrict__ part, urhts::Ws ws,
+                                                                      uint4* __restrict__ zero, int64_t zero_n, int16_t* __restrict__ d_init) {
     __shared__ unsigned int s_hist[URH_GUESS_BINS];
     __shared__ float s_mn[32], s_mx[32];
+    __shared__ unsigned long long s_key[2];
+    __shared__ bool s_last;
+    for (int64_t i = (int64_t)blockIdx.x * blockDim.x + threadIdx.x; i < zero_n; i += (int64_t)gridDim.x * blockDim.x)
+        zero[i] = make_uint4(0u, 0u, 0u, 0u);
+    if (blockIdx.x == 0 && threadIdx.x == 0) {
+        *redone = 0u;
+        if (d_init)
+            for (int j = 0; j < 8; j++) d_init[j] = 0;
+        if (forced) *d_tg = forced_tg;
+    }
     if (forced) {
-        if (threadIdx.x == 0) { *d_tg = forced_tg; *redone = 0u; }
+        if (threadIdx.x == 0) atomicAdd(ws.counter, 1ull);
         return;
     }
     for (int b = threadIdx.x; b < URH_GUESS_BINS; b += blockDim.x) s_hist[b] = 0u;
-    float v[PER];
+    const int q = blockIdx.x * URH_GUESS_THREADS + threadIdx.x;
+    const int64_t i = 1 + (int64_t)q * (n - 1) / URH_GUESS_SAMPLES;
+    const float2 p = iq[i - 1], c = iq[i];
+    float v = NAN;
     float mn = INFINITY, mx = -INFINITY;
-#pragma unroll
-    for (int k = 0; k < PER; k++) {
-        const int64_t i = 1 + (int64_t)(k * URH_GUESS_THREADS + threadIdx.x) * (n - 1) / URH_GUESS_SAMPLES;
-        const float2 p = iq[i - 1], c = iq[i];
-        v[k] = NAN;
-        if (!(c.x * c.x + c.y * c.y <= noise_sqrd)) {
-            v[k] = atan2f(p.x * c.y - p.y * c.x, p.x * c.x + p.y * c.y);
-            mn = fminf(mn, v[k]);
-            mx = fmaxf(mx, v[k]);
-        }
-    }
+    if (!(c.x * c.x + c.y * c.y <= noise_sqrd)) {
+        v = atan2f(p.x * c.y - p.y * c.x, p.x * c.x + p.y * c.y);
+        mn = fminf(mn, v);
+        mx = fmaxf(mx, v);
+    }
+    vals[q] = v;
     for (int off = 16; off > 0; off >>= 1) {
         mn = fminf(mn, __shfl_xor_sync(URH_FULL_MASK, mn, off));
         mx = fmaxf(mx, __shfl_xor_sync(URH_FULL_MASK, mx, off));
     }
     if ((threadIdx.x & 31) == 0) { s_mn[threadIdx.x >> 5] = mn; s_mx[threadIdx.x >> 5] = mx; }
     __syncthreads();
+    if (threadIdx.x == 0) {
+        mn = INFINITY; mx = -INFINITY;
+        for (int w = 0; w < URH_GUESS_THREADS / 32; w++) { mn = fminf(mn, s_mn[w]); mx = fmaxf(mx, s_mx[w]); }
+        part[blockIdx.x] = make_float2(mn, mx);
+    }
+    __threadfence();
+    __syncthreads();
+    if (threadIdx.x == 0) s_last = atomicAdd(ws.counter, 1ull) - ws.base == (unsigned long long)gridDim.x - 1;
+    __syncthreads();
+    if (!s_last) return;
+    __threadfence();
     mn = INFINITY; mx = -INFINITY;
-    for (int w = 0; w < URH_GUESS_THREADS / 32; w++) { mn = fminf(mn, s_mn[w]); mx = fmaxf(mx, s_mx[w]); }
+    for (int b = 0; b < (int)gridDim.x; b++) {
+        const float2 r = __ldcg(part + b);
+        mn = fminf(mn, r.x);
+        mx = fmaxf(mx, r.y);
+    }
     const float width = (mx - mn) / URH_GUESS_BINS;
     if (width > 0.0f) {
-#pragma unroll
-        for (int k = 0; k < PER; k++)
-            if (!isnan(v[k])) atomicAdd(&s_hist[min((int)((v[k] - mn) / width), URH_GUESS_BINS - 1)], 1u);
-    }
+        const int lane = threadIdx.x & 31;
+        for (int k = threadIdx.x; k < URH_GUESS_SAMPLES; k += blockDim.x) {
+            const float u = __ldcg(vals + k);
+            const int bin = isnan(u) ? -1 : min((int)((u - mn) / width), URH_GUESS_BINS - 1);
+            const unsigned peers = __match_any_sync(URH_FULL_MASK, bin);
+            if (bin >= 0 && __ffs(peers) - 1 == lane) atomicAdd(&s_hist[bin], (unsigned)__popc(peers));
+        }
+    }
+    if (threadIdx.x < 2) s_key[threadIdx.x] = 0ull;
     __syncthreads();
-    if (threadIdx.x != 0) return;
-    *redone = 0u;
-    if (!(mn <= mx)) { *d_tg = 0.0f; return; }
-    if (!(width > 0.0f)) { *d_tg = mn; return; }
+    if (!(mn <= mx) || !(width > 0.0f)) {
+        if (threadIdx.x == 0) *d_tg = (mn <= mx) ? mn : 0.0f;
+        return;
+    }
     constexpr int WINDOW = (int)(0.05 * URH_GUESS_BINS) + 1;
-    int top[2] = {-1, -1};
-    for (int b = 0; b < URH_GUESS_BINS; b++) {
+    unsigned long long key = 0ull;
+    const int b = threadIdx.x;
+    if (b < URH_GUESS_BINS) {
         const unsigned int y = s_hist[b];
         bool peak = y > 0u;
         for (int d = 1; d < WINDOW && peak; d++)
             peak = y > (b + d < URH_GUESS_BINS ? s_hist[b + d] : 0u) && y > (b - d >= 0 ? s_hist[b - d] : 0u);
-        if (!peak) continue;
-        if (top[0] < 0 || y > s_hist[top[0]]) { top[1] = top[0]; top[0] = b; }
-        else if (top[1] < 0 || y > s_hist[top[1]]) top[1] = b;
-    }
+        if (peak) key = ((unsigned long long)y << 8) | (unsigned long long)(URH_GUESS_BINS - 1 - b);
+        if (key) atomicMax(&s_key[0], key);
+    }
+    __syncthreads();
+    const int top0 = s_key[0] ? URH_GUESS_BINS - 1 - (int)(s_key[0] & 255ull) : -1;
+    if (key && b != top0) atomicMax(&s_key[1], key);
+    __syncthreads();
+    if (threadIdx.x != 0) return;
+    int top[2] = {top0, s_key[1] ? URH_GUESS_BINS - 1 - (int)(s_key[1] & 255ull) : -1};
     if (top[0] < 0) *d_tg = 0.5f * (mn + mx);
     else if (top[1] < 0) *d_tg = mn + ((float)top[0] + 0.5f) * width;
     else *d_tg = mn + (0.5f * (float)(top[0] + top[1]) + 0.5f) * width;
@@ -651,6 +687,7 @@
                      const UrhFine* fine, CenterPlan** d_plan_out);
 int urh_center_plan_result(urh_ctx* ctx, const CenterPlan* plan, const float** d_centerf, const double** d_center, const int** d_state);
 int urh_center_plan_certify_stats(urh_ctx* ctx, const CenterPlan* plan, int64_t* h_dst3);
+int urh_center_plan_new(urh_ctx* ctx, CenterPlan** plan, CenterResult** rec);
 
 extern "C" int urh_shard_digitize(urh_ctx* ctx, const void* d_iq, int dtype, const float* d_qad_in, int64_t n, int has_halo,
                                   float noise_mag, int mod_type, float center, uint16_t tolerance, uint32_t samples_per_symbol,
@@ -678,11 +715,9 @@
 }
 
 struct CenterMail {
-    double center;
-    int state, pad;
+    CenterResult res;
     int64_t cert[3];
     int64_t kept;
-    unsigned int redone;
 };
 static_assert(40 * sizeof(int64_t) + sizeof(CenterMail) <= 64 * sizeof(int64_t), "CenterMail outgrows the mailbox");
 
@@ -706,6 +741,8 @@
     bool speculate;
     UrhSpec spec;
     UrhDigitizer dz;
+    CenterPlan* plan;
+    CenterResult* rec;
 };
 
 static int center_setup(urh_ctx* ctx, CenterStep& S, bool certify, bool tables, const char* forced_guess, int tol, uint32_t sps) {
@@ -715,21 +752,30 @@
         if (S.fine.slab_tiles < URH_WARPS_PER_BLOCK) S.fine.slab_tiles = URH_WARPS_PER_BLOCK;
         const int64_t nslabs = urh_div_up(S.ntiles, S.fine.slab_tiles);
         URH_CHECK(urh_arena(ctx, (size_t)(nslabs * URH_FINE_NB), &S.fine.gh));
-        URH_CUDA(ctx, cudaMemsetAsync(S.fine.gh, 0, (size_t)(nslabs * URH_FINE_NB) * sizeof(unsigned int), ctx->stream));
+        if (!S.speculate) URH_CUDA(ctx, cudaMemsetAsync(S.fine.gh, 0, (size_t)(nslabs * URH_FINE_NB) * sizeof(unsigned int), ctx->stream));
         S.fine.scale = (S.mod_type == URH_MOD_FSK) ? 512.0f : 4096.0f;
         S.fine.off = (S.mod_type == URH_MOD_FSK) ? 2048.0f : 0.0f;
     }
     S.cls.noise_value = urh_noise_value(S.mod_type);
     S.cls.order = 2;
     if (tables) URH_CHECK(S.dz.init(ctx, S.n, tol, S.mod_type == URH_MOD_ASK, sps, S.ntiles, false));
+    if (S.plan) S.spec.redone = &S.rec->redone;
     if (S.speculate) {
         float* tg;
+        float* vals;
+        float2* part;
+        urhts::Ws ws;
         URH_CHECK(urh_arena(ctx, 1, &tg));
-        URH_CHECK(urh_arena(ctx, 1, &S.spec.redone));
+        if (!S.spec.redone) URH_CHECK(urh_arena(ctx, 1, &S.spec.redone));
         URH_CHECK(urh_arena(ctx, (size_t)S.ntiles, &S.spec.margin));
+        URH_CHECK(urh_arena(ctx, URH_GUESS_SAMPLES, &vals));
+        URH_CHECK(urh_arena(ctx, URH_GUESS_BLOCKS, &part));
+        URH_CHECK(urhts::prepare(ctx, URH_GUESS_BLOCKS, &ws));
         S.spec.tg = tg;
-        URH_LAUNCH(ctx, k_speculate_guess, 1, URH_GUESS_THREADS, 0, (const float2*)S.d_iq, S.n, S.dp.noise_sqrd, forced_guess ? 1 : 0,
-                   forced_guess ? strtof(forced_guess, nullptr) : 0.0f, tg, S.spec.redone);
+        const int64_t zero_n = S.fine.gh ? urh_div_up(S.ntiles, S.fine.slab_tiles) * (URH_FINE_NB / 4) : 0;
+        URH_LAUNCH(ctx, k_speculate_guess, URH_GUESS_BLOCKS, URH_GUESS_THREADS, 0, (const float2*)S.d_iq, S.n, S.dp.noise_sqrd,
+                   forced_guess ? 1 : 0, forced_guess ? strtof(forced_guess, nullptr) : 0.0f, tg, S.spec.redone, vals, part, ws,
+                   (uint4*)S.fine.gh, zero_n, tables ? S.dz.d_init : (int16_t*)nullptr);
     }
     return URH_OK;
 }
@@ -784,8 +830,8 @@
     const double* d_center;
     const int* d_state;
     urh_center_plan_result(ctx, plan, nullptr, &d_center, &d_state);
-    URH_CUDA(ctx, cudaMemcpyAsync(&mail->center, d_center, sizeof(double), cudaMemcpyDeviceToHost, ctx->stream));
-    URH_CUDA(ctx, cudaMemcpyAsync(&mail->state, d_state, sizeof(int), cudaMemcpyDeviceToHost, ctx->stream));
+    URH_CUDA(ctx, cudaMemcpyAsync(&mail->res.center, d_center, sizeof(double), cudaMemcpyDeviceToHost, ctx->stream));
+    URH_CUDA(ctx, cudaMemcpyAsync(&mail->res.state, d_state, sizeof(int), cudaMemcpyDeviceToHost, ctx->stream));
     return urh_center_plan_certify_stats(ctx, plan, mail->cert);
 }
 
@@ -793,7 +839,7 @@
                                     int64_t* rows) {
     const float* d_centerf;
     urh_center_plan_result(ctx, plan, &d_centerf, nullptr, nullptr);
-    URH_CUDA(ctx, cudaMemsetAsync(S.dz.d_init, 0, 16, ctx->stream));
+    if (!S.speculate) URH_CUDA(ctx, cudaMemsetAsync(S.dz.d_init, 0, 16, ctx->stream));
     const int vec_in = (((uintptr_t)S.d_qad % 8) == 0) ? 1 : 0;
     int64_t grid = urh_div_up(S.ntiles, URH_WARPS_PER_BLOCK);
     if (S.speculate) {
@@ -804,9 +850,21 @@
     }
     URH_LAUNCH(ctx, (k_dense_f32<SrcQad2, float>), (unsigned)grid, URH_WARPS_PER_BLOCK * 32, 0, (const float*)S.d_qad, S.n, vec_in, S.cls,
                S.dz.tol, S.dz.tiles, S.dz.staging, S.dz.cap, S.dz.d_init, 0, d_centerf, (const UrhTileStats*)S.ts, S.spec);
+    if (S.rec) {
+        URH_CHECK(finish_tiles(ctx, S.dz, sh, rows, S.rec->rows));
+        URH_CUDA(ctx, cudaMemcpyAsync(&mail->res, S.rec, sizeof(CenterResult), cudaMemcpyDeviceToHost, ctx->stream));
+        URH_CUDA(ctx, cudaStreamSynchronize(ctx->stream));
+        mail->cert[0] = mail->res.certified;
+        mail->cert[1] = 0;
+        mail->cert[2] = mail->res.straddle;
+        if (mail->res.rows[0] > (int64_t)ctx->pulses_cap_rows) return finish_tiles(ctx, S.dz, sh, rows);
+        *rows = mail->res.rows[0];
+        ctx->pulses_k = *rows;
+        return URH_OK;
+    }
     URH_CHECK(center_copy_results(ctx, plan, mail));
-    mail->redone = 0u;
-    if (S.speculate) URH_CUDA(ctx, cudaMemcpyAsync(&mail->redone, S.spec.redone, sizeof(unsigned int), cudaMemcpyDeviceToHost, ctx->stream));
+    mail->res.redone = 0u;
+    if (S.speculate) URH_CUDA(ctx, cudaMemcpyAsync(&mail->res.redone, S.spec.redone, sizeof(unsigned int), cudaMemcpyDeviceToHost, ctx->stream));
     return finish_tiles(ctx, S.dz, sh, rows);
 }
 
@@ -816,7 +874,7 @@
     URH_CUDA(ctx, cudaMemcpyAsync(&mail->kept, (const int64_t*)ctx->center_prefix + S.ntiles, sizeof(int64_t), cudaMemcpyDeviceToHost,
                                   ctx->stream));
     URH_CUDA(ctx, cudaStreamSynchronize(ctx->stream));
-    if (mail->state != 1) return URH_OK;
+    if (mail->res.state != 1) return URH_OK;
     const float* d_centerf;
     urh_center_plan_result(ctx, plan, &d_centerf, nullptr, nullptr);
     StreamDigitizer sd;
@@ -852,6 +910,7 @@
     S.d_qad = d_qad_out;
     S.dp = make_demod_params(noise_mag, mod_type, dtype);
     S.speculate = !sharded && !h_iq && !sc && mod_type == URH_MOD_FSK && dtype == URH_DT_F32 && !no_speculate;
+    if (!sharded && !h_iq && !sc && mod_type == URH_MOD_FSK) URH_CHECK(urh_center_plan_new(ctx, &S.plan, &S.rec));
     URH_CHECK(center_setup(ctx, S, !sharded && !no_certify, !sc, forced_guess, tolerance, samples_per_symbol));
 
     StreamRing ring;
@@ -860,7 +919,7 @@
     else if (h_iq) URH_CHECK(center_demod_host(ctx, S, h_iq, chunk_samples));
     else URH_CHECK(center_demod(ctx, S, 0, S.ntiles));
 
-    CenterPlan* plan = nullptr;
+    CenterPlan* plan = S.plan;
     URH_CHECK(urh_center_chain(ctx, d_qad_out, n, S.ts, max_size, sharded ? ctx->nccl_rank : 0, sharded ? ctx->nccl_world : 1,
                                S.fine.gh ? &S.fine : nullptr, &plan));
 
@@ -872,17 +931,17 @@
         URH_CHECK(center_digitize_resident(ctx, S, plan, sharded ? FinishShard::shard(ctx, S.dz, global_offset, n_total) : FinishShard::local(S.dz),
                                            mail, &rows));
 
-    *center = mail->center;
-    *center_state = mail->state;
+    *center = mail->res.center;
+    *center_state = mail->res.state;
     if (sc) *sc->kept = mail->kept;
     ctx->center_cert[0] = mail->cert[0];
     ctx->center_cert[1] = S.fine.gh ? URH_FINE_NB : 0;
     ctx->center_cert[2] = mail->cert[2];
-    const int64_t redone = (S.spec.hi > S.spec.lo) ? mail->redone : 0;
+    const int64_t redone = (S.spec.hi > S.spec.lo) ? mail->res.redone : 0;
     ctx->spec_stats[0] = S.spec.hi - S.spec.lo;
     ctx->spec_stats[1] = S.spec.hi - S.spec.lo - redone;
     ctx->spec_stats[2] = redone;
-    if (mail->state != 1) {
+    if (mail->res.state != 1) {
         ctx->pulses_k = 0;
         rows = 0;
     }
diff --git a/urh_b200/csrc/finish.cu b/urh_b200/csrc/finish.cu
--- a/urh_b200/csrc/finish.cu
+++ b/urh_b200/csrc/finish.cu
@@ -191,7 +191,7 @@
         if (l_prev == CLS_NONE) l_prev = *d_prev0;
         l_idx = row_off[tl];
         l_pp = prev_fired[tl];
-        if (l_pp < 0) l_pp = *d_xprev_fired;
+        if (l_pp < 0 && d_xprev_fired) l_pp = *d_xprev_fired;
     }
     for (int j0 = 0; j0 < FIN_TILES && t0 + j0 < ntiles; j0 += FIN_BATCH) {
         uint32_t w0[FIN_BATCH];
@@ -321,11 +321,12 @@
     if (rows > 0) chain->last_state = table[2 * (rows - 1)];
 }
 
-int finish_tiles(urh_ctx* ctx, const UrhDigitizer& dz, const FinishShard& sh, int64_t* k) {
+int finish_tiles(urh_ctx* ctx, const UrhDigitizer& dz, const FinishShard& sh, int64_t* k, int64_t* d_got) {
     const int64_t n = sh.n;
     const int64_t ntiles = urh_div_up(n, URH_TILE);
     const bool sharded = sh.world > 1;
     UrhChain* chain = sh.chain;
+    if (d_got && (sharded || chain || dz.is_ask)) URH_FAIL(ctx, URH_ERR_INVALID, "finish_tiles: a deferred row count needs one whole FSK capture");
     RunCarry* carry;
     int32_t *head_rel, *prev_cls;
     int64_t *row_off, *prev_fired, *d_small;
@@ -337,7 +338,7 @@
     TileFire* fire;
     URH_CHECK(urh_arena(ctx, (size_t)ntiles, &fire));
     URH_CHECK(urh_arena(ctx, (size_t)(32 + 8 * (sharded ? sh.world : 0)), &d_small));
-    URH_CUDA(ctx, cudaMemsetAsync(d_small, 0xff, 4 * sizeof(int64_t), ctx->stream));
+    if (!d_got) URH_CUDA(ctx, cudaMemsetAsync(d_small, 0xff, 4 * sizeof(int64_t), ctx->stream));
     RunCarry* d_tot_run = (RunCarry*)(d_small + 4);
     CandAgg* d_tot_cand = (CandAgg*)(d_small + 6);
     FireAgg* d_tot_fire = (FireAgg*)(d_small + 8);
@@ -383,7 +384,7 @@
     FireAgg fi_ident;
     fi_ident.fired = 0; fi_ident.last_pos = -1;
     URH_CHECK((urhts::scan<FireAgg, FireOp, ScanFirings>(ctx, ntiles, fi_ident, FireOp(), fc, d_tot_fire)));
-    const int64_t* xprev = chain ? &chain->prev_fired : d_small + 2;
+    const int64_t* xprev = chain ? &chain->prev_fired : (d_got ? nullptr : d_small + 2);
     if (sharded) {
         URH_TL_MARK(ctx, "x6 firings: enter");
         URH_CHECK(urh_nccl_allgather(ctx, d_tot_fire, d_all3, sizeof(FireAgg)));
@@ -402,6 +403,13 @@
     int64_t* raw = ctx->pulses + 2 * row_base;
     int64_t raw_cap = chain ? sh.rows_cap : cap_rows;
     if (dz.is_ask) URH_CHECK(urh_arena(ctx, (size_t)raw_cap * 2, &raw));
+    if (d_got) {
+        URH_LAUNCH(ctx, k_finish_rows, (unsigned)urh_div_up(ntiles, 8 * FIN_TILES), 256, 0, dz.tiles, dz.staging, dz.cap, (const int32_t*)head_rel,
+                   (const int32_t*)prev_cls, prev0, (const int64_t*)row_off, (const int64_t*)prev_fired, xprev, ntiles, sh.global_offset,
+                   sh.n_total, dz.tol, 0, (int64_t)dz.sps, sh.emit_tail, (int64_t)0, raw, raw_cap, d_got);
+        *k = -1;
+        return URH_OK;
+    }
     int64_t got[2] = {0, 0};
     for (int attempt = 0; attempt < 2; attempt++) {
         URH_LAUNCH(ctx, k_finish_rows, (unsigned)urh_div_up(ntiles, 8 * FIN_TILES), 256, 0, dz.tiles, dz.staging, dz.cap, (const int32_t*)head_rel,
diff --git a/urh_b200/csrc/sparse.cuh b/urh_b200/csrc/sparse.cuh
--- a/urh_b200/csrc/sparse.cuh
+++ b/urh_b200/csrc/sparse.cuh
@@ -85,7 +85,7 @@
         return FinishShard{s1 - s0, 0, 1, s0, n_total, s1 == n_total ? 1 : 0, chain, row_base, rows_cap};
     }
 };
-int finish_tiles(urh_ctx* ctx, const UrhDigitizer& dz, const FinishShard& sh, int64_t* k);
+int finish_tiles(urh_ctx* ctx, const UrhDigitizer& dz, const FinishShard& sh, int64_t* k, int64_t* d_got = nullptr);
 
 struct UrhCandidates {
     int64_t count;
```
